# WeltXing/PyDyNet

Hardware: AMD Instinct MI355X
Metric: training-step samples/sec (6L Llama3, seq=256) (higher is better)
Workload: dtype f32

## Files before the change

### pydynet_amd/_lib.py

```python
from __future__ import annotations

import ctypes
import os
import re

_HERE = os.path.dirname(os.path.abspath(__file__))
LIB_PATH = os.environ.get("PDN_LIB") or os.path.join(_HERE, "libpdnhip.so")
HEADER_PATH = os.path.join(os.path.dirname(_HERE), "include", "pdn_hip.h")
EXT_HEADER_PATHS = (os.path.join(os.path.dirname(_HERE), "include", "pdn_optim.h"),)
LOSS_HEADER_PATHS = (os.path.join(os.path.dirname(_HERE), "include", "pdn_loss.h"),)
SEG_HEADER_PATHS = (os.path.join(os.path.dirname(_HERE), "include", "pdn_segattn.h"),)
ROWLOSS_HEADER_PATHS = (os.path.join(os.path.dirname(_HERE), "include", "pdn_rowloss.h"),)
SMOOTH_HEADER_PATHS = (os.path.join(os.path.dirname(_HERE), "include", "pdn_smoothloss.h"),)
EDIT_HEADER_PATHS = (os.path.join(os.path.dirname(_HERE), "include", "pdn_logitedit.h"),)
PERSAMPLE_HEADER_PATHS = (os.path.join(os.path.dirname(_HERE), "include", "pdn_persample.h"),)
FSM_HEADER_PATHS = (os.path.join(os.path.dirname(_HERE), "include", "pdn_fsm.h"),)
NORMGRAD_HEADER_PATHS = (os.path.join(os.path.dirname(_HERE), "include", "pdn_normgrad.h"),)

_CTYPE = {
    "int": ctypes.c_int,
    "int64_t": ctypes.c_int64,
    "float": ctypes.c_float,
    "double": ctypes.c_double,
}


def parse_header(path: str = HEADER_PATH):
    text = open(path).read()
    text = re.sub(r"/\*.*?\*/", "", text, flags=re.S)
    text = re.sub(r"//[^\n]*", "", text)
    protos = {}
    for m in re.finditer(r"(const\s+char\s*\*|int64_t|int)\s+(pdn[xlsrzeqfg]?_\w+)\s*\(([^)]*)\)\s*;", text, flags=re.S):
        ret, name, args = m.group(1), m.group(2), m.group(3)
        restype = ctypes.c_char_p if "char" in ret else _CTYPE[ret]
        argtypes = []
        args = args.strip()
        if args and args != "void":
            for a in args.split(","):
                a = a.strip()
                if "*" in a:
                    argtypes.append(ctypes.c_void_p)
                else:
                    base = a.replace("const", "").split()[0]
                    argtypes.append(_CTYPE[base])
        protos[name] = (restype, argtypes)
    return protos


class HipLibraryError(RuntimeError):

    def __init__(self, message, code=None):
        super().__init__(message)
        self.code = code


class _Lib:
    def __init__(self):
        if not os.path.exists(LIB_PATH):
            raise HipLibraryError(
                f"{LIB_PATH} not found: build it with `python -c 'import __graft_entry__ as g; g.build()'` "
                "(or `make -C pydynet_amd/csrc`). The HIP backend has no CPU fallback.")
        self.cdll = ctypes.CDLL(LIB_PATH, mode=ctypes.RTLD_GLOBAL)
        self.protos = parse_header()
        for path in (EXT_HEADER_PATHS + LOSS_HEADER_PATHS + SEG_HEADER_PATHS + ROWLOSS_HEADER_PATHS + SMOOTH_HEADER_PATHS
                     + EDIT_HEADER_PATHS + PERSAMPLE_HEADER_PATHS + FSM_HEADER_PATHS + NORMGRAD_HEADER_PATHS):
            self.protos.update(parse_header(path))
        self.fn = {}
        for name, (restype, argtypes) in self.protos.items():
            f = getattr(self.cdll, name)
            f.restype = restype
            f.argtypes = argtypes
            self.fn[name] = f
        self._last_error = self.fn["pdn_last_error"]
        self.free = self.fn["pdn_free"]

    def call(self, name, *args):
        rc = self.fn[name](*args)
        if rc != 0:
            msg = self._last_error()
            raise HipLibraryError(f"{name} failed (code {rc}): {msg.decode() if msg else ''}", rc)

    def query(self, name, *args):
        return self.fn[name](*args)


_LIB = None


def lib() -> _Lib:
    global _LIB
    if _LIB is None:
        _LIB = _Lib()
    return _LIB


def provides(name: str) -> bool:
    L = lib()
    fn = getattr(L, "fn", None)
    return name in fn if fn is not None else hasattr(L, name)


def is_built() -> bool:
    return os.path.exists(LIB_PATH)
```

### pydynet_amd/core/fused/_common.py

```python
from __future__ import annotations

import os

import numpy as np

from ...autograd import is_grad_enable
from ..tensor import Graph


def _hip():
    from ... import hipnp
    return hipnp


def _L():
    from ... import _lib
    return _lib.lib()


def _provides(name):
    from ... import _lib
    return _lib.provides(name)


# ... 37 lines not shown
def _is_leaf_f32(t):
    return (t.requires_grad and not t.last and t.grad is not None and t.grad.dtype == np.float32
            and (isinstance(t.grad, np.ndarray) or t.grad.is_contiguous()))


class _Deferred:

    _pending = None

    def _init_deferred(self, inputs, shape, dtype):
        self._pending, self._shape, self._dtype = tuple(inputs), tuple(int(v) for v in shape), np.dtype(dtype)
        self.__dict__["_data"] = None
        self.device = inputs[0].device
        self.copy = None
        self.grad = None
        self.requires_grad = bool(is_grad_enable() and any(t.requires_grad for t in inputs))
        self.last = list(inputs) if self.requires_grad else []
        if self.requires_grad:
            Graph._add_node(self)

    @property
    def data(self):
        d = self.__dict__.get("_data")
        if d is None and self._pending is not None:
            inputs, self._pending = self._pending, None
            with self.device:
                d = self.forward_(*inputs)
            self.__dict__["_data"] = d
        return d

    @data.setter
    def data(self, value):
        self.__dict__["_data"] = value
        self._pending = None

    @property
    def shape(self): return self._shape if self._pending is not None else self.data.shape
    @property
    def dtype(self): return self._dtype if self._pending is not None else self.data.dtype
    @property
    def ndim(self): return len(self.shape)
    @property
    def size(self): return int(np.prod(self.shape, dtype=np.int64))


def _pack_columns(hp, weights):
    fin = weights[0].shape[0]
    outs = [w.shape[1] for w in weights]
    cat = hp.empty((fin, int(np.sum(outs))), np.float32)
    pos = 0
    for w, n in zip(weights, outs):
        cat[:, pos:pos + n] = w
        pos += n
    return cat


def _weight_blocks(hp, L, dcat, weights, T, fin):
    ws = [_contig(w.data) for w in weights]
    stack = hp.stacked_view(ws)
    kb = ws[0].shape[1]
    if (fin == 288 and stack is not None and abs(stack._strides[0]) < (1 << 40) and dcat.is_contiguous()
            and os.environ.get("PDN_NO_DX_BLOCKS", "0") != "1"
            and L.query("pdn_gemm_outres_blocks_supported", T, kb, len(ws))):
        return ws, stack, kb
    return None


class DeferredInputGrad:

    def __init__(self, hp, dcat, ws, stack, kb, shape, T):
        self._hp, self.dcat, self.ws, self.stack, self.kb, self.T = hp, dcat, ws, stack, kb, T
        self.shape, self.dtype, self._array = tuple(shape), np.dtype(np.float32), None

    def materialise(self):
        if self._array is None:
            hp = self._hp
            dx = hp.empty(self.shape, np.float32)
            _L().call("pdn_gemm_outres_blocks_nt_f32", self.dcat._ptr, self.ws[0]._ptr, self.stack._strides[0], self.kb,
                      len(self.ws), dx._ptr, None, self.T, self.dcat.shape[1], 288, hp.stream())
            self._array, self.dcat, self.ws, self.stack = dx, None, None, None
        return self._array


def _materialised(g):
    return g.materialise() if isinstance(g, DeferredInputGrad) else g


def _dx_of_shared_input(hp, node, x, dcat, weights, T, fin, side=None):
    L = _L()
    blocks = _weight_blocks(hp, L, dcat, weights, T, fin)
    existing = getattr(node, "_existing", None)
    if (blocks is not None and side is None and not two_stream["enabled"] and type(x).__dict__.get("takes_deferred_grad", False)
            and type(x).fuse_bwd and T >= type(x).fuse_bwd_min_rows and x.device.is_hip and x.shape[-1] == 288
            and existing is not None and existing[0] is None and x.grad is None and x.last and x.requires_grad
            and hp.capturing() is None
            and _provides("pdng_outres_blocks_nt_rmsnorm_bwd_f32")):
        ws, stack, kb = blocks
        return DeferredInputGrad(hp, dcat, ws, stack, kb, x.shape, T)
    dx = hp.empty(x.shape, np.float32)
    ex = _foldable(node, 0, x)
    exr = ex.reshape(T, fin) if ex is not None else None
    if blocks is not None:
        ws, stack, kb = blocks
        L.call("pdn_gemm_outres_blocks_nt_f32", dcat._ptr, ws[0]._ptr, stack._strides[0], kb, len(ws),
               dx._ptr, exr._ptr if exr is not None else None, T, dcat.shape[1], fin, hp.stream())
    else:
        wcat = _pack_columns(hp, [w.data for w in weights])
        hp.gemm(dcat, wcat.T, dx.reshape(T, fin), residual=exr)
    return dx


def _gemm_raw(L, st, M, N, K, a_ptr, a_rs, a_cs, b, c_ptr, ldc, beta=0.0, residual_ptr=None, b_transposed=False):
    rs, cs = (b._strides[1], b._strides[0]) if b_transposed else (b._strides[0], b._strides[1])
    L.call("pdn_gemm_f32", M, N, K, 1.0, a_ptr, a_rs, a_cs, b._ptr, rs, cs, beta, c_ptr, ldc, None, 1, 1,
           0, 0, 0, 0, 0, 0, residual_ptr, None, 0, None, 0, st)
```

### pydynet_amd/core/fused/attn.py

```python
from __future__ import annotations

import contextlib
import math
import os

import numpy as np

from . import segments as _seg
from .norm import rms_norm
from ..tensor import Tensor, _Operator
from ._common import _hip, _L, _contig, _require_f32, _beside, _is_leaf_f32, _dx_of_shared_input


def _attn_layout(x):
    B, Lx, H, hd = x.shape
    st = x._strides
    if st[3] != 1 or (H > 1 and st[2] != hd) or st[1] % 4 or (B > 1 and st[0] % 4) or x._ptr % 16:
        return None
    return st[1], (st[0] if B > 1 else 0)


def _attn_mask_args(mask, B, H, Lq, Lk):
    if mask is None:
        return None, 0, 0, 0, 0, None
    m = mask
    if m.dtype != np.float32:
        m = m.astype(np.float32)
    shape = (1,) * (4 - m.ndim) + tuple(m.shape)
    if m.ndim > 4 or any(s not in (1, t) for s, t in zip(shape, (B, H, Lq, Lk))):
        raise ValueError(f"attention mask of shape {mask.shape} does not broadcast to {(B, H, Lq, Lk)}")
    m = _contig(m).reshape(shape)
    st = [0 if s == 1 else k for s, k in zip(shape, m._strides)]
    return m._ptr, st[0], st[1], st[2], st[3], m


def _key_bias_of(mask, B, H, Lq, Lk):
    shape = (1,) * (4 - mask.ndim) + tuple(mask.shape) if mask.ndim <= 4 else None
    if shape is None or shape[1] != 1 or shape[2] != 1 or shape[3] != Lk or shape[0] not in (1, B):
        return None
    m = mask if mask.dtype == np.float32 else mask.astype(np.float32)
    return _contig(m).reshape(shape[0], Lk)


_STREAM_MAX_BH = 65535


def _attn_kernel(B, H, hd, Lq, Lk, start_pos, mask, layouts):
    if not attention.use_flash or any(l is None for l in layouts):
        return None, None
    ql, kl, vl = layouts
    if Lq == Lk and start_pos == 0 and attention.use_resident and ql == kl == vl:
        kb = _key_bias_of(mask, B, H, Lq, Lk) if mask is not None else None
        if (mask is None or kb is not None) and _L().query("pdn_attention_supported", Lq, hd):
            return "resident", kb
    if _L().query("pdn_attention_stream_supported", hd) and kl == vl and B * H <= _STREAM_MAX_BH:
        return "stream", None
    return None, None


class SegmentBounds:
    __slots__ = ("start", "end", "shape", "on_hip")

    def __init__(self, start, end, shape, on_hip):
        self.start, self.end, self.shape, self.on_hip = start, end, tuple(shape), on_hip


def segment_bounds(segment_ids, on_hip):
    if isinstance(segment_ids, SegmentBounds):
        if segment_ids.on_hip != bool(on_hip):
            raise ValueError("segment bounds were made for another device")
        return segment_ids
    ids = segment_ids.data if isinstance(segment_ids, Tensor) else segment_ids
    if not on_hip:
        if not isinstance(ids, (np.ndarray, list, tuple)):
            ids = ids.get()
        ids = _seg.check(ids)
        start, end = _seg.bounds(ids)
        return SegmentBounds(start, end, ids.shape, False)
    hp, L = _hip(), _L()
    if isinstance(ids, (np.ndarray, list, tuple)):
        ids = hp.asarray(_seg.check(ids).astype(np.int32))
    elif ids.ndim != 2 or ids.dtype != np.int32:
        raise ValueError(f"segment_ids on the device must be a (B, L) int32 array, got shape {ids.shape} and dtype {ids.dtype}")
    ids = _contig(ids)
    B, Ls = ids.shape
    start, end = hp.empty((B, Ls), np.int32), hp.empty((B, Ls), np.int32)
    L.call("pdns_segment_bounds_i32", ids._ptr, B, Ls, start._ptr, end._ptr, hp.err_flag_ptr(), hp.stream())
    return SegmentBounds(start, end, (B, Ls), True)


def _segment_mask(seg, Lq):
    hp = _hip()
    keys = hp.asarray(np.arange(Lq, dtype=np.float32)).reshape(1, 1, 1, Lq)
    B = seg.shape[0]
# ... 109 lines not shown
    def backward_all(self, do):
        q, k, v = self.last
        B, Lq, H, hd = q.shape
        Lk = k.shape[1]
        causal = 1 if (self.causal and Lq > 1) else 0
        if self.xp is not np and self._kind == "segmented":
            hp, L = _hip(), _L()
            qd, kd, vd, seg, rs, bs = self._res
            self._res = None
            do = _contig(do)
            dq, dk, dv = (hp.empty((B, Lq, H, hd), np.float32) for _ in range(3))
            if rs != H * hd or (B > 1 and bs != Lq * H * hd):
                qd, kd, vd = qd.copy(), kd.copy(), vd.copy()
                rs, bs = H * hd, Lq * H * hd
            ws, wsb = hp.workspace(L.query("pdn_attention_bwd_workspace_bytes", B, H, Lq))
            L.call("pdns_attention_bwd_f32", qd._ptr, kd._ptr, vd._ptr, self.data._ptr, do._ptr, self._lse._ptr,
                   dq._ptr, dk._ptr, dv._ptr, B, H, Lq, hd, rs, bs, H * hd, Lq * H * hd, None, None, 0,
                   seg.start._ptr, seg.end._ptr, ws, wsb, hp.stream())
            return [dq, dk, dv]
        if self.xp is not np and self._kind == "resident":
            hp, L = _hip(), _L()
            qd, kd, vd, kb, rs, bs = self._res
            self._res = None
            do = _contig(do)
            dq, dk, dv = (hp.empty((B, Lq, H, hd), np.float32) for _ in range(3))
            if rs != H * hd or (B > 1 and bs != Lq * H * hd):
                qd, kd, vd = qd.copy(), kd.copy(), vd.copy()
                rs, bs = H * hd, Lq * H * hd
            ws, wsb = hp.workspace(L.query("pdn_attention_bwd_workspace_bytes", B, H, Lq))
            if kb is None:
                L.call("pdn_attention_bwd_f32", qd._ptr, kd._ptr, vd._ptr, self.data._ptr, do._ptr,
                       self._lse._ptr, dq._ptr, dk._ptr, dv._ptr, B, H, Lq, hd, rs, bs, H * hd, Lq * H * hd,
                       causal, None, None, ws, wsb, hp.stream())
            else:
                L.call("pdn_attention_bwd_bias_f32", qd._ptr, kd._ptr, vd._ptr, self.data._ptr, do._ptr,
                       self._lse._ptr, dq._ptr, dk._ptr, dv._ptr, B, H, Lq, hd, rs, bs, H * hd, Lq * H * hd,
                       causal, kb._ptr, Lq if kb.shape[0] > 1 else 0, ws, wsb, hp.stream())
            return [dq, dk, dv]
        if self.xp is not np and self._kind == "stream":
            hp, L = _hip(), _L()
            do = _contig(do)
            dq = hp.empty(q.shape, np.float32)
            ksrc, vsrc = _contig(k.data), _contig(v.data)
            dk, dv = hp.empty(k.shape, np.float32), hp.empty(v.shape, np.float32)
            klay = (H * hd, Lk * H * hd if B > 1 else 0)
            mp, sb, sh, sq, sk, keep = _attn_mask_args(self._mask_dev, B, H, Lq, Lk) \
                if self._mask_eff is not None else (None, 0, 0, 0, 0, None)
            ws, wsb = hp.workspace(L.query("pdn_attention_stream_bwd_workspace_bytes", B, H, Lq))
            qlay = (H * hd, Lq * H * hd if B > 1 else 0)
            qsrc = self._q_used
            L.call("pdn_attention_stream_bwd_f32", qsrc._ptr, ksrc._ptr, vsrc._ptr, self.data._ptr, do._ptr,
                   self._lse._ptr, dq._ptr, dk._ptr, dv._ptr, B, H, Lq, Lk, hd, qlay[0], qlay[1], klay[0], klay[1],
                   causal, self.start_pos, mp, sb, sh, sq, sk, None, None, ws, wsb, hp.stream())
            return [dq, dk, dv]
        p = self._p
        if self.xp is np:
            doT = do.transpose(0, 2, 1, 3)
            dv = np.matmul(p.swapaxes(-1, -2), doT).transpose(0, 2, 1, 3)
            dp = np.matmul(doT, v.data.transpose(0, 2, 3, 1))
            ds = (dp - (dp * p).sum(-1, keepdims=True)) * p / np.asarray(math.sqrt(hd), q.dtype)
            dq = np.matmul(ds, k.data.transpose(0, 2, 1, 3)).transpose(0, 2, 1, 3)
            dk = np.matmul(ds.swapaxes(-1, -2), q.data.transpose(0, 2, 1, 3)).transpose(0, 2, 1, 3)
            return [dq, dk, dv]
        hp, L = _hip(), _L()
        doT = do.transpose(0, 2, 1, 3)
        dv = hp.empty(v.shape, np.float32)
        hp.gemm(p.swapaxes(-1, -2), doT, dv.transpose(0, 2, 1, 3))
        dp = hp.empty(p.shape, np.float32)
        hp.gemm(doT, v.data.transpose(0, 2, 3, 1), dp)
        L.call("pdn_softmax_bwd_f32", p._ptr, dp._ptr, dp._ptr, B * H * Lq, Lk, math.sqrt(hd), hp.stream())
        dq, dk = hp.empty(q.shape, np.float32), hp.empty(k.shape, np.float32)
        hp.gemm(dp, k.data.transpose(0, 2, 1, 3), dq.transpose(0, 2, 1, 3))
        hp.gemm(dp.swapaxes(-1, -2), q.data.transpose(0, 2, 1, 3), dk.transpose(0, 2, 1, 3))
        return [dq, dk, dv]


class qkv_attention(_Operator):

    folds_existing = True
    enabled = True
    rope_epilogue = os.environ.get("PDN_NO_ROPE_EPILOGUE", "0") != "1"
    rope_min_rows = 4096
    prerotate = os.environ.get("PDN_NO_PREROTATE", "0") != "1"
    _rope_tables = {}

    @staticmethod
    def _rope_table(cos, sin, Lq, hd):
        hp, L = _hip(), _L()
        key = (cos._ptr, sin._ptr, Lq, hd)
        ent = qkv_attention._rope_tables.get(key)
        if ent is None:
            if len(qkv_attention._rope_tables) > 16:
                qkv_attention._rope_tables.clear()
            tab = hp.empty((Lq, hd, 2), np.float32)
            L.call("pdn_rope_table_f32", cos._ptr, sin._ptr, tab._ptr, Lq, hd, hp.stream())
            ent = qkv_attention._rope_tables[key] = (tab, cos, sin)
        return ent[0]

    def __init__(self, x, wq, wk, wv, cos, sin, n_heads, segment_ids=None):
        self._cos, self._sin, self.H = cos, sin, int(n_heads)
        self._segments = segment_ids
        super().__init__(x, wq, wk, wv)

    @staticmethod
    def _resident(L, hd):
        return bool(attention.use_resident and _L().query("pdn_attention_supported", L, hd))

    @staticmethod
    def applicable(x, L, hd, segment_ids=None):
        if not (qkv_attention.enabled and attention.use_flash and x.device.is_hip and x.dtype == np.float32
                and x.ndim == 3):
            return False
        if segment_ids is not None:
            return qkv_attention._resident(L, hd) and bool(_L().query("pdns_attention_supported", L, hd))
        return qkv_attention._resident(L, hd) or bool(_L().query("pdn_attention_stream_supported", hd))

    @staticmethod
    def _blocks(buf, T, D):
        hp = _hip()
        return hp.ndarray(buf._buf, buf._ptr, (3, T, D), (D, 3 * D, 1), buf.dtype)

    def forward_(self, x, wq, wk, wv):
        _require_f32(self, x, wq, wk, wv, self._cos, self._sin)
        hp, L = _hip(), _L()
        B, Lq, D = x.shape
        H, hd, T = self.H, D // self.H, B * Lq
        qkv = hp.empty((T, 3 * D), np.float32)
        blocks = self._blocks(qkv, T, D)
        ws = [_contig(w.data) for w in (wq, wk, wv)]
        stack = hp.stacked_view(ws)
        cos, sin = _contig(self._cos.data), _contig(self._sin.data)
        resident = qkv_attention._resident(Lq, hd)
        self.rotated = bool(qkv_attention.rope_epilogue and resident and stack is not None
                            and abs(stack._strides[0]) < (1 << 40)
                            and T >= qkv_attention.rope_min_rows
                            and L.query("pdn_qkv_rope_supported", T, D, D, Lq, hd))
        self.norm_folded = bool(self.rotated and isinstance(x, rms_norm) and x._pending is not None
                                and L.query("pdn_qkv_rope_norm_supported", T, D, D, Lq, hd))
        if self.norm_folded:
            raw_t, wn = x._pending
            raw = _contig(raw_t.data)
            xn, rms = hp.empty(x.shape, np.float32), hp.empty((T,), np.float32)
            tab = self._rope_table(cos, sin, Lq, hd)
            L.call("pdn_qkv_rope_norm_fwd_f32", raw._ptr, _contig(wn.data)._ptr, x.eps, xn._ptr, rms._ptr, ws[0]._ptr,
                   (ws[1]._ptr - ws[0]._ptr) // 4, qkv._ptr, tab._ptr, T, D, D, Lq, hd, D, hp.stream())
            x._adopt(raw, rms, xn)
        x2 = _contig(x.data).reshape(T, D)
        if self.norm_folded:
            pass
        elif self.rotated:
            tab = self._rope_table(cos, sin, Lq, hd)
            L.call("pdn_qkv_rope_fwd_f32", x2._ptr, ws[0]._ptr, (ws[1]._ptr - ws[0]._ptr) // 4, qkv._ptr, tab._ptr,
                   T, D, D, Lq, hd, D, hp.stream())
        elif stack is not None:
            hp.gemm(x2, stack, blocks)
        else:
            for i in range(3):
                hp.gemm(x2, ws[i], blocks[i])
        self.prerotated = bool(not self.rotated and resident and qkv_attention.rope_epilogue and qkv_attention.prerotate
                               and T >= qkv_attention.rope_min_rows
                               and L.query("pdn_attention_persistent_supported", Lq, hd))
        if self.prerotated:
            L.call("pdn_rope_rows_f32", qkv._ptr, cos._ptr, sin._ptr, qkv._ptr, T, Lq, 2 * H, hd, 3 * D, 3 * D, 0, hp.stream())
            self.rotated = True
        out = hp.empty((B, Lq, H, hd), np.float32)
        lse = hp.empty((B, H, Lq), np.float32)
        q, k, v = qkv._ptr, qkv._ptr + 4 * D, qkv._ptr + 8 * D
        self._seg = None
        if self._segments is not None:
            self._seg = seg = segment_bounds(self._segments, True)
            if seg.shape != (B, Lq) or not (resident and L.query("pdns_attention_supported", Lq, hd)):
                raise ValueError(f"qkv_attention: segment_ids of shape {seg.shape} for x of shape {tuple(x.shape)} "
                                 "(segments need a resident shape: see qkv_attention.applicable)")
            L.call("pdns_attention_fwd_f32", q, k, v, out._ptr, lse._ptr, B, H, Lq, hd, 3 * D, Lq * 3 * D, D, Lq * D,
                   None if self.rotated else cos._ptr, None if self.rotated else sin._ptr, seg.start._ptr, hp.stream())
        elif resident:
            L.call("pdn_attention_fwd_f32", q, k, v, out._ptr, lse._ptr, B, H, Lq, hd, 3 * D, Lq * 3 * D,
                   D, Lq * D, 1, None if self.rotated else cos._ptr, None if self.rotated else sin._ptr, hp.stream())
        else:
            if (3 * D) % 4 or D % 4:
                raise ValueError("qkv_attention: dim must be a multiple of 4")
            qd = blocks[0].copy()
            L.call("pdn_attention_stream_fwd_f32", qd._ptr, k, v, out._ptr, lse._ptr,
                   B, H, Lq, Lq, hd, D, Lq * D, 3 * D, Lq * 3 * D, 1 if Lq > 1 else 0, 0, None, 0, 0, 0, 0,
                   cos._ptr, sin._ptr, hp.stream())
        self._saved = (x2, qkv, lse, cos, sin)
        return out

    def backward_all(self, do):
        hp, L = _hip(), _L()
        x, wq, wk, wv = self.last
        B, Lq, D = x.shape
        H, hd, T = self.H, D // self.H, B * Lq
        x2, qkv, lse, cos, sin = self._saved
        do = _contig(do)
        dqkv = hp.empty((T, 3 * D), np.float32)
        dblocks = self._blocks(dqkv, T, D)
        q, k, v = qkv._ptr, qkv._ptr + 4 * D, qkv._ptr + 8 * D
        dq, dk, dv = dqkv._ptr, dqkv._ptr + 4 * D, dqkv._ptr + 8 * D
        if self._seg is not None:
            ws_, wsb = hp.workspace(L.query("pdn_attention_bwd_workspace_bytes", B, H, Lq))
            L.call("pdns_attention_bwd_f32", q, k, v, self.data._ptr, do._ptr, lse._ptr, dq, dk, dv, B, H, Lq, hd,
                   3 * D, Lq * 3 * D, D, Lq * D, cos._ptr, sin._ptr, 1 if self.rotated else 0,
                   self._seg.start._ptr, self._seg.end._ptr, ws_, wsb, hp.stream())
        elif qkv_attention._resident(Lq, hd):
            ws_, wsb = hp.workspace(L.query("pdn_attention_bwd_workspace_bytes", B, H, Lq))
            L.call("pdn_attention_bwd_rotated_f32" if self.rotated else "pdn_attention_bwd_f32", q, k, v, self.data._ptr,
                   do._ptr, lse._ptr, dq, dk, dv, B, H, Lq, hd,
                   3 * D, Lq * 3 * D, D, Lq * D, 1, cos._ptr, sin._ptr, ws_, wsb, hp.stream())
        else:
            ws_, wsb = hp.workspace(L.query("pdn_attention_stream_bwd_workspace_bytes", B, H, Lq))
            qd, dqd = self._blocks(qkv, T, D)[0].copy(), hp.empty((T, D), np.float32)
            L.call("pdn_attention_stream_bwd_f32", qd._ptr, k, v, self.data._ptr, do._ptr, lse._ptr, dqd._ptr, dk, dv,
                   B, H, Lq, Lq, hd, D, Lq * D, 3 * D, Lq * 3 * D, 1 if Lq > 1 else 0, 0, None, 0, 0, 0, 0,
                   cos._ptr, sin._ptr, ws_, wsb, hp.stream())
            dblocks[0] = dqd
        grads = [None] * 4
        weights = (wq, wk, wv)
        gstack = None
        if all(w.requires_grad and _is_leaf_f32(w) for w in weights):
            gstack = hp.stacked_view([w.grad for w in weights])
        side = _beside(hp, D, 3 * D, x.requires_grad and any(w.requires_grad for w in weights))
        dws = [hp.empty(w.shape, np.float32) if gstack is None and w.requires_grad and not _is_leaf_f32(w) else None
               for w in weights]
        with side or contextlib.nullcontext():
            if gstack is not None:
                hp.gemm(x2.T, dblocks, gstack, beta=1.0)
            else:
                for i, w in enumerate(weights):
                    if not w.requires_grad:
                        continue
                    if dws[i] is None:
                        hp.gemm(x2.T, dblocks[i], w.grad, beta=1.0)
                    else:
                        hp.gemm(x2.T, dblocks[i], dws[i])
                        grads[1 + i] = dws[i]
        if x.requires_grad:
            grads[0] = _dx_of_shared_input(hp, self, x, dqkv, (wq, wk, wv), T, D, side)
        if side is not None:
            side.join()
        return grads
```

### pydynet_amd/core/fused/ffn.py

```python
from __future__ import annotations

import contextlib
import os

import numpy as np

from .norm import rms_norm
from ..tensor import _Operator
from ._common import (_hip, _L, _contig, _require_f32, _foldable, _beside, _is_leaf_f32, _pack_columns, _dx_of_shared_input)


class gate_up_swiglu(_Operator):

    folds_existing = True
    enabled = True

    @staticmethod
    def applicable(x, wg, wu):
        return (gate_up_swiglu.enabled and x.device.is_hip and x.dtype == np.float32 and wg.dtype == np.float32
                and wu.dtype == np.float32 and wg.shape == wu.shape and wg.shape[1] % 4 == 0 and x.ndim >= 2)

    def __init__(self, x, w_gate, w_up):
        super().__init__(x, w_gate, w_up)

    @staticmethod
    def _halves(buf, T, F):
        hp = _hip()
        return hp.ndarray(buf._buf, buf._ptr, (2, T, F), (F, 2 * F, 1), buf.dtype)

    def forward_(self, x, wg, wu):
        _require_f32(self, x, wg, wu)
        hp, L = _hip(), _L()
        fin, F = wg.shape
        x2 = _contig(x.data).reshape(-1, fin)
        T = x2.shape[0]
        gu = hp.empty((T, 2 * F), np.float32)
        halves = self._halves(gu, T, F)
        ws = [_contig(wg.data), _contig(wu.data)]
        stack = hp.stacked_view(ws)
        if stack is not None:
            hp.gemm(x2, stack, halves)
        else:
            hp.gemm(x2, ws[0], halves[0])
            hp.gemm(x2, ws[1], halves[1])
        out = hp.empty(x.shape[:-1] + (F,), np.float32)
        L.call("pdn_swiglu_rows_fwd_f32", gu._ptr, out._ptr, T, F, hp.stream())
        self._saved = (x2, gu)
        return out

    def backward_all(self, dh):
        hp, L = _hip(), _L()
        x, wg, wu = self.last
        fin, F = wg.shape
        x2, gu = self._saved
        T = x2.shape[0]
        dh = _contig(dh)
        dgu = hp.empty((T, 2 * F), np.float32)
        L.call("pdn_swiglu_rows_bwd_f32", gu._ptr, dh._ptr, dgu._ptr, T, F, hp.stream())
        dhalves = self._halves(dgu, T, F)
        grads = [None] * 3
        weights = (wg, wu)
        gstack = None
        if all(w.requires_grad and _is_leaf_f32(w) for w in weights):
            gstack = hp.stacked_view([w.grad for w in weights])
        side = _beside(hp, fin, 2 * F, x.requires_grad and any(w.requires_grad for w in weights))
        dws = [hp.empty(w.shape, np.float32) if gstack is None and w.requires_grad and not _is_leaf_f32(w) else None
               for w in weights]
        with side or contextlib.nullcontext():
            if gstack is not None:
                hp.gemm(x2.T, dhalves, gstack, beta=1.0)
            else:
                for i, w in enumerate(weights):
                    if not w.requires_grad:
                        continue
                    if dws[i] is None:
                        hp.gemm(x2.T, dhalves[i], w.grad, beta=1.0)
                    else:
                        hp.gemm(x2.T, dhalves[i], dws[i])
                        grads[1 + i] = dws[i]
        if x.requires_grad:
            dx = hp.empty(x.shape, np.float32)
            ex = _foldable(self, 0, x)
            wcat = _pack_columns(hp, [wg.data, wu.data])
            hp.gemm(dgu, wcat.T, dx.reshape(T, fin), residual=ex.reshape(T, fin) if ex is not None else None)
            grads[0] = dx
        if side is not None:
            side.join()
        return grads


class ffn_swiglu(_Operator):

    folds_existing = True
    enabled = os.environ.get("PDN_NO_FFN_NODE", "0") != "1"
    epilogues = os.environ.get("PDN_NO_SWIGLU_EPILOGUE", "0") != "1"
    epilogue_min_rows = 4096

    @staticmethod
    def applicable(x, wg, wu, wd):
        return (ffn_swiglu.enabled and gate_up_swiglu.applicable(x, wg, wu) and wd.dtype == np.float32
                and wd.shape == (wg.shape[1], wg.shape[0]))

    def __init__(self, x, w_gate, w_up, w_down, residual=None):
        self.has_res = residual is not None
        super().__init__(*([x, w_gate, w_up, w_down] + ([residual] if self.has_res else [])))

    @staticmethod
    def _epilogue(T, F, fin, stack):
        return bool(ffn_swiglu.epilogues and stack is not None and T >= ffn_swiglu.epilogue_min_rows
                    and fin * F <= abs(stack._strides[0]) < (1 << 30) - fin * F
                    and _L().query("pdn_gateup_swiglu_supported", T, F, fin))

    def forward_(self, x, wg, wu, wd, r=None):
        _require_f32(self, x, wg, wu, wd, r)
        hp, L = _hip(), _L()
        fin, F = wg.shape
        T = x.size // fin
        gu = hp.empty((T, 2 * F), np.float32)
        h = hp.empty((T, F), np.float32)
        ws = [_contig(wg.data), _contig(wu.data)]
        stack = hp.stacked_view(ws)
        self.used_epilogue = self._epilogue(T, F, fin, stack)
        self.tiled_epilogue = bool(not self.used_epilogue and ffn_swiglu.epilogues and stack is not None
                                   and T >= ffn_swiglu.epilogue_min_rows and x.size == T * fin
                                   and L.query("pdn_gateup_swiglu_tiled_supported", T, F, fin))
        self.norm_folded = bool(self.used_epilogue and isinstance(x, rms_norm) and x._pending is not None
                                and L.query("pdn_gateup_swiglu_norm_supported", T, F, fin))
        if self.norm_folded:
            raw_t, wn = x._pending
            raw = _contig(raw_t.data)
            xn, rms = hp.empty(x.shape, np.float32), hp.empty((T,), np.float32)
            L.call("pdn_gateup_swiglu_norm_fwd_f32", raw._ptr, _contig(wn.data)._ptr, x.eps, xn._ptr, rms._ptr, ws[0]._ptr,
                   (ws[1]._ptr - ws[0]._ptr) // 4, gu._ptr, h._ptr, T, F, fin, fin, hp.stream())
            x._adopt(raw, rms, xn)
        x2 = _contig(x.data).reshape(-1, fin)
        if self.norm_folded:
            pass
        elif self.used_epilogue:
            L.call("pdn_gateup_swiglu_fwd_f32", x2._ptr, ws[0]._ptr, (ws[1]._ptr - ws[0]._ptr) // 4, gu._ptr, h._ptr,
                   T, F, fin, fin, hp.stream())
        elif self.tiled_epilogue:
            wsp, wsb = hp.workspace(L.query("pdn_gateup_swiglu_tiled_workspace_bytes", F, fin))
            L.call("pdn_gateup_swiglu_tiled_fwd_f32", x2._ptr, x2._strides[0], ws[0]._ptr, (ws[1]._ptr - ws[0]._ptr) // 4,
                   gu._ptr, h._ptr, T, F, fin, wsp, wsb, hp.stream())
        else:
            halves = gate_up_swiglu._halves(gu, T, F)
            if stack is not None:
                hp.gemm(x2, stack, halves)
            else:
                hp.gemm(x2, ws[0], halves[0])
                hp.gemm(x2, ws[1], halves[1])
            L.call("pdn_swiglu_rows_fwd_f32", gu._ptr, h._ptr, T, F, hp.stream())
        out = hp.empty(x.shape[:-1] + (fin,), np.float32)
        res = _contig(r.data).reshape(-1, fin) if r is not None else None
        hp.gemm(h, wd.data, out.reshape(-1, fin), residual=res)
        self._saved = (x2, gu, h)
        return out

    def backward_all(self, g):
        hp, L = _hip(), _L()
        x, wg, wu, wd = self.last[:4]
        fin, F = wg.shape
        x2, gu, h = self._saved
        T = x2.shape[0]
        grads = [None] * len(self.last)
        if self.has_res and self.last[4].requires_grad:
            grads[4] = g
        g2 = _contig(g).reshape(T, fin)
        if wd.requires_grad:
            if _is_leaf_f32(wd):
                hp.gemm(h.T, g2, wd.grad, beta=1.0)
            else:
                grads[3] = hp.empty((F, fin), np.float32)
                hp.gemm(h.T, g2, grads[3])
        if not (x.requires_grad or wg.requires_grad or wu.requires_grad):
            return grads
        dgu = hp.empty((T, 2 * F), np.float32)
        wdd = _contig(wd.data)
        if self.used_epilogue:
            L.call("pdn_swiglu_bwd_gemm_f32", g2._ptr, wdd._ptr, gu._ptr, dgu._ptr, T, F, fin, fin, hp.stream())
        elif self.tiled_epilogue and L.query("pdn_swiglu_bwd_tiled_supported", T, F, fin):
            L.call("pdn_swiglu_bwd_tiled_f32", g2._ptr, g2._strides[0], wdd._ptr, gu._ptr, dgu._ptr, T, F, fin, hp.stream())
        else:
            dh = hp.empty((T, F), np.float32)
            hp.gemm(g2, wdd.T, dh)
            L.call("pdn_swiglu_rows_bwd_f32", gu._ptr, dh._ptr, dgu._ptr, T, F, hp.stream())
        dhalves = gate_up_swiglu._halves(dgu, T, F)
        weights = (wg, wu)
        gstack = None
        if all(w.requires_grad and _is_leaf_f32(w) for w in weights):
            gstack = hp.stacked_view([w.grad for w in weights])
        if gstack is not None:
            hp.gemm(x2.T, dhalves, gstack, beta=1.0)
        else:
            for i, w in enumerate(weights):
                if not w.requires_grad:
                    continue
                if _is_leaf_f32(w):
                    hp.gemm(x2.T, dhalves[i], w.grad, beta=1.0)
                else:
                    grads[1 + i] = hp.empty(w.shape, np.float32)
                    hp.gemm(x2.T, dhalves[i], grads[1 + i])
        if x.requires_grad:
            grads[0] = _dx_of_shared_input(hp, self, x, dgu, (wg, wu), T, fin)
        return grads
```

### pydynet_amd/core/fused/norm.py

```python
from __future__ import annotations

import numpy as np

import os

from ...autograd import is_grad_enable
from ..tensor import _Operator
from ._common import (_hip, _L, _contig, _require_f32, _foldable, _is_leaf_f32, _Deferred, DeferredInputGrad, _materialised,
                      _provides)


class rms_norm(_Deferred, _Operator):

    folds_existing = True
    fold = os.environ.get("PDN_NO_NORM_FOLD", "0") != "1"
    fold_min_rows = 4096
    takes_deferred_grad = True
    fuse_bwd = os.environ.get("PDN_NO_NORM_BWD_FUSE", "0") != "1"
    fuse_bwd_min_rows = 65536

    def __init__(self, x, weight, eps=1e-6):
        self.eps = float(eps)
        if (rms_norm.fold and type(self) is rms_norm and x.device.is_hip and is_grad_enable()
                and x.dtype == np.float32 and weight.dtype == np.float32 and x.ndim >= 2 and x.shape[-1] == 288
                and weight.shape == (288,) and x.size // 288 >= rms_norm.fold_min_rows):
            self._init_deferred((x, weight), x.shape, np.float32)
        else:
            super().__init__(x, weight)

    def _adopt(self, raw, rms, out):
        self._x, self._rms = raw, rms
        self.data = out

    def forward_(self, x, w):
        if self.xp is np:
            self._rms = np.sqrt((x.data * x.data).mean(-1, keepdims=True) + np.asarray(self.eps, x.dtype))
            return x.data / self._rms * w.data
        _require_f32(self, x, w)
        hp, L = _hip(), _L()
        cols = x.shape[-1]
        self._x = _contig(x.data)
        rows = self._x.size // cols
        out = hp.empty(x.shape, np.float32)
        self._rms = hp.empty((rows,), np.float32)
        L.call("pdn_rmsnorm_fwd_f32", self._x._ptr, w.data._ptr, out._ptr, self._rms._ptr, rows, cols,
               self.eps, hp.stream())
        return out

    def backward_all(self, g):
        x, w = self.last
        if self.xp is np:
            z = x.data / self._rms
            dz = g * w.data
            dx = (dz - z * (z * dz).mean(-1, keepdims=True)) / self._rms
            return [dx if x.requires_grad else None,
                    (g * z).reshape(-1, w.shape[-1]).sum(0) if w.requires_grad else None]
        hp, L = _hip(), _L()
        cols = x.shape[-1]
        rows = self._x.size // cols
        fused = (isinstance(g, DeferredInputGrad) and x.requires_grad and cols == 288 and g.T == rows
                 and _provides("pdng_outres_blocks_nt_rmsnorm_bwd_f32"))
        g = g if fused else _contig(_materialised(g))
        dx = hp.empty(x.shape, np.float32)
        direct = w.requires_grad and _is_leaf_f32(w)
        dw = w.grad if direct else (hp.empty((cols,), np.float32) if w.requires_grad else None)
        ex = _foldable(self, 0, x) if x.requires_grad else None
        if fused:
            kb, nb = g.kb, len(g.ws)
            ws, wsb = hp.workspace(L.query("pdng_outres_blocks_nt_rmsnorm_bwd_workspace_bytes", rows, kb, nb))
            L.call("pdng_outres_blocks_nt_rmsnorm_bwd_f32", g.dcat._ptr, g.ws[0]._ptr, g.stack._strides[0], kb, nb,
                   self._x._ptr, w.data._ptr, self._rms._ptr, ex._ptr if ex is not None else None, dx._ptr,
                   dw._ptr if dw is not None else None, 1 if direct else 0, rows, g.dcat.shape[1], ws, wsb, hp.stream())
            return [dx, None if direct else dw]
        ws, wsb = hp.workspace(L.query("pdn_rmsnorm_bwd_workspace_bytes", rows, cols))
        L.call("pdn_rmsnorm_bwd_f32", self._x._ptr, w.data._ptr, self._rms._ptr, g._ptr,
               ex._ptr if ex is not None else None, dx._ptr,
               dw._ptr if dw is not None else None, 1 if direct else 0, rows, cols, ws, wsb, hp.stream())
        return [dx if x.requires_grad else None, None if direct else dw]


class layer_norm(_Operator):

    folds_existing = True

    def __init__(self, x, scale, shift, eps=1e-5):
        self.eps = float(eps)
        super().__init__(x, scale, shift)

    def forward_(self, x, w, b):
        if self.xp is np:
            mu = x.data.mean(-1, keepdims=True)
            self._c = x.data - mu
            self._sd = np.sqrt(np.square(self._c).mean(-1, keepdims=True) + np.asarray(self.eps, x.dtype))
            return self._c / self._sd * w.data + b.data
        _require_f32(self, x, w, b)
        hp, L = _hip(), _L()
        cols = x.shape[-1]
        self._x = _contig(x.data)
        rows = self._x.size // cols
        out = hp.empty(x.shape, np.float32)
        self._mean, self._rstd = hp.empty((rows,), np.float32), hp.empty((rows,), np.float32)
        L.call("pdn_layernorm_fwd_f32", self._x._ptr, _contig(w.data)._ptr, _contig(b.data)._ptr, out._ptr,
               self._mean._ptr, self._rstd._ptr, rows, cols, self.eps, hp.stream())
        return out

    def backward_all(self, g):
        x, w, b = self.last
        cols = x.shape[-1]
        if self.xp is np:
            xh = self._c / self._sd
            dz = g * w.data
            dx = (dz - dz.mean(-1, keepdims=True) - xh * (dz * xh).mean(-1, keepdims=True)) / self._sd
            return [dx if x.requires_grad else None,
                    (g * xh).reshape(-1, cols).sum(0).reshape(w.shape) if w.requires_grad else None,
                    g.reshape(-1, cols).sum(0).reshape(b.shape) if b.requires_grad else None]
        hp, L = _hip(), _L()
        rows = self._x.size // cols
        g = _contig(g)
        dx = hp.empty(x.shape, np.float32)
        dw_direct = w.requires_grad and _is_leaf_f32(w)
        db_direct = b.requires_grad and _is_leaf_f32(b)
        direct = dw_direct and db_direct
        dw = (w.grad if direct else hp.empty((cols,), np.float32)) if w.requires_grad else None
        db = (b.grad if direct else hp.empty((cols,), np.float32)) if b.requires_grad else None
        ws, wsb = hp.workspace(L.query("pdn_layernorm_bwd_workspace_bytes", rows, cols))
        ex = _foldable(self, 0, x) if x.requires_grad else None
        L.call("pdn_layernorm_bwd_f32", self._x._ptr, _contig(w.data)._ptr, self._mean._ptr, self._rstd._ptr, g._ptr,
               ex._ptr if ex is not None else None, dx._ptr, dw.reshape(-1)._ptr if dw is not None else None,
               db.reshape(-1)._ptr if db is not None else None, 1 if direct else 0, rows, cols, ws, wsb, hp.stream())
# ... 51 lines not shown
```

### pydynet_amd/csrc/gemm.hip

```cpp
#include "common.h"
#include <vector>
#include <mutex>
#include <stdlib.h>
#include <stdio.h>
#include <type_traits>

#include "gemm_tiled.h"
#include "gemm_stream.h"
#include "split_tn.h"

#include "gemm_select.h"
#include "gemm_prof.h"
#include "gemm_routes.h"


template <int WMV, int WNV, int WM, int WN, int BK, bool VEC, bool MASKS = false>
static void launch_layout(const GemmParams& p, bool a_kin, bool b_kin, dim3 grid, hipStream_t st) {
  constexpr int NT = WMV * WNV * 64;
  if (a_kin && b_kin)
    hipLaunchKernelGGL((gemm_f32_mfma_kernel<WMV, WNV, WM, WN, BK, true, true, VEC, false, MASKS>), grid, dim3(NT), 0, st, p);
  else if (a_kin && !b_kin)
    hipLaunchKernelGGL((gemm_f32_mfma_kernel<WMV, WNV, WM, WN, BK, true, false, VEC, false, MASKS>), grid, dim3(NT), 0, st, p);
  else if (!a_kin && b_kin)
    hipLaunchKernelGGL((gemm_f32_mfma_kernel<WMV, WNV, WM, WN, BK, false, true, VEC, false, MASKS>), grid, dim3(NT), 0, st, p);
// ... 27 lines not shown
extern "C" int pdn_gemm_prof_enable(int on) {
  std::lock_guard<std::mutex> lk(g_prof_mu);
  g_prof_on = on != 0;
  return PDN_OK;
}

extern "C" int pdn_gemm_prof_collect_fused(double* ms, double* flops, double* bytes, int64_t* launches) {
  std::lock_guard<std::mutex> lk(g_prof_mu);
  double tm = 0, tf = 0, tb = 0;
  int64_t n = 0;
  std::vector<ProfRec> keep;
  for (auto& r : g_prof) {
    if (r.family != 5) { keep.push_back(r); continue; }
    PDN_HIP(hipEventSynchronize(r.e1));
    float t = 0.f;
    PDN_HIP(hipEventElapsedTime(&t, r.e0, r.e1));
    tm += t; tf += r.flops; tb += r.bytes; n++;
    (void)hipEventDestroy(r.e0);
    (void)hipEventDestroy(r.e1);
  }
  g_prof.swap(keep);
  if (ms) *ms = tm;
  if (flops) *flops = tf;
  if (bytes) *bytes = tb;
  if (launches) *launches = n;
  return PDN_OK;
}

#define PDN_GEMM_FAMILIES 5
extern "C" int pdn_gemm_prof_collect_families(double* ms5, double* flops5, int64_t* launches5) {
  std::lock_guard<std::mutex> lk(g_prof_mu);
  double ms[PDN_GEMM_FAMILIES] = {0}, fl[PDN_GEMM_FAMILIES] = {0};
  int64_t n[PDN_GEMM_FAMILIES] = {0};
  for (auto& r : g_prof) {
    PDN_HIP(hipEventSynchronize(r.e1));
    float t = 0.f;
    PDN_HIP(hipEventElapsedTime(&t, r.e0, r.e1));
    const int f = r.family == 5 ? 2 : (r.family < 0 || r.family >= PDN_GEMM_FAMILIES ? 0 : r.family);
    ms[f] += t; fl[f] += r.flops; n[f]++;
    (void)hipEventDestroy(r.e0);
    (void)hipEventDestroy(r.e1);
  }
  for (int f = 0; f < PDN_GEMM_FAMILIES; ++f) {
    if (ms5) ms5[f] = ms[f];
    if (flops5) flops5[f] = fl[f];
    if (launches5) launches5[f] = n[f];
  }
  g_prof.clear();
  return PDN_OK;
}

extern "C" int pdn_gemm_prof_collect(double* total_ms, double* total_flops, int64_t* launches) {
  double ms[PDN_GEMM_FAMILIES], fl[PDN_GEMM_FAMILIES];
  int64_t n[PDN_GEMM_FAMILIES];
  int rc = pdn_gemm_prof_collect_families(ms, fl, n);
  if (rc) return rc;
  double tm = 0, tf = 0;
  int64_t tn = 0;
  for (int f = 0; f < PDN_GEMM_FAMILIES; ++f) { tm += ms[f]; tf += fl[f]; tn += n[f]; }
  if (total_ms) *total_ms = tm;
  if (total_flops) *total_flops = tf;
  if (launches) *launches = tn;
  return PDN_OK;
}

extern "C" int64_t pdn_gemm_f32_workspace_bytes(int M, int N, int K, int nbatch) {
  const int64_t base = (int64_t)64 * M * N * (int64_t)nbatch * 4;
  if (!pdn_outres_tn_split_supported(M, N, nbatch, K) && !(nbatch == 1 && pdn_down_dw_split_supported(M, N, K))) return base;
  return ((base + 255) & ~(int64_t)255) + pdn_outres_tn_split_extra_bytes(K);
}

struct GemmCall {
  GemmParams p;
  int nb1, nbatch;
  bool ext_on, mask_colsum;
  GemmLayout lay;
  int bt;
  int64_t ldb;
  void* workspace;
  int64_t workspace_bytes;
  int64_t ws_bytes, ws_floats;
  void* stream;
  hipStream_t st;
};
constexpr int kNotTaken = -0x7fffffff - 1;

static inline bool al16(const void* q) { return gemm_al16((uintptr_t)q); }

static int reduce_slabs(const GemmParams& p, int64_t total, int nbatch, int rvec, hipStream_t st) {
  const int blocks = (int)((total + 255) / 256 < 2048 ? (total + 255) / 256 : 2048);
  hipLaunchKernelGGL(gemm_splitk_reduce_kernel, dim3(blocks), dim3(256), 0, st, p, nbatch, rvec);
  PDN_LAUNCH_CHECK();
  return PDN_OK;
}

static int route_skinny(const GemmCall& c) {
  const GemmParams& p = c.p;
  if (!(p.M <= 4 && !c.ext_on && c.nbatch == 1 && !p.colsum && p.b_cs == 1 && p.a_cs == 1 && gemm_m4(p.N) && gemm_m4(p.b_rs) &&
        gemm_m4(p.ldc) && al16(p.B) && al16(p.C) && (!p.bias || al16(p.bias)) && (!p.residual || al16(p.residual)) && p.K > 0 &&
        (p.K <= 4096 || (int64_t)p.K <= 4ll * p.N)))
    return kNotTaken;
  const dim3 g((p.N + 127) / 128);
  switch (p.M) {
    case 1: hipLaunchKernelGGL((gemm_skinny_kernel<1>), g, dim3(256), 0, c.st, p); break;
    case 2: hipLaunchKernelGGL((gemm_skinny_kernel<2>), g, dim3(256), 0, c.st, p); break;
    case 3: hipLaunchKernelGGL((gemm_skinny_kernel<3>), g, dim3(256), 0, c.st, p); break;
    default: hipLaunchKernelGGL((gemm_skinny_kernel<4>), g, dim3(256), 0, c.st, p); break;
  }
  PDN_LAUNCH_CHECK();
  return PDN_OK;
}

static int route_narrow(GemmCall& c) {
  GemmParams& p = c.p;
  const int M = p.M, N = p.N, K = p.K;
  if (!(c.nbatch == 1 && !c.ext_on && N <= 16 && p.alpha == 1.f && !p.residual && !p.colsum && !getenv("PDN_GEMM_NO_NARROW")))
    return kNotTaken;
  if (p.beta == 0.f && pdn_gemm_narrow_nn_ok(M, N, K, p.a_rs, p.a_cs, p.A)) {
    if (getenv("PDN_GEMM_DEBUG")) fprintf(stderr, "pdn_gemm_f32 M=%d N=%d K=%d -> narrow NN\n", M, N, K);
    return pdn_gemm_narrow_nn_launch(p.A, p.a_rs, p.B, p.b_rs, p.b_cs, p.bias, p.C, p.ldc, M, N, K, c.stream);
  }
  int kps = 0;
  const int64_t cap = al16(c.workspace) ? c.ws_floats : 0;
  const int sp = !p.bias ? pdn_gemm_narrow_tn_plan(M, N, K, p.a_rs, p.a_cs, p.b_cs, p.A, cap, &kps) : 0;
  if (sp <= 0) return kNotTaken;
  if (getenv("PDN_GEMM_DEBUG")) fprintf(stderr, "pdn_gemm_f32 M=%d N=%d K=%d -> narrow TN (%d slabs)\n", M, N, K, sp);
  const int rc = pdn_gemm_narrow_tn_launch(p.A, p.a_cs, p.B, p.b_rs, (float*)c.workspace, M, N, K, kps, sp, c.stream);
  if (rc) return rc;
  p.splits = sp;
  return reduce_slabs(p, (int64_t)M * N, 1, (N % 4 == 0) && (p.ldc % 4 == 0) && al16(p.C), c.st);
}

static int route_outres(const GemmCall& c) {
  const GemmParams& p = c.p;
  const int M = p.M, N = p.N, K = p.K;
  if (!(c.nbatch == 1 && !c.ext_on && N == 288 && p.a_cs == 1 && p.alpha == 1.f && p.beta == 0.f && !p.colsum && K >= 768 &&
        al16(p.A) && al16(p.B) && !getenv("PDN_GEMM_NO_OUTRES")))
    return kNotTaken;
  const bool big = (M + 255) / 256 >= 224, mid = (M + 127) / 128 >= 224 && K >= 1536;
  int pl_nw, pl_kps;
  const bool cut = !big && M >= 8192 && K >= 1536 && pdn_gemm_outres_plan(M, K, &pl_nw, &pl_kps) > 1 &&
                   c.ws_bytes >= pdn_gemm_outres_workspace_bytes(M, K);
  if (!((big || mid || cut) && (c.bt || p.b_cs == 1) && pdn_gemm_outres_supported(M, N, K, p.a_rs, c.ldb, p.ldc, c.bt)))
    return kNotTaken;
  GemmProfScope prof(3, 2.0 * M * (double)N * (double)K, 0.0, c.stream);
  if (getenv("PDN_GEMM_DEBUG"))
    fprintf(stderr, "pdn_gemm_f32 M=%d N=%d K=%d -> output-resident (%s)\n", M, N, K, c.bt ? "NT" : "NN");
  return cut ? pdn_gemm_outres_ws_f32(p.A, p.B, p.C, p.bias, p.residual, M, N, K, p.a_rs, c.ldb, p.ldc, c.bt, c.workspace, c.ws_bytes,
                                      c.stream)
             : pdn_gemm_outres_f32(p.A, p.B, p.C, p.bias, p.residual, M, N, K, p.a_rs, c.ldb, p.ldc, c.bt, c.stream);
}

static int route_outres_split288(const GemmCall& c) {
  const GemmParams& p = c.p;
  const int M = p.M, N = p.N, K = p.K;
  if (!(c.nbatch == 1 && !c.ext_on && N == 288 && K == 288 && p.a_cs == 1 && p.alpha == 1.f && p.beta == 0.f && !p.colsum &&
        !getenv("PDN_GEMM_NO_OUTRES") && !getenv("PDN_GEMM_NO_ROWRES") && pdn_gemm_rowtile_mode(-1) != 3))
    return kNotTaken;
  auto overlaps_c = [&](const float* q, int64_t floats) {
    return q && q < (const float*)p.C + (int64_t)M * p.ldc && (const float*)p.C < q + floats;
  };
  if (!((c.bt || p.b_cs == 1) && pdn_rowtile_plain_ok(M, N, c.bt) && pdn_gemm_rowres_supported(M, N, K, p.a_rs, c.ldb, p.ldc, c.bt) &&
        !overlaps_c(p.A, (int64_t)M * p.a_rs) && !overlaps_c(p.B, (int64_t)288 * c.ldb) &&
        (p.residual == p.C || !overlaps_c(p.residual, (int64_t)M * p.ldc)) &&
        pdn_outres_split_takes(p.A, p.B, p.C, p.bias, p.residual, M, K, p.a_rs, c.ldb, p.ldc, c.bt, 0, 0, 1, c.stream)))
    return kNotTaken;
  if (getenv("PDN_GEMM_DEBUG"))
    fprintf(stderr, "pdn_gemm_f32 M=%d N=%d K=%d -> output-resident, split fp16 (%s)\n", M, N, K, c.bt ? "NT" : "NN");
  GemmProfScope prof(3, 2.0 * M * (double)N * (double)K, 0.0, c.stream);
  return pdn_outres_split_launch(p.A, p.B, p.C, p.bias, p.residual, M, K, p.a_rs, c.ldb, p.ldc, c.bt, 0, 0, c.stream, PDN_CNT_PROJ288_SPLIT);
}

static int route_rowres(const GemmCall& c) {
  const GemmParams& p = c.p;
  const int M = p.M, N = p.N, K = p.K, nbatch = c.nbatch;
  const bool one_dim = c.nb1 == 1 || p.nb2 == 1;
  const int64_t a_bs = c.nb1 == 1 ? p.a_bs2 : p.a_bs1, b_bs = c.nb1 == 1 ? p.b_bs2 : p.b_bs1, c_bs = c.nb1 == 1 ? p.c_bs2 : p.c_bs1;
  const bool blocks = nbatch > 1 && one_dim && a_bs == 0 && c_bs == N && p.ldc >= (int64_t)nbatch * N && !p.bias &&
                      N % 96 == 0 && (b_bs & 3) == 0;
  const int64_t n_all = (int64_t)N * (blocks ? nbatch : 1);
  const bool tilepiece = nbatch == 1 && K == 288 && n_all >= 96 && n_all % 32 == 0 && M >= 8192 &&
                         pdn_rowtile_plain_ok(M, (int)n_all, c.bt);
  if (!((nbatch == 1 || blocks) && !c.ext_on && K == 288 && p.a_cs == 1 && p.alpha == 1.f && p.beta == 0.f && !p.colsum &&
        (tilepiece || (!p.residual && n_all >= 768)) && n_all < (1 << 30) && M >= 8192 && al16(p.A) && al16(p.B) &&
        (!p.residual || al16(p.residual)) && !getenv("PDN_GEMM_NO_ROWRES")))
    return kNotTaken;
  if (!((c.bt || p.b_cs == 1) && pdn_gemm_rowres_supported(M, N, K, p.a_rs, c.ldb, p.ldc, c.bt))) return kNotTaken;
  GemmProfScope prof(2, 2.0 * M * (double)n_all * (double)K, 0.0, c.stream);
  if (getenv("PDN_GEMM_DEBUG"))
    fprintf(stderr, "pdn_gemm_f32 M=%d N=%lld K=%d -> row-resident (%s, %d block%s)\n", M, (long long)n_all, K,
            c.bt ? "NT" : "NN", blocks ? nbatch : 1, blocks ? "s" : "");
  return blocks ? pdn_gemm_rowres_blocks(p.A, p.B, p.C, M, (int)n_all, K, p.a_rs, c.ldb, p.ldc, c.bt, nbatch, b_bs, c.stream)
                : pdn_gemm_rowres_f32(p.A, p.B, p.C, p.bias, p.residual, M, N, K, p.a_rs, c.ldb, p.ldc, c.bt, c.stream);
}

static int route_outres_tn(GemmCall& c) {
  GemmParams& p = c.p;
  const int M = p.M, N = p.N, K = p.K;
  if (!(c.nbatch == 1 && !c.ext_on && M == 288 && p.a_rs == 1 && p.a_cs >= 288 && p.b_cs == 1 && p.alpha == 1.f && !p.colsum &&
        !p.bias && !p.residual && N >= 8192 && N % 32 == 0 && K % 32 == 0 && K >= 4096 && gemm_m4(p.a_cs) && gemm_m4(p.b_rs) &&
        al16(p.A) && al16(p.B) && (int64_t)288 * p.ldc < (1ll << 30) && (int64_t)32 * p.b_rs < (1ll << 30) &&
        !getenv("PDN_GEMM_NO_OUTRES")))
    return kNotTaken;
  int nw = 8, kps = K;
  const int splits = pdn_gemm_outres_tn_plan(N, K, &nw, &kps);
  const bool direct = splits == 1 && p.beta == 0.f;
  if (!(direct || (int64_t)splits * M * N <= c.ws_floats)) return kNotTaken;
  GemmProfScope prof(4, 2.0 * M * (double)N * (double)K, 0.0, c.stream);
  if (getenv("PDN_GEMM_DEBUG"))
    fprintf(stderr, "pdn_gemm_f32 M=%d N=%d K=%d -> output-resident TN (splits %d)\n", M, N, K, splits);
  const int rc = direct ? pdn_gemm_outres_tn_launch(p.A, p.B, p.C, N, K, p.a_cs, p.b_rs, p.ldc, 0, nw, kps, c.stream)
                        : pdn_gemm_outres_tn_launch(p.A, p.B, (float*)c.workspace, N, K, p.a_cs, p.b_rs, N, (int64_t)M * N, nw, kps,
                                                    c.stream);
  if (rc || direct) return rc;
  p.splits = splits;
  return reduce_slabs(p, (int64_t)M * N, 1, (p.ldc % 4 == 0) && al16(p.C) && al16(c.workspace), c.st);
}

static int route_outres_tn_blocks(GemmCall& c) {
  GemmParams& p = c.p;
  const int M = p.M, N = p.N, K = p.K, nbatch = c.nbatch;
  const bool one_dim = c.nb1 == 1 || p.nb2 == 1;
  const int64_t a_bs = c.nb1 == 1 ? p.a_bs2 : p.a_bs1, b_bs = c.nb1 == 1 ? p.b_bs2 : p.b_bs1;
  const int64_t n_all = (int64_t)N * nbatch;
  if (!(nbatch > 1 && one_dim && M == 288 && a_bs == 0 && b_bs == N && p.a_rs == 1 && p.a_cs >= 288 && p.b_cs == 1 &&
        p.b_rs >= n_all && p.alpha == 1.f && !p.colsum && !p.bias && !p.residual && N % 32 == 0 && n_all >= 768 && n_all <= 8192 &&
        K % 32 == 0 && K >= 16384 && gemm_m4(p.a_cs) && gemm_m4(p.b_rs) && al16(p.A) && al16(p.B) && !getenv("PDN_GEMM_NO_OUTRES")))
    return kNotTaken;
  int nw = 8, kps = K;
  int splits = pdn_gemm_outres_tn_plan((int)n_all, K, &nw, &kps);
  const int64_t xoff = (((int64_t)64 * M * n_all * 4 + 255) & ~(int64_t)255);
  const bool split16 = pdn_outres_tn_split_supported(M, N, nbatch, K) && pdn_outres_tn_split_enabled() && c.workspace &&
                       c.workspace_bytes >= xoff + pdn_outres_tn_split_extra_bytes(K) && al16(c.workspace);
  if (split16) {
    kps = ((K / 32 + pdn_outres_tn_split_ranges((int)n_all, K, splits) - 1) / pdn_outres_tn_split_ranges((int)n_all, K, splits)) * 32;
    splits = (K + kps - 1) / kps;
  }
  if (!(splits > 1 && (int64_t)splits * M * n_all <= c.ws_floats && nbatch * splits <= 65535)) return kNotTaken;
  GemmProfScope prof(4, 2.0 * M * (double)n_all * (double)K, 0.0, c.stream);
  if (getenv("PDN_GEMM_DEBUG"))
    fprintf(stderr, "pdn_gemm_f32 M=%d N=%lld K=%d -> output-resident TN%s (%d blocks, splits %d)\n", M,
            (long long)n_all, K, split16 ? ", split-fp16" : "", nbatch, splits);
  const int rc = split16 ? pdn_outres_tn_split_launch(p.A, p.B, (float*)c.workspace, (int)n_all, K, p.a_cs, p.b_rs, N, kps,
                                                      (char*)c.workspace + xoff, c.stream)
                         : pdn_gemm_outres_tn_blocks_launch(p.A, p.B, (float*)c.workspace, (int)n_all, K, p.a_cs, p.b_rs, N, nw, kps,
                                                            c.stream);
  if (rc) return rc;
  p.splits = splits;
  return reduce_slabs(p, (int64_t)M * n_all, nbatch,
                      (p.ldc % 4 == 0) && al16(p.C) && gemm_m4(p.c_bs1) && gemm_m4(p.c_bs2) && al16(c.workspace), c.st);
}

static int route_down_dw_split(GemmCall& c) {
  GemmParams& p = c.p;
  const int M = p.M, N = p.N, K = p.K;
  if (!(c.nbatch == 1 && !c.ext_on && p.a_rs == 1 && p.b_cs == 1 && p.alpha == 1.f && !p.colsum && !p.bias && !p.residual &&
        pdn_down_dw_split_supported(M, N, K) && p.a_cs >= M && p.b_rs >= N && gemm_m4(p.a_cs) && gemm_m4(p.b_rs) && al16(p.A) &&
        al16(p.B) && c.workspace && al16(c.workspace) && pdn_outres_tn_split_enabled() && !getenv("PDN_GEMM_NO_OUTRES")))
    return kNotTaken;
  const int64_t xoff = (((int64_t)64 * M * N * 4 + 255) & ~(int64_t)255);
  const int ranges = pdn_down_dw_split_ranges(M, K);
  const int kps = ((K / 32 + ranges - 1) / ranges) * 32;
  const int splits = (K + kps - 1) / kps;
  if (!(c.workspace_bytes >= xoff + pdn_outres_tn_split_extra_bytes(K) && splits > 1 && splits <= 64)) return kNotTaken;
  if (getenv("PDN_GEMM_DEBUG"))
    fprintf(stderr, "pdn_gemm_f32 M=%d N=%d K=%d -> output-resident TN, split-fp16, transposed (splits %d)\n", M, N, K, splits);
  GemmProfScope prof(4, 2.0 * M * (double)N * (double)K, 0.0, c.stream);
  const int rc = pdn_down_dw_split_launch(p.B, p.A, (float*)c.workspace, M, K, p.b_rs, p.a_cs, kps, (char*)c.workspace + xoff, c.stream);
  if (rc) return rc;
  p.splits = splits;
  return reduce_slabs(p, (int64_t)M * N, 1, (p.ldc % 4 == 0) && al16(p.C), c.st);
}

static int route_stream_or_tiled(GemmCall& c) {
  GemmParams& p = c.p;
  const int M = p.M, N = p.N, K = p.K, nbatch = c.nbatch;
  const bool a_kin = c.lay.a_kin, b_kin = c.lay.b_kin, vec = c.lay.vec;
  const GemmChoice ch = gemm_select(M, N, K, nbatch, p.a_rs, p.b_cs, c.lay, c.ext_on, p.colsum != nullptr, c.mask_colsum, c.ws_floats);
  PDN_CHECK_ARG(ch.cfg >= 0, "pdn_gemm_f32: no tile configuration");
  if (getenv("PDN_GEMM_DEBUG")) {
    char line[256];
    gemm_route_line(line, sizeof(line), M, N, K, nbatch, c.lay, ch);
    fputs(line, stderr);
  }
  p.tiles_m = ch.tiles_m; p.tiles_n = ch.tiles_n; p.k_per_split = ch.k_per_split; p.splits = ch.splits;
  PDN_CHECK_ARG((int64_t)nbatch * p.splits <= 65535, "pdn_gemm_f32: batch*splits too large (%d)",
                nbatch * p.splits);
  dim3 grid(p.tiles_m * p.tiles_n, nbatch * p.splits);
  hipStream_t st = c.st;

  GemmProfScope prof(ch.use_stream ? 1 : 0, 2.0 * M * N * (double)K * nbatch, 0.0, c.stream);
  if (ch.use_stream) {
    constexpr int SNW = kStreamWaves;
    const dim3 sgrid(p.tiles_m * p.tiles_n * p.splits, nbatch);
    switch (ch.kind) {
      case kStreamLdsEdge:
        switch (ch.sshape) {
          case 0: hipLaunchKernelGGL((gemm_tn_stream_lds_kernel<3, 3, SNW, true>), sgrid, dim3(SNW * 64), 0, st, p); break;
          case 1: hipLaunchKernelGGL((gemm_tn_stream_lds_kernel<5, 2, SNW, true>), sgrid, dim3(SNW * 64), 0, st, p); break;
          case 2: hipLaunchKernelGGL((gemm_tn_stream_lds_kernel<2, 5, SNW, true>), sgrid, dim3(SNW * 64), 0, st, p); break;
          case 3: hipLaunchKernelGGL((gemm_tn_stream_lds_kernel<4, 2, SNW, true>), sgrid, dim3(SNW * 64), 0, st, p); break;
          default: hipLaunchKernelGGL((gemm_tn_stream_lds_kernel<2, 4, SNW, true>), sgrid, dim3(SNW * 64), 0, st, p); break;
        }
        break;
      case kStreamDma: hipLaunchKernelGGL((gemm_tn_stream_dma_kernel<3, 3, SNW>), sgrid, dim3(SNW * 64), 0, st, p); break;
      case kStreamLds: hipLaunchKernelGGL((gemm_tn_stream_lds_kernel<3, 3, SNW, false>), sgrid, dim3(SNW * 64), 0, st, p); break;
      case kStreamDirect: hipLaunchKernelGGL((gemm_tn_stream_kernel<3, 3, SNW, false>), sgrid, dim3(SNW * 64), 0, st, p); break;
      case kStreamDirectEdge: hipLaunchKernelGGL((gemm_tn_stream_kernel<3, 3, SNW, true>), sgrid, dim3(SNW * 64), 0, st, p); break;
    }
  } else if (c.ext_on) {
    if (!vec) launch_layout<2, 2, 1, 1, 32, false, true>(p, a_kin, b_kin, grid, st);
    else switch (ch.cfg) {
      case 0: launch_layout<2, 2, 2, 2, 32, true, true>(p, a_kin, b_kin, grid, st); break;
      case 3: launch_layout<4, 1, 1, 2, 32, true, true>(p, a_kin, b_kin, grid, st); break;
      case 6: launch_layout<2, 2, 4, 2, 16, true, true>(p, a_kin, b_kin, grid, st); break;
      case 7: launch_layout<2, 2, 2, 4, 16, true, true>(p, a_kin, b_kin, grid, st); break;
      case 8: launch_layout<4, 1, 2, 3, 16, true, true>(p, a_kin, b_kin, grid, st); break;
      default: launch_layout<2, 2, 1, 1, 32, true, true>(p, a_kin, b_kin, grid, st); break;
    }
  } else if (vec) {
    switch (ch.cfg) {
      case 0: launch_layout<2, 2, 2, 2, 32, true>(p, a_kin, b_kin, grid, st); break;
      case 1: launch_layout<4, 1, 1, 3, 32, true>(p, a_kin, b_kin, grid, st); break;
      case 2: launch_layout<1, 4, 3, 1, 32, true>(p, a_kin, b_kin, grid, st); break;
      case 3: launch_layout<4, 1, 1, 2, 32, true>(p, a_kin, b_kin, grid, st); break;
      case 4: launch_layout<1, 4, 2, 1, 32, true>(p, a_kin, b_kin, grid, st); break;
      case 6: launch_layout<2, 2, 4, 2, 16, true>(p, a_kin, b_kin, grid, st); break;
      case 7: launch_layout<2, 2, 2, 4, 16, true>(p, a_kin, b_kin, grid, st); break;
      case 8: launch_layout<4, 1, 2, 3, 16, true>(p, a_kin, b_kin, grid, st); break;
      case 9: launch_layout<1, 4, 3, 2, 16, true>(p, a_kin, b_kin, grid, st); break;
      case 10: launch_layout<2, 1, 1, 3, 32, true>(p, a_kin, b_kin, grid, st); break;
      case 11: launch_layout<1, 2, 3, 1, 32, true>(p, a_kin, b_kin, grid, st); break;
      case 12: launch_layout<4, 1, 1, 3, 16, true>(p, a_kin, b_kin, grid, st); break;
      default: launch_layout<2, 2, 1, 1, 32, true>(p, a_kin, b_kin, grid, st); break;
    }
  } else {
    launch_layout<2, 2, 1, 1, 32, false>(p, a_kin, b_kin, grid, st);
  }
  PDN_LAUNCH_CHECK();
  if (p.splits <= 1) return PDN_OK;
  return reduce_slabs(p, (int64_t)M * N * nbatch, nbatch,
                      (N % 4 == 0) && (p.ldc % 4 == 0) && al16(p.C) && gemm_m4(p.c_bs1) && gemm_m4(p.c_bs2) &&
                          (!p.bias || al16(p.bias)) && (!p.residual || al16(p.residual)) && al16(c.workspace), st);
}

static int gemm_f32_impl(int M, int N, int K, float alpha, const float* A, int64_t a_rs,
                         int64_t a_cs, const float* B, int64_t b_rs, int64_t b_cs, float beta,
                         float* C, int64_t ldc, const float* bias, int nb1, int nb2,
                         int64_t a_bs1, int64_t a_bs2, int64_t b_bs1, int64_t b_bs2,
                         int64_t c_bs1, int64_t c_bs2, const float* residual,
                         float* b_colsum, int colsum_accumulate, void* workspace,
                         int64_t workspace_bytes, void* stream, uint32_t* relu_mask, const uint32_t* grad_mask,
                         float* mask_colsum = nullptr) {
  const bool ext_on = relu_mask || grad_mask;
  PDN_CHECK_ARG(!ext_on || (nb1 == 1 && nb2 == 1 && N % 32 == 0 && !b_colsum),
                "pdn_gemm_f32: the mask epilogues need one batch and N a multiple of 32 (N = %d)", N);
  PDN_CHECK_ARG(M >= 0 && N >= 0 && K >= 0 && nb1 >= 0 && nb2 >= 0, "pdn_gemm_f32: negative extent");
  if (M == 0 || N == 0 || nb1 == 0 || nb2 == 0) return PDN_OK;
  PDN_CHECK_ARG(A && B && C, "pdn_gemm_f32: null operand");
  PDN_CHECK_ARG(ldc >= N, "pdn_gemm_f32: ldc (%lld) < N (%d)", (long long)ldc, N);

  GemmCall c;
  GemmParams& p = c.p;
  p.A = A; p.B = B; p.C = C; p.bias = bias; p.ws = (float*)workspace;
  p.residual = residual; p.colsum = b_colsum; p.colsum_acc = colsum_accumulate;
  p.relu_mask = relu_mask; p.grad_mask = grad_mask; p.mask_colsum = grad_mask ? mask_colsum : nullptr;
  p.M = M; p.N = N; p.K = K;
  p.a_rs = a_rs; p.a_cs = a_cs; p.b_rs = b_rs; p.b_cs = b_cs; p.ldc = ldc;
  p.nb2 = nb2;
  p.a_bs1 = a_bs1; p.a_bs2 = a_bs2; p.b_bs1 = b_bs1; p.b_bs2 = b_bs2; p.c_bs1 = c_bs1; p.c_bs2 = c_bs2;
  p.alpha = alpha; p.beta = beta;
  c.nb1 = nb1; c.nbatch = nb1 * nb2;
  c.ext_on = ext_on; c.mask_colsum = mask_colsum != nullptr;
  c.lay = gemm_layout(M, N, K, a_rs, a_cs, b_rs, b_cs, a_bs1, a_bs2, b_bs1, b_bs2, (uintptr_t)A, (uintptr_t)B);
  c.bt = (b_rs == 1 && b_cs != 1) ? 1 : 0;
  c.ldb = c.bt ? b_cs : b_rs;
  c.workspace = workspace; c.workspace_bytes = workspace_bytes;
  c.ws_bytes = (workspace && workspace_bytes > 0) ? workspace_bytes : 0;
  c.ws_floats = c.ws_bytes / 4;
  c.stream = stream; c.st = (hipStream_t)stream;

  if (b_colsum) {
    if (c.lay.a_kin || c.lay.b_kin || !c.lay.vec || c.nbatch != 1) {
      pdn_set_error("pdn_gemm_f32: b_colsum needs the x^T @ g layout (A m-contiguous, B n-contiguous, aligned, unbatched)");
      return PDN_EUNSUPPORTED;
    }
  }
  int rc;
  if ((rc = route_skinny(c)) != kNotTaken) return rc;
  if ((rc = route_narrow(c)) != kNotTaken) return rc;
  if ((rc = route_outres(c)) != kNotTaken) return rc;
  if ((rc = route_outres_split288(c)) != kNotTaken) return rc;
  if ((rc = route_rowres(c)) != kNotTaken) return rc;
  if ((rc = route_outres_tn(c)) != kNotTaken) return rc;
  if ((rc = route_outres_tn_blocks(c)) != kNotTaken) return rc;
  if ((rc = route_down_dw_split(c)) != kNotTaken) return rc;
  return route_stream_or_tiled(c);
}

extern "C" int pdn_gemm_f32(int M, int N, int K, float alpha, const float* A, int64_t a_rs,
                            int64_t a_cs, const float* B, int64_t b_rs, int64_t b_cs, float beta,
                            float* C, int64_t ldc, const float* bias, int nb1, int nb2,
                            int64_t a_bs1, int64_t a_bs2, int64_t b_bs1, int64_t b_bs2,
                            int64_t c_bs1, int64_t c_bs2, const float* residual,
                            float* b_colsum, int colsum_accumulate, void* workspace,
                            int64_t workspace_bytes, void* stream) {
  return gemm_f32_impl(M, N, K, alpha, A, a_rs, a_cs, B, b_rs, b_cs, beta, C, ldc, bias, nb1, nb2, a_bs1, a_bs2, b_bs1, b_bs2,
                       c_bs1, c_bs2, residual, b_colsum, colsum_accumulate, workspace, workspace_bytes, stream, nullptr, nullptr);
}

extern "C" int pdn_relu_mask_supported(int64_t rows, int cols) { return rows > 0 && cols > 0 && cols % 32 == 0; }

extern "C" int pdn_linear_relu_fwd_f32(const float* x, int64_t x_rs, const float* W, int64_t w_rs, int64_t w_cs,
                                       const float* bias, float* h, int64_t ldh, uint32_t* mask, int M, int N, int K,
                                       void* stream) {
  PDN_CHECK_ARG(x && W && h && mask, "pdn_linear_relu_fwd_f32: null operand");
  PDN_CHECK_ARG(pdn_relu_mask_supported(M, N), "pdn_linear_relu_fwd_f32: out features must be a multiple of 32 (N = %d)", N);
  pdn_count(PDN_CNT_LINEAR_RELU_FWD);
  return gemm_f32_impl(M, N, K, 1.f, x, x_rs, 1, W, w_rs, w_cs, 0.f, h, ldh, bias, 1, 1, 0, 0, 0, 0, 0, 0, nullptr, nullptr, 0,
                       nullptr, 0, stream, mask, nullptr);
}

extern "C" int pdn_linear_dx_masked_f32(const float* g, int64_t g_rs, const float* W, int64_t w_rs, int64_t w_cs,
                                        float* dx, int64_t ld, const float* existing, const uint32_t* mask,
                                        float* colsum_partials, int M, int fin, int fout, void* stream) {
  PDN_CHECK_ARG(g && W && dx && mask, "pdn_linear_dx_masked_f32: null operand");
  PDN_CHECK_ARG(pdn_relu_mask_supported(M, fin), "pdn_linear_dx_masked_f32: in features must be a multiple of 32 (%d)", fin);
  PDN_CHECK_ARG(!colsum_partials || ((uintptr_t)colsum_partials & 15) == 0, "pdn_linear_dx_masked_f32: unaligned partials");
  pdn_count(PDN_CNT_LINEAR_DX_MASKED);
  return gemm_f32_impl(M, fin, fout, 1.f, g, g_rs, 1, W, w_cs, w_rs, 0.f, dx, ld, nullptr, 1, 1, 0, 0, 0, 0, 0, 0, existing,
                       nullptr, 0, nullptr, 0, stream, nullptr, mask, colsum_partials);
}

__global__ __launch_bounds__(256) void relu_mask_bwd_kernel(const float4* __restrict__ g, const uint32_t* __restrict__ mask,
                                                            float4* __restrict__ dz, int64_t n4) {
  for (int64_t i = (int64_t)blockIdx.x * 256 + threadIdx.x; i < n4; i += (int64_t)gridDim.x * 256) {
    const uint32_t w = mask[i >> 3] >> (4 * (i & 7));
    float4 v = g[i];
    v.x = (w & 1u) ? v.x : 0.f; v.y = (w & 2u) ? v.y : 0.f; v.z = (w & 4u) ? v.z : 0.f; v.w = (w & 8u) ? v.w : 0.f;
    dz[i] = v;
  }
}

extern "C" int pdn_relu_mask_bwd_f32(const float* g, const uint32_t* mask, float* dz, int64_t rows, int cols, void* stream) {
  PDN_CHECK_ARG(g && mask && dz, "pdn_relu_mask_bwd_f32: null operand");
  PDN_CHECK_ARG(pdn_relu_mask_supported(rows, cols) && (((uintptr_t)g | (uintptr_t)dz) & 15) == 0,
                "pdn_relu_mask_bwd_f32: cols must be a multiple of 32 and the arrays 16-byte aligned");
  const int64_t n4 = rows * cols / 4;
  const int blocks = (int)std::min<int64_t>((n4 + 255) / 256, 8192);
  hipLaunchKernelGGL(relu_mask_bwd_kernel, dim3(blocks), dim3(256), 0, (hipStream_t)stream, (const float4*)g, mask, (float4*)dz, n4);
  PDN_LAUNCH_CHECK();
  return PDN_OK;
}

__global__ __launch_bounds__(256) void swiglu_pack_weights_kernel(const float* __restrict__ wg, int64_t w_stride, float* __restrict__ out,
                                                                  int K, int F, int Np) {
  const int64_t total = (int64_t)K * (Np / 4);
  for (int64_t i = (int64_t)blockIdx.x * 256 + threadIdx.x; i < total; i += (int64_t)gridDim.x * 256) {
    const int k = (int)(i / (Np / 4)), c = (int)(i - (int64_t)k * (Np / 4)) * 4;
    const int grp = c >> 6, up = (c >> 5) & 1, col = 32 * grp + (c & 31);
    float4 v = make_float4(0.f, 0.f, 0.f, 0.f);
    if (col < F) v = *reinterpret_cast<const float4*>(wg + (up ? w_stride : 0) + (int64_t)k * F + col);
    *reinterpret_cast<float4*>(out + (int64_t)k * Np + c) = v;
  }
}

static int swiglu_packed_cols(int F) { return (2 * F + 255) / 256 * 256; }

extern "C" int pdn_gateup_swiglu_tiled_supported(int M, int F, int K) {
  return M >= 4096 && M % 128 == 0 && F >= 256 && F % 32 == 0 && K >= 64 && K % 4 == 0 && !getenv("PDN_NO_TILED_SWIGLU");
}
extern "C" int64_t pdn_gateup_swiglu_tiled_workspace_bytes(int F, int K) { return (int64_t)K * swiglu_packed_cols(F) * 4; }

static void swiglu_params(GemmParams& p, int M, int N, int K, int BM, int BN, int BK) {
  p.bias = nullptr; p.residual = nullptr; p.colsum = nullptr; p.colsum_acc = 0;
  p.relu_mask = nullptr; p.grad_mask = nullptr; p.mask_colsum = nullptr; p.ws = nullptr;
  p.M = M; p.N = N; p.K = K; p.nb2 = 1;
  p.a_bs1 = p.a_bs2 = p.b_bs1 = p.b_bs2 = p.c_bs1 = p.c_bs2 = 0;
  p.alpha = 1.f; p.beta = 0.f; p.splits = 1;
  p.k_per_split = (K + BK - 1) / BK * BK;
  p.tiles_m = (M + BM - 1) / BM; p.tiles_n = (N + BN - 1) / BN;
}

extern "C" int pdn_gateup_swiglu_tiled_fwd_f32(const float* x, int64_t ldx, const float* w_gate, int64_t w_stride, float* gu,
                                               float* h, int M, int F, int K, void* workspace, int64_t workspace_bytes,
                                               void* stream) {
  PDN_CHECK_ARG(x && w_gate && gu && h && workspace, "pdn_gateup_swiglu_tiled_fwd_f32: null operand");
  PDN_CHECK_ARG(pdn_gateup_swiglu_tiled_supported(M, F, K) && ldx % 4 == 0 && w_stride % 4 == 0 &&
                    ((((uintptr_t)x | (uintptr_t)w_gate | (uintptr_t)gu | (uintptr_t)h | (uintptr_t)workspace) & 15) == 0),
                "pdn_gateup_swiglu_tiled_fwd_f32: unsupported shape or alignment (M %d, F %d, K %d)", M, F, K);
  const int Np = swiglu_packed_cols(F);
// ... 132 lines not shown
```

### pydynet_amd/csrc/gemm_routes.h

```cpp
#pragma once
#include <stdint.h>

bool pdn_gemm_narrow_nn_ok(int M, int N, int K, int64_t a_rs, int64_t a_cs, const void* A);
int pdn_gemm_narrow_nn_launch(const float* A, int64_t lda, const float* B, int64_t b_rs, int64_t b_cs, const float* bias,
                              float* C, int64_t ldc, int M, int N, int K, void* stream);
int pdn_gemm_narrow_tn_plan(int Mc, int N, int K, int64_t a_rs, int64_t a_cs, int64_t b_cs, const void* A, int64_t ws_cap_floats,
                            int* kps);
int pdn_gemm_narrow_tn_launch(const float* A, int64_t a_cs, const float* B, int64_t b_rs, float* slabs, int Mc, int N, int K,
                              int kps, int splits, void* stream);

extern "C" int64_t pdn_gemm_outres_workspace_bytes(int M, int K);
extern "C" int pdn_gemm_outres_plan(int M, int K, int* nw, int* kps);
extern "C" int pdn_gemm_outres_supported(int M, int N, int K, int64_t lda, int64_t ldb, int64_t ldc, int b_trans);
extern "C" int pdn_gemm_outres_f32(const float* A, const float* B, float* C, const float* bias,
                                   const float* residual, int M, int N, int K, int64_t lda, int64_t ldb,
                                   int64_t ldc, int b_trans, void* stream);
extern "C" int pdn_gemm_outres_ws_f32(const float* A, const float* B, float* C, const float* bias, const float* residual,
                                      int M, int N, int K, int64_t lda, int64_t ldb, int64_t ldc, int b_trans,
                                      void* workspace, int64_t workspace_bytes, void* stream);
int pdn_outres_blocks_nt_launch(const float* A, const float* W, int64_t b_block_stride, int kb, int nb, float* C, int M,
                                int64_t lda, int64_t ldc, void* stream);
int pdn_gemm_outres_tn_plan(int N, int K, int* nw_out, int* k_per_split_out);
int pdn_gemm_outres_tn_launch(const float* X, const float* G, float* C, int N, int K, int64_t ldx, int64_t ldg,
                              int64_t ldc, int64_t slab, int nw, int k_per_split, void* stream);
int pdn_gemm_outres_tn_blocks_launch(const float* X, const float* G, float* C, int N, int K, int64_t ldx, int64_t ldg,
                                     int nb_cols, int nw, int k_per_split, void* stream);
int pdn_outres_ce_dx_launch(const float* logits, int64_t ldl, const float* lse, const int64_t* targets, float gscale,
                            const float* gdev, const float* W, int64_t ldw, float* dx, int64_t ldc,
                            const float* residual, int M, int V, void* workspace, int64_t workspace_bytes, void* stream);
int pdn_outres_ce_dw_launch(const float* X, const float* logits, float* C, int N, int K, int64_t ldx, int64_t ldg,
                            int64_t ldc, int64_t slab, int nw, int k_per_split, const float* lse,
                            const int64_t* targets, float gscale, const float* gdev, float* colsum, void* stream);
int pdn_outres_ce_dx_deferred_launch(const float* logits, int64_t ldl, const float* rowmax, int max_parts,
                                     const int64_t* targets, float gscale, const float* W, int64_t ldw, float* dx,
                                     int64_t ldc, float* lse_out, int M, int V, void* workspace, int64_t workspace_bytes,
                                     void* stream);
extern "C" int pdn_linear_ce_dx_deferred_supported(int64_t M, int V, int K);

int pdn_outres_split_takes(const float* A, const float* B, const float* C, const float* bias, const float* residual, int M,
                           int K, int64_t lda, int64_t ldb, int64_t ldc, int b_trans, int kb, int64_t b_bstride, int splits,
                           void* stream);
int pdn_outres_split_launch(const float* A, const float* B, float* C, const float* bias, const float* residual, int M, int K,
                            int64_t lda, int64_t ldb, int64_t ldc, int b_trans, int kb, int64_t b_bstride, void* stream,
                            int count_slot);
int pdn_outres_split_norm_bwd_partial_rows(int M);
int pdn_outres_split_norm_bwd_launch(const float* A, const float* W, int64_t b_bstride, int kb, int nb, const float* x,
                                     const float* w, const float* rms, const float* ex, float* dx, float* dwpart, int M,
                                     int64_t lda, void* stream);

int pdn_colsum_partials_launch(const float* part, int nb, int cols, float* out, int accumulate, void* stream);

extern "C" int pdn_gemm_rowres_supported(int M, int N, int K, int64_t lda, int64_t ldb, int64_t ldc, int b_trans);
int pdn_rowtile_plain_ok(int M, int N, int b_trans);
extern "C" int pdn_gemm_rowres_f32(const float* A, const float* B, float* C, const float* bias,
                                   const float* residual, int M, int N, int K, int64_t lda, int64_t ldb,
                                   int64_t ldc, int b_trans, void* stream);
int pdn_gemm_rowres_blocks(const float* A, const float* B, float* C, int M, int N, int K, int64_t lda, int64_t ldb,
                           int64_t ldc, int b_trans, int nblocks, int64_t b_block_stride, void* stream);
extern "C" int pdn_gemm_rowtile_mode(int mode);
```

### pydynet_amd/csrc/gemm_rowres.hip

```cpp
#include "common.h"
#include "gemm_rowtile.h"
#include "gemm_prof.h"
#include "gemm_routes.h"
#include <stdlib.h>

static int pdn_ablation_switch(const char* name) {
  const char* e = getenv(name);
  const int v = e ? atoi(e) : 0;
  if (v) fprintf(stderr, "[pdnhip] WARNING: %s=%d -- timing ablation active, results of the affected kernels are WRONG\n", name, v);
  return v;
}

typedef float f32x16 __attribute__((ext_vector_type(16)));

struct RowResParams {
  const float* A;
  const float* B;
  float* C;
  const float* bias;
  const float* residual;
  int M, N;
  int64_t lda, ldb, ldc;
  int chunks, chunks_per_wg;
  int cpb;
  int64_t b_bstride;
  float* H;
  const float* GU;
  const float2* rope;
  int64_t ldh;
  int F;
  int L, hd, rope_chunks;
  unsigned hd_magic;
  unsigned g_off, u_off;
  float* lse;
  int epi_ablate;
};

__device__ __forceinline__ void rr_glds16(const float* g, float* l) {
  __builtin_amdgcn_global_load_lds((const __attribute__((address_space(1))) void*)g,
                                   (__attribute__((address_space(3))) void*)l, 16, 0, 0);
}

#define RR_NC 96
#define RR_KP 96

__device__ __forceinline__ void rr_store(const RowResParams& p, f32x16 (&acc)[3], int m0, int c, int li, int lh,
                                         bool full, int nt) {
  float* __restrict__ Cw = p.C + (int64_t)m0 * p.ldc + c * RR_NC;
  const float* __restrict__ Rw = p.residual ? p.residual + (int64_t)m0 * p.ldc + c * RR_NC : nullptr;
  const unsigned ldc = (unsigned)p.ldc;
  unsigned o0 = (unsigned)(4 * lh) * ldc + li;
  asm volatile("" : "+v"(o0));
  float bv[3];
#pragma unroll
  for (int j = 0; j < 3; ++j) bv[j] = (p.bias && j < nt) ? p.bias[c * RR_NC + 32 * j + li] : 0.f;
  const int mrem = p.M - m0 - 4 * lh;
#define RR_ROWS(GUARD, RES)                                                      \
  {                                                                              \
    unsigned o = o0;                                                             \
    _Pragma("unroll") for (int q = 0; q < 4; ++q) {                              \
      _Pragma("unroll") for (int e = 0; e < 4; ++e) {                            \
        const int r = 4 * q + e;                                                 \
        if (!GUARD || 8 * q + e < mrem) {                                        \
          _Pragma("unroll") for (int j = 0; j < 3; ++j) {                        \
            if (!GUARD || j < nt) {                                              \
              float v = acc[j][r] + bv[j];                                       \
              if (RES) v += Rw[o + 32 * j];                                      \
              Cw[o + 32 * j] = v;                                                \
            }                                                                    \
          }                                                                      \
        }                                                                        \
        o += (e == 3) ? 5 * ldc : ldc;                                           \
      }                                                                          \
    }                                                                            \
  }
  if (p.epi_ablate & 4) {
  } else if (full && nt == 3) {
    if (Rw) RR_ROWS(false, true) else RR_ROWS(false, false)
  } else {
    if (Rw) RR_ROWS(true, true) else RR_ROWS(true, false)
  }
#undef RR_ROWS
#pragma unroll
  for (int j = 0; j < 3; ++j)
#pragma unroll
    for (int r = 0; r < 16; ++r) acc[j][r] = 0.f;
// ... 522 lines not shown
    p.rope = reinterpret_cast<const float2*>(epi->rope); p.L = epi->L; p.hd = epi->hd;
    p.rope_chunks = epi->rope_cols / RR_NC;
    p.hd_magic = (unsigned)(((1ull << 32) + (unsigned)epi->hd - 1) / (unsigned)epi->hd);
    p.g_off = epi->g_off; p.u_off = epi->u_off;
    p.lse = epi->lse;
  }
  static const int s_pdn_rowres_epi_ablate = pdn_ablation_switch("PDN_ROWRES_EPI_ABLATE");
  p.epi_ablate = s_pdn_rowres_epi_ablate;
  hipStream_t st = (hipStream_t)stream;
  static const int ablate = getenv("PDN_ROWRES_ABLATE") ? atoi(getenv("PDN_ROWRES_ABLATE")) : 0;
  static const int nw_env = getenv("PDN_ROWRES_NW") ? atoi(getenv("PDN_ROWRES_NW")) : 0;
  static const int stage_env = getenv("PDN_ROWRES_STAGE") ? atoi(getenv("PDN_ROWRES_STAGE")) : -1;
  const int rb8 = (M + 255) / 256;
  const int nw = kind ? 8 : nw_env ? nw_env : (rb8 >= 192 || (int64_t)rb8 * p.chunks >= 256) ? 8 : 4;
  const int stage = kind ? 1 : stage_env >= 0 ? stage_env : (nw == 8 ? 1 : 0);
  const int row_blocks = (M + 32 * nw - 1) / (32 * nw), target = nw == 4 ? 512 : 256;
  int nsplit = 1;
  while (row_blocks * nsplit < target && nsplit < p.chunks) ++nsplit;
  p.chunks_per_wg = (p.chunks + nsplit - 1) / nsplit;
  if (kind == 1) p.chunks_per_wg += p.chunks_per_wg & 1;
  if (kind == 4) p.chunks_per_wg = p.chunks;
  nsplit = (p.chunks + p.chunks_per_wg - 1) / p.chunks_per_wg;
  if (kind == 5 && !epi->lse) { const_cast<RowResEpi*>(epi)->parts = nsplit; return PDN_OK; }
  const dim3 grid(row_blocks, nsplit);
#define RR_LAUNCH(BT_, NW_, AB_) if (stage) hipLaunchKernelGGL((gemm_rowres_kernel<36, BT_, NW_, 1, 0>), grid, dim3(NW_ * 64), 0, st, p); else hipLaunchKernelGGL((gemm_rowres_kernel<36, BT_, NW_, 0, AB_>), grid, dim3(NW_ * 64), 0, st, p)
  if (kind == 1) {
    hipLaunchKernelGGL((gemm_rowres_kernel<36, false, 8, 1, 0, 1>), grid, dim3(512), 0, st, p);
  } else if (kind == 2) {
    hipLaunchKernelGGL((gemm_rowres_kernel<36, true, 8, 1, 0, 2>), grid, dim3(512), 0, st, p);
  } else if (kind == 3) {
    hipLaunchKernelGGL((gemm_rowres_kernel<36, false, 8, 1, 0, 3>), grid, dim3(512), 0, st, p);
  } else if (kind == 4) {
    hipLaunchKernelGGL((gemm_rowres_kernel<36, false, 8, 1, 0, 4>), grid, dim3(512), 0, st, p);
  } else if (kind == 5) {
    hipLaunchKernelGGL((gemm_rowres_kernel<36, false, 8, 1, 0, 5>), grid, dim3(512), 0, st, p);
  } else if (nw == 8) {
    if (b_trans) RR_LAUNCH(true, 8, 0); else RR_LAUNCH(false, 8, 0);
  } else if (b_trans) {
    RR_LAUNCH(true, 4, 0);
  } else if (ablate == 2) {
    RR_LAUNCH(false, 4, 2);
  } else if (ablate == 32) {
    RR_LAUNCH(false, 4, 32);
  } else {
    RR_LAUNCH(false, 4, 0);
  }
#undef RR_LAUNCH
  pdn_count(PDN_CNT_ROWRES_CHUNK);
  if (kind) pdn_count(PDN_CNT_ROWRES_CHUNK_EPI);
  PDN_LAUNCH_CHECK();
  return PDN_OK;
}

extern "C" int pdn_gateup_swiglu_supported(int M, int F, int K) {
  return (K == 288 && F % RR_NC == 0 && F >= RR_NC && M >= 1 && (int64_t)64 * F < (1ll << 29)) ? 1 : 0;
}
extern "C" int pdn_gateup_swiglu_fwd_f32(const float* x, const float* w_gate, int64_t w_stride, float* gu, float* h, int M,
                                         int F, int K, int64_t ldx, void* stream) {
  if (M == 0 || F == 0) return PDN_OK;
  PDN_CHECK_ARG(x && w_gate && gu && h, "pdn_gateup_swiglu_fwd_f32: null operand");
  const int64_t ws = w_stride < 0 ? -w_stride : w_stride;
  if (!pdn_gateup_swiglu_supported(M, F, K) || ws % 4 != 0 || ws < (int64_t)K * F || ws + (int64_t)K * F >= (1ll << 30)) {
    pdn_set_error("pdn_gateup_swiglu_fwd_f32: unsupported shape M=%d F=%d K=%d (K 288, F a multiple of 96)", M, F, K);
    return PDN_EUNSUPPORTED;
  }
  RowResEpi e{1, h, F, nullptr, F, nullptr, 1, 1, 0};
  e.g_off = w_stride < 0 ? (unsigned)ws : 0u;
  e.u_off = w_stride < 0 ? 0u : (unsigned)ws;
  const float* wbase = w_stride < 0 ? w_gate + w_stride : w_gate;
  const int tk = pdn_gemm_prof_begin(5, 2.0 * M * (2.0 * F) * K, 4.0 * ((double)M * K + 2.0 * K * F + 3.0 * M * F), stream);
  const int rc = rowres_launch(x, wbase, gu, nullptr, nullptr, M, 2 * F, K, ldx, F, 2 * F, 0, 2, ws, stream, &e);
  pdn_gemm_prof_end(tk, stream);
  return rc;
}
static int rowtile_would_take(int M, int N, int epi, int F) {
  RowTileArgs ta;
  memset(&ta, 0, sizeof(ta));
  ta.M = M; ta.N = N; ta.lda = 288; ta.ldb = N; ta.ldc = N; ta.nblocks = 1; ta.epi = epi; ta.F = F;
  return pdn_rowtile_takes(ta);
}
extern "C" int pdn_gateup_swiglu_norm_supported(int M, int F, int K) {
  return (pdn_gateup_swiglu_supported(M, F, K) && rowtile_would_take(M, 2 * F, 1, F)) ? 1 : 0;
}
extern "C" int pdn_gateup_swiglu_norm_fwd_f32(const float* x, const float* norm_w, float eps, float* xn, float* rms,
                                              const float* w_gate, int64_t w_stride, float* gu, float* h, int M, int F,
                                              int K, int64_t ldx, void* stream) {
  if (M == 0 || F == 0) return PDN_OK;
  PDN_CHECK_ARG(x && norm_w && xn && rms && w_gate && gu && h, "pdn_gateup_swiglu_norm_fwd_f32: null operand");
  const int64_t ws = w_stride < 0 ? -w_stride : w_stride;
  if (!pdn_gateup_swiglu_norm_supported(M, F, K) || ws % 4 != 0 || ws < (int64_t)K * F || ws + (int64_t)K * F >= (1ll << 30)) {
    pdn_set_error("pdn_gateup_swiglu_norm_fwd_f32: unsupported shape M=%d F=%d K=%d", M, F, K);
    return PDN_EUNSUPPORTED;
  }
  RowResEpi e{1, h, F, nullptr, F, nullptr, 1, 1, 0};
  e.g_off = w_stride < 0 ? (unsigned)ws : 0u;
  e.u_off = w_stride < 0 ? 0u : (unsigned)ws;
  e.norm_w = norm_w; e.xn = xn; e.rms = rms; e.ldxn = K; e.norm_eps = eps;
  const float* wbase = w_stride < 0 ? w_gate + w_stride : w_gate;
  const int tk = pdn_gemm_prof_begin(5, 2.0 * M * (2.0 * F) * K, 4.0 * (2.0 * M * K + 2.0 * K * F + 3.0 * M * F), stream);
  const int rc = rowres_launch(x, wbase, gu, nullptr, nullptr, M, 2 * F, K, ldx, F, 2 * F, 0, 2, ws, stream, &e);
  pdn_gemm_prof_end(tk, stream);
  return rc;
}
extern "C" int pdn_swiglu_bwd_gemm_f32(const float* dy, const float* w_down, const float* gu, float* dgu, int M, int F, int K,
                                       int64_t ldy, void* stream) {
  if (M == 0 || F == 0) return PDN_OK;
  PDN_CHECK_ARG(dy && w_down && gu && dgu, "pdn_swiglu_bwd_gemm_f32: null operand");
  if (!pdn_gateup_swiglu_supported(M, F, K)) {
    pdn_set_error("pdn_swiglu_bwd_gemm_f32: unsupported shape M=%d F=%d K=%d (K 288, F a multiple of 96)", M, F, K);
    return PDN_EUNSUPPORTED;
  }
  RowResEpi e{2, nullptr, 0, gu, F, nullptr, 1, 1, 0};
  const int tk = pdn_gemm_prof_begin(5, 2.0 * M * (double)F * K, 4.0 * ((double)M * K + (double)K * F + 4.0 * M * F), stream);
  const int rc = rowres_launch(dy, w_down, dgu, nullptr, nullptr, M, F, K, ldy, K, 2 * F, 1, 1, 0, stream, &e);
  pdn_gemm_prof_end(tk, stream);
  return rc;
}
extern "C" int pdn_qkv_rope_supported(int M, int D, int K, int L, int hd) {
  return (K == 288 && D % RR_NC == 0 && hd >= 32 && hd % 2 == 0 && D % hd == 0 && 3 * D < 65536 && L % 32 == 0 && L > 0 && M % L == 0) ? 1 : 0;
}
extern "C" int pdn_qkv_rope_fwd_f32(const float* x, const float* wq, int64_t w_stride, float* qkv, const float* rope, int M,
                                    int D, int K, int L, int hd, int64_t ldx, void* stream) {
  if (M == 0 || D == 0) return PDN_OK;
  PDN_CHECK_ARG(x && wq && qkv && rope && (((uintptr_t)rope & 7) == 0), "pdn_qkv_rope_fwd_f32: null / misaligned operand");
  if (!pdn_qkv_rope_supported(M, D, K, L, hd) || w_stride % 4 != 0) {
    pdn_set_error("pdn_qkv_rope_fwd_f32: unsupported shape M=%d D=%d K=%d L=%d hd=%d", M, D, K, L, hd);
    return PDN_EUNSUPPORTED;
  }
  RowResEpi e{3, nullptr, 0, nullptr, 0, rope, L, hd, 2 * D};
  const int tk = pdn_gemm_prof_begin(5, 2.0 * M * (3.0 * D) * K, 4.0 * ((double)M * K + 3.0 * K * D + 3.0 * M * D), stream);
  const int rc = rowres_launch(x, wq, qkv, nullptr, nullptr, M, 3 * D, K, ldx, D, 3 * D, 0, 3, w_stride, stream, &e);
  pdn_gemm_prof_end(tk, stream);
  return rc;
}

extern "C" int pdn_qkv_rope_norm_supported(int M, int D, int K, int L, int hd) {
  return (pdn_qkv_rope_supported(M, D, K, L, hd) && rowtile_would_take(M, 3 * D, 3, 0)) ? 1 : 0;
}
extern "C" int pdn_qkv_rope_norm_fwd_f32(const float* x, const float* norm_w, float eps, float* xn, float* rms, const float* wq,
                                         int64_t w_stride, float* qkv, const float* rope, int M, int D, int K, int L, int hd,
                                         int64_t ldx, void* stream) {
  if (M == 0 || D == 0) return PDN_OK;
  PDN_CHECK_ARG(x && norm_w && xn && rms && wq && qkv && rope && (((uintptr_t)rope & 7) == 0),
                "pdn_qkv_rope_norm_fwd_f32: null / misaligned operand");
  if (!pdn_qkv_rope_norm_supported(M, D, K, L, hd) || w_stride % 4 != 0) {
    pdn_set_error("pdn_qkv_rope_norm_fwd_f32: unsupported shape M=%d D=%d K=%d L=%d hd=%d", M, D, K, L, hd);
    return PDN_EUNSUPPORTED;
  }
  RowResEpi e{3, nullptr, 0, nullptr, 0, rope, L, hd, 2 * D};
  e.norm_w = norm_w; e.xn = xn; e.rms = rms; e.ldxn = K; e.norm_eps = eps;
  const int tk = pdn_gemm_prof_begin(5, 2.0 * M * (3.0 * D) * K, 4.0 * (2.0 * M * K + 3.0 * K * D + 3.0 * M * D), stream);
  const int rc = rowres_launch(x, wq, qkv, nullptr, nullptr, M, 3 * D, K, ldx, D, 3 * D, 0, 3, w_stride, stream, &e);
  pdn_gemm_prof_end(tk, stream);
  return rc;
}

extern "C" int pdn_linear_lse_supported(int64_t M, int V, int K) {
  return (K == 288 && V % 32 == 0 && V >= RR_NC && M >= 49152 && M < (1ll << 31)) ? 1 : 0;
}
extern "C" int pdn_linear_lse_fwd_f32(const float* x, const float* w, const float* bias, float* logits, float* lse, int M,
                                      int V, int K, int64_t ldx, int64_t ldw, int64_t ldl, void* stream) {
  if (M == 0 || V == 0) return PDN_OK;
  PDN_CHECK_ARG(x && w && logits && lse, "pdn_linear_lse_fwd_f32: null operand");
  if (!pdn_linear_lse_supported(M, V, K) || (ldl & 3) || ((uintptr_t)logits & 15) || ((uintptr_t)bias & 15)) {
    pdn_set_error("pdn_linear_lse_fwd_f32: unsupported shape M=%d V=%d K=%d", M, V, K);
    return PDN_EUNSUPPORTED;
  }
  RowResEpi e{4, nullptr, 0, nullptr, 0, nullptr, 1, 1, 0};
  e.lse = lse;
  const int tk = pdn_gemm_prof_begin(2, 2.0 * M * (double)V * K, 0.0, stream);
  const int rc = rowres_launch(x, w, logits, bias, nullptr, M, V, K, ldx, ldw, ldl, 0, 1, 0, stream, &e);
  pdn_gemm_prof_end(tk, stream);
  return rc;
}

extern "C" int pdn_linear_rowmax_supported(int64_t M, int V, int K) {
  return (K == 288 && V % 32 == 0 && V >= RR_NC && M >= 1 && M < (1ll << 31)) ? 1 : 0;
}
extern "C" int pdn_linear_rowmax_parts(int64_t M, int V, int K) {
  if (!pdn_linear_rowmax_supported(M, V, K)) return 0;
  RowResEpi e{5, nullptr, 0, nullptr, 0, nullptr, 1, 1, 0};
  alignas(16) static float dummy[4];
  if (rowres_launch(dummy, dummy, dummy, nullptr, nullptr, (int)M, V, K, K, V, V, 0, 1, 0, nullptr, &e) != PDN_OK) return 0;
  return e.parts;
}
extern "C" int pdn_linear_rowmax_fwd_f32(const float* x, const float* w, const float* bias, float* logits, float* rowmax,
                                         int M, int V, int K, int64_t ldx, int64_t ldw, int64_t ldl, void* stream) {
  if (M == 0 || V == 0) return PDN_OK;
  PDN_CHECK_ARG(x && w && logits && rowmax, "pdn_linear_rowmax_fwd_f32: null operand");
  if (!pdn_linear_rowmax_supported(M, V, K) || (ldl & 3) || ((uintptr_t)logits & 15) || ((uintptr_t)bias & 15)) {
    pdn_set_error("pdn_linear_rowmax_fwd_f32: unsupported shape M=%d V=%d K=%d", M, V, K);
    return PDN_EUNSUPPORTED;
  }
  RowResEpi e{5, nullptr, 0, nullptr, 0, nullptr, 1, 1, 0};
  e.lse = rowmax;
  const int tk = pdn_gemm_prof_begin(2, 2.0 * M * (double)V * K, 0.0, stream);
  const int rc = rowres_launch(x, w, logits, bias, nullptr, M, V, K, ldx, ldw, ldl, 0, 1, 0, stream, &e);
  pdn_gemm_prof_end(tk, stream);
  return rc;
}

__global__ void rr_rope_table_kernel(const float* __restrict__ cs, const float* __restrict__ sn, float2* __restrict__ out,
                                     int total, int hd) {
  const int i = blockIdx.x * blockDim.x + threadIdx.x;
  if (i >= total) return;
  const int pos = i / hd, col = i - pos * hd;
  const float c = cs[pos * (hd / 2) + (col >> 1)], s = sn[pos * (hd / 2) + (col >> 1)];
  out[i] = make_float2(c, (col & 1) ? s : -s);
}
extern "C" int pdn_rope_table_f32(const float* cos_t, const float* sin_t, float* out, int L, int hd, void* stream) {
  if (L == 0 || hd == 0) return PDN_OK;
  PDN_CHECK_ARG(cos_t && sin_t && out && hd % 2 == 0 && (((uintptr_t)out & 7) == 0), "pdn_rope_table_f32: bad arguments");
  hipLaunchKernelGGL(rr_rope_table_kernel, dim3((L * hd + 255) / 256), dim3(256), 0, (hipStream_t)stream, cos_t, sin_t,
                     reinterpret_cast<float2*>(out), L * hd, hd);
  PDN_LAUNCH_CHECK();
  return PDN_OK;
}

extern "C" int pdn_gemm_rowres_f32(const float* A, const float* B, float* C, const float* bias,
                                   const float* residual, int M, int N, int K, int64_t lda, int64_t ldb,
                                   int64_t ldc, int b_trans, void* stream) {
  return rowres_launch(A, B, C, bias, residual, M, N, K, lda, ldb, ldc, b_trans, 1, 0, stream);
}

int pdn_gemm_rowres_blocks(const float* A, const float* B, float* C, int M, int N, int K, int64_t lda, int64_t ldb,
                           int64_t ldc, int b_trans, int nblocks, int64_t b_block_stride, void* stream) {
  return rowres_launch(A, B, C, nullptr, nullptr, M, N, K, lda, ldb, ldc, b_trans, nblocks, b_block_stride, stream);
}
```

### pydynet_amd/csrc/gemm_rowtile.h

```cpp
#pragma once
#include <stdint.h>

struct RowTileArgs {
  const float* A;
  const float* B;
  float* C;
  const float* bias;
  const float* residual;
  int M, N;
  int64_t lda, ldb, ldc;
  int b_trans;
  int nblocks;
  int64_t b_block_stride;
  int epi;
  float* H; int64_t ldh;
  const float* GU;
  int F;
  const float* rope; int L, hd, rope_cols;
  unsigned g_off, u_off;
  float* lse;
  int* parts;
  const float* norm_w; float* xn; float* rms; int64_t ldxn; float norm_eps;
};

int pdn_rowtile_takes(const RowTileArgs& a);
int pdn_rowtile_launch(const RowTileArgs& a, void* stream);
int pdn_rowtile_split_takes(const RowTileArgs& a, void* stream);
int pdn_rowtile_split_launch(const RowTileArgs& a, void* stream);
```

### pydynet_amd/csrc/outres_tn_split.hip

```cpp
#include "split_tn.h"

struct OtsParams {
  const float* g;
  const char* ximg;
  const int* xsh;
  float* C;
  int n_all, nb_cols, K, k_per_split;
  int64_t ldg, slab, blk_stride;
};

__device__ __forceinline__ unsigned ots_finite_bits(float v) {
  const unsigned b = __float_as_uint(v) & 0x7fffffffu;
  return b < 0x7f800000u ? b : 0u;
}
__device__ __forceinline__ unsigned ots_wave_max_bits(const float (&v)[8]) {
  unsigned m = ots_finite_bits(v[0]);
#pragma unroll
  for (int k = 1; k < 8; ++k) m = max(m, ots_finite_bits(v[k]));
  m = max(m, (unsigned)__builtin_amdgcn_update_dpp(0, (int)m, 0xB1, 0xf, 0xf, false));
  m = max(m, (unsigned)__builtin_amdgcn_update_dpp(0, (int)m, 0x4E, 0xf, 0xf, false));
  m = max(m, (unsigned)__builtin_amdgcn_update_dpp(0, (int)m, 0x141, 0xf, 0xf, false));
  m = max(m, (unsigned)__builtin_amdgcn_update_dpp(0, (int)m, 0x140, 0xf, 0xf, false));
  const unsigned a = __builtin_amdgcn_readlane((int)m, 0), b = __builtin_amdgcn_readlane((int)m, 16);
  const unsigned c = __builtin_amdgcn_readlane((int)m, 32), d = __builtin_amdgcn_readlane((int)m, 48);
// ... 77 lines not shown
  int cur = 0;
  for (int s = 0; s < np; ++s) {
    asm volatile("s_waitcnt vmcnt(%0)" ::"n"(TOPWAIT) : "memory");
    __builtin_amdgcn_s_barrier();
    asm volatile("" ::: "memory");
    const char* fb = smem + cur + frag;
    const char* raw = smem + g_lane + ((s + 1) & (STN_RING - 1)) * STN_RAW;
    f16x8 xh[2], xl[2];
    u32x4 nh = __builtin_bit_cast(u32x4, bh), nl = __builtin_bit_cast(u32x4, bl);
    float rv[8] = {0.f, 0.f, 0.f, 0.f, 0.f, 0.f, 0.f, 0.f};
    int Sn = S;
    stn_load_frag(fb, 0, xh[0], xl[0]);
#pragma unroll
    for (int j = 0; j < STN_NT; ++j) {
      if (j + 1 < STN_NT) stn_load_frag(fb, j + 1, xh[(j + 1) & 1], xl[(j + 1) & 1]);
      if (j == 0) {
        dma_x(min(s + 1, np - 1), 1 - (cur != 0));
        if (ABLATE == 0) dma_g(s + 4, s & (STN_RING - 1));
        if (ABLATE != 1) {
#pragma unroll
          for (int k = 0; k < 8; ++k) rv[k] = *reinterpret_cast<const float*>(raw + k * 512);
        }
      }
      if (ABLATE != 1 && j == 2) Sn = ots_next_scale(ots_wave_max_bits(rv), S);
      __builtin_amdgcn_sched_barrier(0);
      stn_mfma3(xh[j & 1], xl[j & 1], bh, bl, acc0[j], acc1[j]);
      if (ABLATE != 1 && (j & 3) == 0 && j >= 4) {
        const int e = (j >> 2) - 1;
        unsigned hp, lp;
        ots_form2(rv[2 * e], rv[2 * e + 1], Sn, hp, lp);
        if (e == 0) { nh.x = hp; nl.x = lp; } else if (e == 1) { nh.y = hp; nl.y = lp; }
        else if (e == 2) { nh.z = hp; nl.z = lp; } else { nh.w = hp; nl.w = lp; }
        stn_sched_pair();
      }
      __builtin_amdgcn_sched_barrier(0);
    }
    bh = __builtin_bit_cast(f16x8, nh); bl = __builtin_bit_cast(f16x8, nl);
    if (Sn != S) {
      if (S != OTS_S_UNSET) {
        const int dS = Sn - S;
#pragma unroll
        for (int j = 0; j < STN_NT; ++j)
#pragma unroll
          for (int i = 0; i < 4; ++i) { acc0[j][i] = ldexpf(acc0[j][i], dS); acc1[j][i] = ldexpf(acc1[j][i], dS); }
      }
      S = Sn;
    }
    cur = cur ? 0 : stn_xpiece(OTS_XKIB);
  }
  asm volatile("s_waitcnt vmcnt(0)" ::: "memory");

  if (!active) return;
  const int Se = S == OTS_S_UNSET ? 0 : S;
  const int* __restrict__ shp = p.xsh + 4 * q;
#pragma unroll
  for (int j = 0; j < STN_NT; ++j) {
    const int4 sv = *reinterpret_cast<const int4*>(shp + 16 * j);
    const int sh[4] = {sv.x, sv.y, sv.z, sv.w};
    if (TSTORE) {
      float4 o;
      o.x = stn_unscale(acc1[j][0], acc0[j][0], Se + sh[0]); o.y = stn_unscale(acc1[j][1], acc0[j][1], Se + sh[1]);
      o.z = stn_unscale(acc1[j][2], acc0[j][2], Se + sh[2]); o.w = stn_unscale(acc1[j][3], acc0[j][3], Se + sh[3]);
      *reinterpret_cast<float4*>(p.C + ots_out_elem_t(by, p.slab, stn_out_row(j, q, 0), col)) = o;
    } else {
#pragma unroll
      for (int i = 0; i < 4; ++i)
        p.C[ots_out_elem(by, p.slab, p.blk_stride, p.nb_cols, stn_out_row(j, q, i), col)] =
            stn_unscale(acc1[j][i], acc0[j][i], Se + sh[i]);
    }
  }
}

int pdn_outres_tn_split_enabled() {
  static const int s_on = ls_env_switch("PDN_OUTRES_TN_SPLIT", 1, "the packed layer weight gradients stay on the fp32 MFMA kernel");
  return s_on;
}
int pdn_outres_tn_split_supported(int M, int nb_cols, int nbatch, int K) {
  const int64_t n_all = (int64_t)nb_cols * nbatch;
  return (M == STN_N && nbatch > 1 && nb_cols % 16 == 0 && n_all >= 768 && n_all <= 8192 && K >= OTS_MIN_K && K % STN_KP == 0) ? 1 : 0;
}
int64_t pdn_outres_tn_split_extra_bytes(int K) { return stn_extra_bytes(K, OTS_XKIB); }
int pdn_outres_tn_split_ranges(int n_all, int K, int plan) { return ots_ranges(n_all, plan, K / STN_KP); }

int pdn_outres_tn_split_launch(const float* X, const float* G, float* C, int n_all, int K, int64_t ldx, int64_t ldg,
                               int nb_cols, int k_per_split, void* extra, void* stream) {
  PDN_CHECK_ARG(n_all % nb_cols == 0 && pdn_outres_tn_split_supported(STN_N, nb_cols, n_all / nb_cols, K) && k_per_split > 0 &&
                    k_per_split % STN_KP == 0 && ((((uintptr_t)X | (uintptr_t)G | (uintptr_t)extra | (uintptr_t)C) & 15) == 0) &&
                    (ldx & 3) == 0 && (ldg & 3) == 0 && ldx >= STN_N && ldg >= n_all,
                "pdn_outres_tn_split_launch: unsupported shape or alignment (K %d, columns %d)", K, n_all);
  static const int s_ablate = ls_env_switch("PDN_OUTRES_TN_SPLIT_ABLATE", 0,
                                            "timing ablation active, the split packed layer weight gradients are WRONG");
  const int ranges = (K + k_per_split - 1) / k_per_split;
  PDN_CHECK_ARG(ranges <= 65535, "pdn_outres_tn_split_launch: %d K ranges", ranges);
  OtsParams p;
  memset(&p, 0, sizeof(p));
  p.g = G; p.ximg = static_cast<const char*>(extra); p.xsh = stn_x_planes_launch(X, ldx, K, extra, nullptr, nullptr, stream);
  p.C = C;
  p.n_all = n_all; p.nb_cols = nb_cols; p.K = K; p.k_per_split = k_per_split;
  p.ldg = ldg; p.slab = (int64_t)STN_N * nb_cols; p.blk_stride = (int64_t)ranges * STN_N * nb_cols;
  STN_LAUNCH_ABLATE(ots_main_kernel, s_ablate, dim3((unsigned)((n_all + STN_COLS - 1) / STN_COLS), (unsigned)ranges), stream, p);
  pdn_count(PDN_CNT_OUTRES_TN);
  pdn_count(PDN_CNT_OUTRES_TN_SPLIT);
  PDN_LAUNCH_CHECK();
  return PDN_OK;
}

int pdn_down_dw_split_supported(int M, int N, int K) {
  return (N == STN_N && M % 16 == 0 && M >= 512 && M <= 1024 && K >= OTS_MIN_K && K % STN_KP == 0) ? 1 : 0;
}
int pdn_down_dw_split_ranges(int M, int K) { return ots_t_ranges(M, K / STN_KP); }

int pdn_down_dw_split_launch(const float* G2, const float* H, float* C, int M, int K, int64_t ldx, int64_t ldg, int k_per_split,
                             void* extra, void* stream) {
  PDN_CHECK_ARG(pdn_down_dw_split_supported(M, STN_N, K) && k_per_split > 0 && k_per_split % STN_KP == 0 &&
                    ((((uintptr_t)G2 | (uintptr_t)H | (uintptr_t)extra | (uintptr_t)C) & 15) == 0) && (ldx & 3) == 0 &&
                    (ldg & 3) == 0 && ldx >= STN_N && ldg >= M,
                "pdn_down_dw_split_launch: unsupported shape or alignment (K %d, rows %d)", K, M);
  const int ranges = (K + k_per_split - 1) / k_per_split;
  PDN_CHECK_ARG(ranges <= OTS_MAX_RANGES, "pdn_down_dw_split_launch: %d K ranges", ranges);
  OtsParams p;
  memset(&p, 0, sizeof(p));
  p.g = H; p.ximg = static_cast<const char*>(extra); p.xsh = stn_x_planes_launch(G2, ldx, K, extra, nullptr, nullptr, stream);
  p.C = C;
  p.n_all = M; p.nb_cols = M; p.K = K; p.k_per_split = k_per_split;
  p.ldg = ldg; p.slab = (int64_t)STN_N * M; p.blk_stride = 0;
  hipLaunchKernelGGL((ots_main_kernel<0, true>), dim3((unsigned)((M + STN_COLS - 1) / STN_COLS), (unsigned)ranges), dim3(512), 0,
                     (hipStream_t)stream, p);
  pdn_count(PDN_CNT_DOWN_DW_SPLIT);
  PDN_LAUNCH_CHECK();
  return PDN_OK;
}
```

### pydynet_amd/csrc/rowtile_split.hip

```cpp
#include "common.h"
#include "lm_head_split.h"
#include "gemm_rowtile.h"
#include "rowtile_split_index.h"
#include <stdlib.h>
#include <type_traits>

typedef float f32x16 __attribute__((ext_vector_type(16)));
typedef _Float16 f16x8 __attribute__((ext_vector_type(8)));

extern "C" int pdn_malloc(void** ptr, int64_t bytes);
extern "C" int pdn_free(void* ptr);

struct RtsWParams {
  const float* B;
  char* wimg;
  int kind, nper;
  int64_t ldb, bstride;
  unsigned g_off, u_off;
};
__global__ __launch_bounds__(256) void rts_w_kernel(RtsWParams p) {
  __shared__ float sm[RTS_K * 33];
  __shared__ float smax[8 * 32];
  const int tid = threadIdx.x, c = tid & 31, kq = tid >> 5, tile = blockIdx.x;
  float amax = 0.f;
// ... 71 lines not shown
}

template <int EPI, bool GUARD, bool NORM>
__global__ __launch_bounds__(512, 1) void rts_main_kernel(RtsParams p) {
  static_assert(EPI == 1 || EPI == 2 || EPI == 3, "SwiGLU, SwiGLU backward or RoPE");
  static_assert(EPI != 2 || !NORM, "SwiGLU backward: no RMSNorm in front");
  __shared__ __attribute__((aligned(16))) char smem[RTS_LDS];
  const int tid = threadIdx.x, lane = tid & 63;
  const int wave = __builtin_amdgcn_readfirstlane(tid >> 6);
  const int li = lane & 31, lh = lane >> 5;
  const int m0 = (blockIdx.x * 8 + wave) * 32;
  const int T0 = blockIdx.y * p.tpw;
  const int T1 = min(p.ntiles, T0 + p.tpw);
  if (T0 >= T1) return;

  const bool q4_on = rts_stage_on(4, tid);
  auto stage_ld = [&](const char* base, int q, uint4& r) __attribute__((always_inline)) {
    if (q < 4 || q4_on) r = *reinterpret_cast<const uint4*>(base + (unsigned)rts_stage_unit(q, tid) * 16u);
  };
  auto stage_park = [&](int slot, int q, const uint4& r) __attribute__((always_inline)) {
    if (q < 4 || q4_on) *reinterpret_cast<uint4*>(smem + slot + rts_stage_unit(q, tid) * 16) = r;
  };

  {
    const char* b0 = p.wimg + (int64_t)T0 * RTS_TILE;
    uint4 t0 = make_uint4(0, 0, 0, 0), t1 = t0, t2 = t0, t3 = t0, t4 = t0;
    stage_ld(b0, 0, t0); stage_ld(b0, 1, t1); stage_ld(b0, 2, t2); stage_ld(b0, 3, t3); stage_ld(b0, 4, t4);
    stage_park(0, 0, t0); stage_park(0, 1, t1); stage_park(0, 2, t2); stage_park(0, 3, t3); stage_park(0, 4, t4);
  }
  char* stg0 = smem + 3 * RTS_TILE + wave * RTS_STG;
  f16x8 xh[RTS_KS], xl[RTS_KS];
  int nexv = 0;
  if (p.ablate & 2) {
#pragma unroll
    for (int s = 0; s < RTS_KS; ++s)
#pragma unroll
      for (int j = 0; j < 8; ++j) { xh[s][j] = (_Float16)1.f; xl[s][j] = (_Float16)0.5f; }
  } else {
    const char* arow[4];
#pragma unroll
    for (int i = 0; i < 4; ++i)
      arow[i] = reinterpret_cast<const char*>(p.A + rts_a_row(m0, rts_pl_row(lane, i), p.M) * p.lda + rts_pl_col(lane, 0));
    const char* wp = reinterpret_cast<const char*>(p.norm_w + rts_pl_col(lane, 0));
    float4 xa[RTS_CHUNKS][4];
#pragma unroll
    for (int c = 0; c < RTS_CHUNKS; ++c)
#pragma unroll
      for (int i = 0; i < 4; ++i) xa[c][i] = *reinterpret_cast<const float4*>(arow[i] + 128 * c);
    float ss[4] = {0.f, 0.f, 0.f, 0.f}, am[4] = {0.f, 0.f, 0.f, 0.f};
#pragma unroll
    for (int c = 0; c < RTS_CHUNKS; ++c) {
      float4 w = make_float4(1.f, 1.f, 1.f, 1.f);
      if (NORM) w = *reinterpret_cast<const float4*>(wp + 128 * c);
#pragma unroll
      for (int i = 0; i < 4; ++i) {
        const float4 a = xa[c][i];
        ss[i] += (a.x * a.x + a.y * a.y) + (a.z * a.z + a.w * a.w);
        const float f0 = fabsf(a.x * w.x), f1 = fabsf(a.y * w.y), f2 = fabsf(a.z * w.z), f3 = fabsf(a.w * w.w);
        am[i] = fmaxf(am[i], fmaxf(fmaxf(f0, f1), fmaxf(f2, f3)));
        if (!((f0 + f1) + (f2 + f3) < INFINITY)) am[i] = INFINITY;
      }
    }
    float inv[4];
#pragma unroll
    for (int i = 0; i < 4; ++i) {
#pragma unroll
      for (int d = 1; d < 8; d <<= 1) {
        ss[i] += __shfl_xor(ss[i], d, 64);
        am[i] = fmaxf(am[i], __shfl_xor(am[i], d, 64));
      }
      float r = 1.f;
      inv[i] = 1.f;
      if (NORM) { r = sqrtf(ss[i] / 288.f + p.norm_eps); inv[i] = 1.f / r; }
      const float amax = NORM ? am[i] * inv[i] : am[i];
      const int sh_i = ls_shift(!(amax < INFINITY) ? INFINITY : amax);
      if ((lane & 7) == 0)
        *reinterpret_cast<float2*>(__builtin_assume_aligned(stg0 + rts_pl_stat(rts_pl_row(lane, i)), 8)) = make_float2(r, __int_as_float(sh_i));
    }
    const float2 st = *reinterpret_cast<const float2*>(__builtin_assume_aligned(stg0 + rts_pl_stat(li), 8));
    const int sh = __float_as_int(st.y);
    nexv = -sh;
    const bool wr_on = blockIdx.y == 0 && !(p.ablate & 1);
    if (NORM && lh == 0 && wr_on && (!GUARD || m0 + li < p.M)) p.rms[m0 + li] = st.x;
    char* xrow[4];
#pragma unroll
    for (int i = 0; i < 4; ++i)
      xrow[i] = reinterpret_cast<char*>(p.xn + rts_a_row(m0, rts_pl_row(lane, i), p.M) * p.ldxn + rts_pl_col(lane, 0));
    char* pw = stg0 + rts_pl_stg_w(lane, 0);
    const char* pf = stg0 + rts_pl_stg_r(li, lh, 0, 0);
#pragma unroll
    for (int c = 0; c < RTS_CHUNKS; ++c) {
      float4 w = make_float4(1.f, 1.f, 1.f, 1.f);
      if (NORM) w = *reinterpret_cast<const float4*>(wp + 128 * c);
#pragma unroll
      for (int i = 0; i < 4; ++i) {
        float4 v = xa[c][i];
        if (NORM) {
          v.x = v.x * inv[i] * w.x; v.y = v.y * inv[i] * w.y; v.z = v.z * inv[i] * w.z; v.w = v.w * inv[i] * w.w;
          if (wr_on && (!GUARD || m0 + rts_pl_row(lane, i) < p.M)) *reinterpret_cast<float4*>(xrow[i] + 128 * c) = v;
        }
        *reinterpret_cast<float4*>(__builtin_assume_aligned(pw + i * (8 * 144), 16)) = v;
      }
#pragma unroll
      for (int e = 0; e < 2; ++e) {
        const int s = 2 * c + e;
        const float4 va = *reinterpret_cast<const float4*>(__builtin_assume_aligned(pf + 64 * e, 16));
        const float4 vb = *reinterpret_cast<const float4*>(__builtin_assume_aligned(pf + 64 * e + 16, 16));
        const float v[8] = {va.x, va.y, va.z, va.w, vb.x, vb.y, vb.z, vb.w};
#pragma unroll
        for (int j = 0; j < 8; ++j) {
          _Float16 h, l;
          ls_split(v[j], sh, h, l);
          xh[s][j] = h; xl[s][j] = l;
        }
      }
    }
  }

  f32x16 acc0, acc1;
  float out[16];
#pragma unroll
  for (int r = 0; r < 16; ++r) { acc0[r] = 0.f; acc1[r] = 0.f; out[r] = 0.f; }
  const f32x16 zero16 = {0.f, 0.f, 0.f, 0.f, 0.f, 0.f, 0.f, 0.f, 0.f, 0.f, 0.f, 0.f, 0.f, 0.f, 0.f, 0.f};

  const int fr_even = rts_frag_base(li, lh, 0), fr_odd = rts_frag_base(li, lh, 1);
  const int tail_lane = RTS_TAIL + 4 * rts_reg_col(0, lh);
  char* stg = stg0;
  char* stg_w = stg + rts_stg_w(li, lh, 0);
  const char* stg_r = stg + rts_stg_r(lane, 0);
  const char* stgh_r = stg + rts_h_r(lane, 0);
  const bool st_all = !(p.ablate & 1);
  const int srow = m0 + rts_st_row(lane, 0), hrow = m0 + rts_h_row(lane, 0);
  const unsigned ob = 4u * (unsigned)rts_st_row(lane, 0) * p.ldc +
                      (EPI == 1 ? ((lane & 4) ? 4u * (unsigned)p.F + 16u * (unsigned)(lane & 3) : 16u * (unsigned)(lane & 3))
                                : 4u * (unsigned)rts_st_col(lane));
  const unsigned obh = 4u * (unsigned)rts_h_row(lane, 0) * p.ldh + 16u * (unsigned)(lane & 3);
  const unsigned ldc32 = 32u * p.ldc, ldh64 = 64u * p.ldh;
  const unsigned Fb = 4u * (unsigned)p.F;
  const bool gu_on = !(p.ablate & 4);
  float4 pg[2], pu[2];
  pg[0] = pg[1] = pu[0] = pu[1] = make_float4(1.f, 1.f, 1.f, 1.f);
  const unsigned tab_lane = 8u * (unsigned)rts_rope_pos(m0, li, p.L) * (unsigned)p.hd;

  auto rope_ld = [&](int t, int g, float4& r) __attribute__((always_inline)) {
    const unsigned x = 32u * (unsigned)t + 8u * (unsigned)g + 4u * (unsigned)lh;
    const unsigned colh = rts_rope_colh_magic(x, (unsigned)p.hd, p.hd_magic);
    const char* src = reinterpret_cast<const char*>(p.rope) + (tab_lane + 8u * colh);
    const float2 a = *reinterpret_cast<const float2*>(src), b = *reinterpret_cast<const float2*>(src + 16);
    r.x = a.x; r.y = a.y; r.z = b.x; r.w = b.y;
  };
  auto drain_group = [&](int g, const int4& ne, const float4& tb, bool rot) __attribute__((always_inline)) {
    float4 o;
    o.x = ldexpf(out[4 * g + 0], nexv + ne.x);
    o.y = ldexpf(out[4 * g + 1], nexv + ne.y);
    o.z = ldexpf(out[4 * g + 2], nexv + ne.z);
    o.w = ldexpf(out[4 * g + 3], nexv + ne.w);
    if (EPI == 3) {
      const float ex = fmaf(o.x, tb.x, o.y * tb.y), oy = fmaf(o.y, tb.x, -(o.x * tb.y));
      const float ez = fmaf(o.z, tb.z, o.w * tb.w), ow = fmaf(o.w, tb.z, -(o.z * tb.w));
      if (rot) { o.x = ex; o.y = oy; o.z = ez; o.w = ow; }
    }
    *reinterpret_cast<float4*>(__builtin_assume_aligned(stg_w + 32 * g, 16)) = o;
  };
  auto h_group = [&](int g, const int4& ng, const int4& nu) __attribute__((always_inline)) {
    const float g0 = ldexpf(out[4 * g + 0], nexv + ng.x), u0 = ldexpf(out[4 * g + 8], nexv + nu.x);
    const float g1 = ldexpf(out[4 * g + 1], nexv + ng.y), u1 = ldexpf(out[4 * g + 9], nexv + nu.y);
    const float g2 = ldexpf(out[4 * g + 2], nexv + ng.z), u2 = ldexpf(out[4 * g + 10], nexv + nu.z);
    const float g3 = ldexpf(out[4 * g + 3], nexv + ng.w), u3 = ldexpf(out[4 * g + 11], nexv + nu.w);
    float4 o;
    o.x = g0 * rts_sigmoid(g0) * u0; o.y = g1 * rts_sigmoid(g1) * u1;
    o.z = g2 * rts_sigmoid(g2) * u2; o.w = g3 * rts_sigmoid(g3) * u3;
    *reinterpret_cast<float4*>(__builtin_assume_aligned(stg + rts_h_w(li, lh, 0) + 32 * g, 16)) = o;
  };
  auto store_rows = [&](int j, float* Cd) __attribute__((always_inline)) {
    const float4 v = *reinterpret_cast<const float4*>(__builtin_assume_aligned(stg_r + j * (8 * 144), 16));
    if (st_all && (!GUARD || srow + 8 * j < p.M))
      *reinterpret_cast<float4*>(reinterpret_cast<char*>(Cd) + ob + (unsigned)j * ldc32) = v;
  };
  auto store_h = [&](int j, float* Hd) __attribute__((always_inline)) {
    const float4 v = *reinterpret_cast<const float4*>(__builtin_assume_aligned(stgh_r + j * (16 * 144), 16));
    if (st_all && (!GUARD || hrow + 16 * j < p.M))
      *reinterpret_cast<float4*>(reinterpret_cast<char*>(Hd) + obh + (unsigned)j * ldh64) = v;
// ... 68 lines not shown
      if (!FIRST && dg >= 0) drain_group(dg, ne, tb, rot);
      if (EPI == 3 && !FIRST && (s == 0 || s == 4 || s == 8 || s == 12)) rope_ld(t - 1, s >> 2, tb);
      if (EPI == 2 && !FIRST && (s == 4 || s == 5)) store_bwd(s - 4, Cd, pg[s - 4], pu[s - 4]);
      if (EPI == 2 && !FIRST && s == 6) { gu_ld(2, g_of(t - 1), pg[0], pu[0]); gu_ld(3, g_of(t - 1), pg[1], pu[1]); }
      if (EPI == 2 && !FIRST && (s == 11 || s == 12)) store_bwd(s - 9, Cd, pg[s - 11], pu[s - 11]);
      if (s == 0) { stage_ld(nb, 0, r0); stage_ld(nb, 1, r1); }
      if (s == 6) { stage_ld(nb, 2, r0); stage_ld(nb, 3, r1); }
      if (s == 12) stage_ld(nb, 4, r0);
      if (EPI == 2 && s == 13) { gu_ld(0, g_of(t), pg[0], pu[0]); gu_ld(1, g_of(t), pg[1], pu[1]); }
      if (EPI == 3 && !FIRST && s >= 16) { store_rows(2 * (s - 16), Cd); store_rows(2 * (s - 16) + 1, Cd); }
      if (EPI == 1 && !FIRST && s >= 8 && s < 12) store_rows(s - 8, Cd);
      if (!FIRST && hg >= 0) h_group(hg, ne, nu);
      if (EPI == 1 && !FIRST && (s == 14 || s == 15)) store_h(s - 14, Hd);
      __builtin_amdgcn_sched_barrier(0);
    }
#undef RTS_LOADH
#undef RTS_LOADL
#pragma unroll
    for (int r = 0; r < 16; ++r) out[r] = fmaf(acc1[r], 1.f / 2048.f, acc0[r]);
  };

  int cur = 0, prv = 2 * RTS_TILE, nxt = RTS_TILE;
  run_tile(rts_ic<1>{}, T0, cur, prv, nxt);
  for (int t = T0 + 1; t < T1; ++t) {
    prv = cur; cur = nxt; nxt = nxt == 2 * RTS_TILE ? 0 : nxt + RTS_TILE;
    run_tile(rts_ic<0>{}, t, cur, prv, nxt);
  }
  {
    float* Cd = c_of(T1 - 1);
    const bool rot = EPI == 3 && T1 - 1 < p.rope_tiles;
    const char* tl = smem + cur + tail_lane;
    float4 tb[4];
#pragma unroll
    for (int g = 0; g < 4; ++g) {
      tb[g] = make_float4(0.f, 0.f, 0.f, 0.f);
      if (EPI == 3) rope_ld(T1 - 1, g, tb[g]);
    }
    float4 lg[2], lu[2];
    lg[0] = lg[1] = lu[0] = lu[1] = make_float4(1.f, 1.f, 1.f, 1.f);
    if (EPI == 2) { gu_ld(2, g_of(T1 - 1), lg[0], lu[0]); gu_ld(3, g_of(T1 - 1), lg[1], lu[1]); }
#pragma unroll
    for (int g = 0; g < 4; ++g) {
      const int4 ne = *reinterpret_cast<const int4*>(__builtin_assume_aligned(tl + 32 * g, 16));
      drain_group(g, ne, tb[g], rot);
    }
    __builtin_amdgcn_sched_barrier(0);
    if (EPI == 2) {
      store_bwd(0, Cd, pg[0], pu[0]); store_bwd(1, Cd, pg[1], pu[1]);
      store_bwd(2, Cd, lg[0], lu[0]); store_bwd(3, Cd, lg[1], lu[1]);
    } else {
#pragma unroll
      for (int j = 0; j < 4; ++j) store_rows(j, Cd);
    }
    if (EPI == 1) {
      __builtin_amdgcn_sched_barrier(0);
#pragma unroll
      for (int g = 0; g < 2; ++g) {
        const int4 ng = *reinterpret_cast<const int4*>(__builtin_assume_aligned(tl + 32 * g, 16));
        const int4 nu = *reinterpret_cast<const int4*>(__builtin_assume_aligned(tl + 32 * g + 64, 16));
        h_group(g, ng, nu);
      }
      __builtin_amdgcn_sched_barrier(0);
      float* Hd = h_of(T1 - 1);
      store_h(0, Hd); store_h(1, Hd);
    }
  }
}

namespace {
struct RtsTemp {
  void* p = nullptr;
  hipStream_t st = nullptr;
  int get(int64_t bytes, void* stream) { st = (hipStream_t)stream; return pdn_malloc(&p, bytes); }
  ~RtsTemp() {
    static const bool two_stream = getenv("PDN_TWO_STREAM") && atoi(getenv("PDN_TWO_STREAM")) != 0;
    if (p && two_stream) (void)hipStreamSynchronize(st);
    if (p) pdn_free(p);
  }
};
}

static int rts_tiles(const RowTileArgs& a) { return a.epi == 1 ? a.F / 16 : a.N / 32; }

int pdn_rowtile_split_takes(const RowTileArgs& a, void* stream) {
  static const int s_on = ls_env_switch("PDN_ROWTILE_SPLIT", 1, "the q | k | v and gate | up projections and dh + SwiGLU backward stay on the fp32 MFMA kernel");
  if (!s_on || (a.epi != 1 && a.epi != 2 && a.epi != 3) || a.M < RTS_MIN_ROWS || a.bias || a.residual) return 0;
  if ((a.epi == 2) != (a.b_trans != 0)) return 0;
  if (a.N < 32 || a.N % 32 != 0 || a.nblocks < 1 || (a.N / a.nblocks) * a.nblocks != a.N || (a.N / a.nblocks) % 32 != 0) return 0;
  if ((a.lda & 3) || (a.ldc & 3) || a.lda < RTS_K || a.ldc < a.N || a.ldc >= (1 << 24) || a.ldb < (a.b_trans ? RTS_K : a.N / a.nblocks)) return 0;
  if (((uintptr_t)a.A | (uintptr_t)a.C) & 15) return 0;
  if (a.epi == 1 && (a.F < 16 || a.F % 16 != 0 || a.N != 2 * a.F || a.nblocks != 2 || !a.H || (a.ldh & 3) || a.ldh < a.F ||
                     a.ldh >= (1 << 24) || ((uintptr_t)a.H & 15)))
    return 0;
  if (a.epi == 2) {
    if (a.F < 32 || a.F % 32 != 0 || a.N != a.F || a.nblocks != 1 || a.ldc < 2 * (int64_t)a.F || !a.GU || ((uintptr_t)a.GU & 15)) return 0;
    const float* ce = a.C + (int64_t)a.M * a.ldc;
    if ((const float*)a.C < a.GU + (int64_t)a.M * a.ldc && a.GU < ce) return 0;
    if ((const float*)a.C < a.A + (int64_t)a.M * a.lda && a.A < ce) return 0;
  }
  if (a.epi == 3 && (!a.rope || a.hd < 4 || a.hd % 4 != 0 || a.L < 1 || a.rope_cols % 32 != 0 || a.rope_cols > a.N ||
                     (int64_t)a.L * a.hd >= (1 << 27) || ((uintptr_t)a.rope & 7)))
    return 0;
  if (a.norm_w && !(a.xn && a.rms && (a.ldxn & 3) == 0 && a.ldxn >= RTS_K && (((uintptr_t)a.xn | (uintptr_t)a.norm_w) & 15) == 0)) return 0;
  hipStreamCaptureStatus cs = hipStreamCaptureStatusNone;
  if (hipStreamIsCapturing((hipStream_t)stream, &cs) != hipSuccess) { (void)hipGetLastError(); return 0; }
  return cs == hipStreamCaptureStatusNone ? 1 : 0;
}

int pdn_rowtile_split_launch(const RowTileArgs& a, void* stream) {
  static const int s_ablate = ls_env_switch("PDN_ROWTILE_SPLIT_ABLATE", 0, "timing ablation active, the results of the split q | k | v, gate | up and dh + SwiGLU backward kernels are WRONG");
  const int nt = rts_tiles(a);
  RtsTemp img;
  const int rc = img.get((int64_t)nt * RTS_TILE, stream);
  if (rc) return rc;
  hipStream_t st = (hipStream_t)stream;
  RtsWParams w;
  memset(&w, 0, sizeof(w));
  w.B = a.B; w.wimg = static_cast<char*>(img.p); w.kind = a.epi; w.nper = a.N / a.nblocks; w.ldb = a.ldb;
  w.bstride = a.nblocks > 1 ? a.b_block_stride : 0; w.g_off = a.g_off; w.u_off = a.u_off;
  hipLaunchKernelGGL(rts_w_kernel, dim3(nt), dim3(256), 0, st, w);
  RtsParams p;
  memset(&p, 0, sizeof(p));
  p.A = a.A; p.lda = a.lda; p.wimg = w.wimg; p.C = a.C; p.H = a.H; p.GU = a.GU ? a.GU : a.A; p.ldc = (unsigned)a.ldc; p.ldh = (unsigned)a.ldh;
  p.rope = a.rope ? a.rope : a.A; p.L = a.L > 0 ? a.L : 1; p.hd = a.hd > 0 ? a.hd : 32; p.rope_tiles = a.rope_cols / 32;
  p.hd_magic = rts_rope_magic(p.hd);
  p.F = a.F; p.norm_w = a.norm_w ? a.norm_w : a.A; p.xn = a.xn ? a.xn : a.C; p.rms = a.rms; p.ldxn = a.ldxn; p.norm_eps = a.norm_eps;
  p.M = a.M; p.ntiles = nt; p.ablate = s_ablate;
  int parts;
  rts_plan(a.M, nt, &p.tpw, &parts);
  const dim3 grid((a.M + 255) / 256, parts), block(512);
  const bool guard = a.M % 256 != 0, norm = a.norm_w != nullptr;
#define RTS_LAUNCH(EPI_)                                                                                      \
  if (guard) { if (norm) hipLaunchKernelGGL((rts_main_kernel<EPI_, true, true>), grid, block, 0, st, p);      \
               else hipLaunchKernelGGL((rts_main_kernel<EPI_, true, false>), grid, block, 0, st, p); }        \
  else { if (norm) hipLaunchKernelGGL((rts_main_kernel<EPI_, false, true>), grid, block, 0, st, p);           \
         else hipLaunchKernelGGL((rts_main_kernel<EPI_, false, false>), grid, block, 0, st, p); }
  if (a.epi == 1) { RTS_LAUNCH(1) }
  else if (a.epi == 3) { RTS_LAUNCH(3) }
  else if (guard) hipLaunchKernelGGL((rts_main_kernel<2, true, false>), grid, block, 0, st, p);
  else hipLaunchKernelGGL((rts_main_kernel<2, false, false>), grid, block, 0, st, p);
#undef RTS_LAUNCH
  pdn_count(PDN_CNT_ROWTILE_PLAIN + a.epi);
  pdn_count(a.epi == 2 ? PDN_CNT_ROWTILE_BWD_SPLIT : PDN_CNT_ROWTILE_SPLIT);
  PDN_LAUNCH_CHECK();
  return PDN_OK;
}
```

### pydynet_amd/csrc/split_tn.h

```cpp
#pragma once
#include "common.h"
#include "lm_head_split.h"
#include "split_tn_index.h"

int* stn_x_planes_launch(const float* x, int64_t ldx, int rows, void* extra, const float* lse, const int64_t* targets, void* stream);
int pdn_outres_tn_split_enabled();
int pdn_outres_tn_split_supported(int M, int nb_cols, int nbatch, int K);
int64_t pdn_outres_tn_split_extra_bytes(int K);
int pdn_outres_tn_split_ranges(int n_all, int K, int plan);
int pdn_outres_tn_split_launch(const float* X, const float* G, float* C, int n_all, int K, int64_t ldx, int64_t ldg,
                               int nb_cols, int k_per_split, void* extra, void* stream);
int pdn_down_dw_split_supported(int M, int N, int K);
int pdn_down_dw_split_ranges(int M, int K);
int pdn_down_dw_split_launch(const float* G2, const float* H, float* C, int M, int K, int64_t ldx, int64_t ldg, int k_per_split,
                             void* extra, void* stream);
int pdn_outres_ce_dw_split_enabled();
int pdn_outres_ce_dw_split_supported(int64_t rows, int V, int in_features);
int64_t pdn_outres_ce_dw_split_extra_bytes(int64_t rows);
int pdn_outres_ce_dw_split_launch(const float* x, int64_t ldx, const float* logits, float* C, int V, int64_t rows,
                                  int64_t slab, int k_per_split, const float* lse, const int64_t* targets, float gscale,
                                  const float* gdev, float* colsum, void* extra, void* stream);

typedef float f32x4 __attribute__((ext_vector_type(4)));
typedef _Float16 f16x8 __attribute__((ext_vector_type(8)));
typedef _Float16 f16x2 __attribute__((ext_vector_type(2)));
typedef unsigned u32x4 __attribute__((ext_vector_type(4)));

__device__ __forceinline__ void split_dma16(const void* g, unsigned lds) {
  asm volatile("s_mov_b32 m0, %1\n\ts_nop 0\n\tglobal_load_lds_dwordx4 %0, off" ::"v"(g), "s"(lds) : "memory");
}

__device__ __forceinline__ void stn_load_frag(const char* fb, int J, f16x8& h, f16x8& l) {
  h = *reinterpret_cast<const f16x8*>(__builtin_assume_aligned(fb + J * 1024, 16));
  l = *reinterpret_cast<const f16x8*>(__builtin_assume_aligned(fb + J * 1024 + STN_PLANE, 16));
}
__device__ __forceinline__ void stn_mfma3(f16x8 xh, f16x8 xl, f16x8 bh, f16x8 bl, f32x4& acc0, f32x4& acc1) {
  acc0 = __builtin_amdgcn_mfma_f32_16x16x32_f16(xh, bh, acc0, 0, 0, 0);
  acc1 = __builtin_amdgcn_mfma_f32_16x16x32_f16(xl, bh, acc1, 0, 0, 0);
  acc1 = __builtin_amdgcn_mfma_f32_16x16x32_f16(xh, bl, acc1, 0, 0, 0);
}
__device__ __forceinline__ void stn_sched_pair() {
  __builtin_amdgcn_sched_group_barrier(0x008, 1, 0);
  __builtin_amdgcn_sched_group_barrier(0x002, 8, 0);
  __builtin_amdgcn_sched_group_barrier(0x008, 1, 0);
  __builtin_amdgcn_sched_group_barrier(0x002, 8, 0);
  __builtin_amdgcn_sched_group_barrier(0x008, 1, 0);
}
__device__ __forceinline__ f16x8 stn_pack4(unsigned w0, unsigned w1, unsigned w2, unsigned w3) {
  const u32x4 v = {w0, w1, w2, w3};
  return __builtin_bit_cast(f16x8, v);
}
#define STN_CLEAR(acc0, acc1)                                                \
  _Pragma("unroll") for (int j_ = 0; j_ < STN_NT; ++j_)                      \
    _Pragma("unroll") for (int i_ = 0; i_ < 4; ++i_) { acc0[j_][i_] = 0.f; acc1[j_][i_] = 0.f; }
__device__ __forceinline__ float stn_unscale(float a1, float a0, int e) { return ldexpf(fmaf(a1, 1.f / 2048.f, a0), -e); }

#define STN_LAUNCH_ABLATE(K, ablate, grid, stream, p)                                              \
  do {                                                                                             \
    if ((ablate) == 1) hipLaunchKernelGGL(K<1>, grid, dim3(512), 0, (hipStream_t)(stream), p);     \
    else if ((ablate) == 2) hipLaunchKernelGGL(K<2>, grid, dim3(512), 0, (hipStream_t)(stream), p); \
    else hipLaunchKernelGGL(K<0>, grid, dim3(512), 0, (hipStream_t)(stream), p);                   \
  } while (0)
```

### pydynet_amd/csrc/split_tn_planes.hip

```cpp
#include "split_tn.h"

#define STN_L2E 1.4426950408889634f

__global__ __launch_bounds__(288) void stn_x_colmax_kernel(const float* __restrict__ x, int64_t ldx, int rows, int rows_per_block,
                                                            float* __restrict__ partial) {
  __shared__ float sm[4][STN_N];
  const int c4 = threadIdx.x % 72, g = threadIdx.x / 72;
  const int r0 = blockIdx.x * rows_per_block, r1 = min(rows, r0 + rows_per_block);
  float4 m = make_float4(0.f, 0.f, 0.f, 0.f);
  float4 z = m;
#pragma unroll 4
  for (int r = r0 + g; r < r1; r += 4) {
    const float4 v = *reinterpret_cast<const float4*>(x + (int64_t)r * ldx + 4 * c4);
    m.x = fmaxf(m.x, fabsf(v.x)); m.y = fmaxf(m.y, fabsf(v.y)); m.z = fmaxf(m.z, fabsf(v.z)); m.w = fmaxf(m.w, fabsf(v.w));
    z.x = fmaf(v.x, 0.f, z.x); z.y = fmaf(v.y, 0.f, z.y); z.z = fmaf(v.z, 0.f, z.z); z.w = fmaf(v.w, 0.f, z.w);
  }
  if (z.x != z.x) m.x = INFINITY;
  if (z.y != z.y) m.y = INFINITY;
  if (z.z != z.z) m.z = INFINITY;
  if (z.w != z.w) m.w = INFINITY;
  sm[g][4 * c4 + 0] = m.x; sm[g][4 * c4 + 1] = m.y; sm[g][4 * c4 + 2] = m.z; sm[g][4 * c4 + 3] = m.w;
  __syncthreads();
  const int d = threadIdx.x;
  partial[(int64_t)blockIdx.x * STN_N + d] = fmaxf(fmaxf(sm[0][d], sm[1][d]), fmaxf(sm[2][d], sm[3][d]));
}

__global__ __launch_bounds__(256) void stn_x_shift_kernel(const float* __restrict__ partial, int nparts, int* __restrict__ xsh) {
  __shared__ float sm[4];
  const int d = blockIdx.x;
  float m = 0.f;
  for (int b = threadIdx.x; b < nparts; b += 256) m = fmaxf(m, partial[(int64_t)b * STN_N + d]);
  m = wave_max(m);
  if ((threadIdx.x & 63) == 0) sm[threadIdx.x >> 6] = m;
  __syncthreads();
  if (threadIdx.x == 0) xsh[d] = ls_shift(fmaxf(fmaxf(sm[0], sm[1]), fmaxf(sm[2], sm[3])));
}

template <int XKIB, bool TAIL>
__device__ __forceinline__ void stn_split_x(const float* __restrict__ x, int64_t ldx, const int* __restrict__ xsh,
                                            const float* __restrict__ lse, const int64_t* __restrict__ targets, int rows,
                                            char* __restrict__ ximg) {
  __shared__ __attribute__((aligned(16))) float raw[STN_KP * STN_N];
  char* img = ximg + (int64_t)blockIdx.x * stn_xpiece(XKIB);
  const float* xp = x + (int64_t)blockIdx.x * STN_KP * ldx;
  float4 v[STN_PASS_LOADS];
#pragma unroll
  for (int e = 0; e < STN_PASS_LOADS; ++e) {
    const int i = threadIdx.x + STN_PASS_THREADS * e;
    v[e] = *reinterpret_cast<const float4*>(xp + (int64_t)stn_pass_row(i) * ldx + 4 * stn_pass_chunk(i));
  }
#pragma unroll
  for (int e = 0; e < STN_PASS_LOADS; ++e) {
    const int i = threadIdx.x + STN_PASS_THREADS * e;
    *reinterpret_cast<float4*>(raw + stn_pass_lds(stn_pass_row(i), 4 * stn_pass_chunk(i))) = v[e];
  }
  __syncthreads();
#pragma unroll
  for (int e = 0; e < (STN_N * 4 + STN_PASS_THREADS - 1) / STN_PASS_THREADS; ++e) {
    const int u = threadIdx.x + STN_PASS_THREADS * e;
    if (u < STN_N * 4) {
      const int d = stn_pass_unit_d(u), q = stn_pass_unit_q(u);
      const int sh = xsh[d];
      f16x8 hv, lv;
#pragma unroll
      for (int k = 0; k < 8; ++k) {
        _Float16 h, l;
        ls_split(raw[stn_pass_lds(8 * q + k, d)], sh, h, l);
        hv[k] = h; lv[k] = l;
      }
      *reinterpret_cast<f16x8*>(img + 16 * u) = hv;
      *reinterpret_cast<f16x8*>(img + STN_PLANE + 16 * u) = lv;
    }
  }
  if (TAIL) {
    const int i = threadIdx.x;
    const int64_t t = ((int64_t)blockIdx.x + 1) * STN_KP + (i & 31);
    unsigned v = 0u;
    if (i < 64 && t < rows) v = i < 32 ? __float_as_uint(-STN_L2E * lse[t]) : (unsigned)(int)targets[t];
    reinterpret_cast<unsigned*>(img + LDW_TAIL)[i] = v;
  }
}
__global__ __launch_bounds__(256) void stn_split_x_kernel(const float* __restrict__ x, int64_t ldx, const int* __restrict__ xsh,
                                                           char* __restrict__ ximg) {
  stn_split_x<OTS_XKIB, false>(x, ldx, xsh, nullptr, nullptr, 0, ximg);
}
__global__ __launch_bounds__(256) void stn_split_x_tail_kernel(const float* __restrict__ x, int64_t ldx, const int* __restrict__ xsh,
                                                                const float* __restrict__ lse, const int64_t* __restrict__ targets,
                                                                int rows, char* __restrict__ ximg) {
  stn_split_x<LDW_XKIB, true>(x, ldx, xsh, lse, targets, rows, ximg);
}

int* stn_x_planes_launch(const float* x, int64_t ldx, int rows, void* extra, const float* lse, const int64_t* targets, void* stream) {
  hipStream_t st = (hipStream_t)stream;
  const bool tail = lse != nullptr;
  const int npieces = rows / STN_KP;
  char* ximg = static_cast<char*>(extra);
  int* xsh = reinterpret_cast<int*>(ximg + (int64_t)npieces * stn_xpiece(tail ? LDW_XKIB : OTS_XKIB));
  float* partial = reinterpret_cast<float*>(ximg);
  const int nparts = stn_partials(rows);
  const int rpb = (rows + nparts - 1) / nparts;
  const int nblk = (rows + rpb - 1) / rpb;
  hipLaunchKernelGGL(stn_x_colmax_kernel, dim3(nblk), dim3(288), 0, st, x, ldx, rows, rpb, partial);
  hipLaunchKernelGGL(stn_x_shift_kernel, dim3(STN_N), dim3(256), 0, st, partial, nblk, xsh);
  if (tail) hipLaunchKernelGGL(stn_split_x_tail_kernel, dim3(npieces), dim3(256), 0, st, x, ldx, xsh, lse, targets, rows, ximg);
  else hipLaunchKernelGGL(stn_split_x_kernel, dim3(npieces), dim3(256), 0, st, x, ldx, xsh, ximg);
  return xsh;
}
```

Before: 9388.

## Fold RMSNorm into QKV and gate/up weight-gradient planes instead of storing xn

For large row counts, the fused norm+QKV/rope and norm+gate/up forward kernels no longer write the normalized activation xn; they keep only the raw input and the per-row rms. In backward, the stacked weight-gradient GEMM rebuilds the normalized input on the fly inside a new plane-split kernel. That kernel scales raw x by 1/rms and the norm weight while producing the fp16 hi/lo planes. It derives the per-column shift from the norm weights, which skips the column-max and shift passes. This removes an activation-sized write and read per layer, at the cost of recomputing the normalization and relying on a weight-based scaling bound for the split precision.

```diff
diff --git a/include/pdn_normplanes.h b/include/pdn_normplanes.h
--- /dev/null
+++ b/include/pdn_normplanes.h
@@ -0,0 +1,25 @@
+#ifndef PDN_NORMPLANES_H
+#define PDN_NORMPLANES_H
+#include <stdint.h>
+#ifdef __cplusplus
+extern "C" {
+#endif
+
+int pdnp_gateup_swiglu_norm_supported(int M, int F, int K);
+int pdnp_gateup_swiglu_norm_fwd_f32(const float* x, const float* norm_w, float eps, float* rms, const float* w_gate,
+                                    int64_t w_stride, float* gu, float* h, int M, int F, int K, int64_t ldx, void* stream);
+int pdnp_qkv_rope_norm_supported(int M, int D, int K, int L, int hd);
+int pdnp_qkv_rope_norm_fwd_f32(const float* x, const float* norm_w, float eps, float* rms, const float* wq, int64_t w_stride,
+                               float* qkv, const float* rope, int M, int D, int K, int L, int hd, int64_t ldx, void* stream);
+
+int pdnp_norm_dw_blocks_f32(const float* x, const float* norm_w, const float* rms, const float* G, int64_t ldg, float* dW,
+                            int64_t dw_block_stride, float beta, int K, int nb_cols, int nb, void* workspace,
+                            int64_t workspace_bytes, void* stream);
+int64_t pdnp_norm_dw_blocks_workspace_bytes(int K, int nb_cols, int nb);
+int pdnp_norm_dw_blocks_supported(int K, int nb_cols, int nb);
+int64_t pdnp_norm_dw_blocks_plane_launches(int reset);
+
+#ifdef __cplusplus
+}
+#endif
+#endif
diff --git a/pydynet_amd/_lib.py b/pydynet_amd/_lib.py
--- a/pydynet_amd/_lib.py
+++ b/pydynet_amd/_lib.py
@@ -16,6 +16,7 @@
 PERSAMPLE_HEADER_PATHS = (os.path.join(os.path.dirname(_HERE), "include", "pdn_persample.h"),)
 FSM_HEADER_PATHS = (os.path.join(os.path.dirname(_HERE), "include", "pdn_fsm.h"),)
 NORMGRAD_HEADER_PATHS = (os.path.join(os.path.dirname(_HERE), "include", "pdn_normgrad.h"),)
+NORMPLANES_HEADER_PATHS = (os.path.join(os.path.dirname(_HERE), "include", "pdn_normplanes.h"),)
 
 _CTYPE = {
     "int": ctypes.c_int,
@@ -30,7 +31,7 @@
     text = re.sub(r"/\*.*?\*/", "", text, flags=re.S)
     text = re.sub(r"//[^\n]*", "", text)
     protos = {}
-    for m in re.finditer(r"(const\s+char\s*\*|int64_t|int)\s+(pdn[xlsrzeqfg]?_\w+)\s*\(([^)]*)\)\s*;", text, flags=re.S):
+    for m in re.finditer(r"(const\s+char\s*\*|int64_t|int)\s+(pdn[xlsrzeqfgp]?_\w+)\s*\(([^)]*)\)\s*;", text, flags=re.S):
         ret, name, args = m.group(1), m.group(2), m.group(3)
         restype = ctypes.c_char_p if "char" in ret else _CTYPE[ret]
         argtypes = []
@@ -63,7 +64,8 @@
         self.cdll = ctypes.CDLL(LIB_PATH, mode=ctypes.RTLD_GLOBAL)
         self.protos = parse_header()
         for path in (EXT_HEADER_PATHS + LOSS_HEADER_PATHS + SEG_HEADER_PATHS + ROWLOSS_HEADER_PATHS + SMOOTH_HEADER_PATHS
-                     + EDIT_HEADER_PATHS + PERSAMPLE_HEADER_PATHS + FSM_HEADER_PATHS + NORMGRAD_HEADER_PATHS):
+                     + EDIT_HEADER_PATHS + PERSAMPLE_HEADER_PATHS + FSM_HEADER_PATHS + NORMGRAD_HEADER_PATHS
+                     + NORMPLANES_HEADER_PATHS):
             self.protos.update(parse_header(path))
         self.fn = {}
         for name, (restype, argtypes) in self.protos.items():
diff --git a/pydynet_amd/core/fused/_common.py b/pydynet_amd/core/fused/_common.py
--- a/pydynet_amd/core/fused/_common.py
+++ b/pydynet_amd/core/fused/_common.py
@@ -143,6 +143,20 @@
         return self._array
 
 
+def _norm_dw_blocks(hp, L, norm, dcat, gstack, T, nb_cols, nb):
+    raw, rms, wn, eps = norm
+    ws, wsb = hp.workspace(L.query("pdnp_norm_dw_blocks_workspace_bytes", T, nb_cols, nb))
+    L.call("pdnp_norm_dw_blocks_f32", raw._ptr, wn._ptr, rms._ptr, dcat._ptr, dcat._strides[0], gstack._ptr, gstack._strides[0],
+           1.0, T, nb_cols, nb, ws, wsb, hp.stream())
+
+
+def _xn_of(hp, L, norm, T, cols):
+    raw, rms, wn, eps = norm
+    xn = hp.empty((T, cols), np.float32)
+    L.call("pdn_rmsnorm_fwd_f32", raw._ptr, wn._ptr, xn._ptr, None, T, cols, eps, hp.stream())
+    return xn
+
+
 def _materialised(g):
     return g.materialise() if isinstance(g, DeferredInputGrad) else g
 
diff --git a/pydynet_amd/core/fused/attn.py b/pydynet_amd/core/fused/attn.py
--- a/pydynet_amd/core/fused/attn.py
+++ b/pydynet_amd/core/fused/attn.py
@@ -9,7 +9,8 @@
 from . import segments as _seg
 from .norm import rms_norm
 from ..tensor import Tensor, _Operator
-from ._common import _hip, _L, _contig, _require_f32, _beside, _is_leaf_f32, _dx_of_shared_input
+from ._common import (_hip, _L, _contig, _require_f32, _beside, _is_leaf_f32, _dx_of_shared_input, _provides, _norm_dw_blocks,
+                      _xn_of)
 
 
 def _attn_layout(x):
@@ -285,6 +286,8 @@
     rope_epilogue = os.environ.get("PDN_NO_ROPE_EPILOGUE", "0") != "1"
     rope_min_rows = 4096
     prerotate = os.environ.get("PDN_NO_PREROTATE", "0") != "1"
+    norm_planes = os.environ.get("PDN_NO_NORM_PLANES", "0") != "1"
+    norm_planes_min_rows = 65536
     _rope_tables = {}
 
     @staticmethod
@@ -340,15 +343,25 @@
                             and L.query("pdn_qkv_rope_supported", T, D, D, Lq, hd))
         self.norm_folded = bool(self.rotated and isinstance(x, rms_norm) and x._pending is not None
                                 and L.query("pdn_qkv_rope_norm_supported", T, D, D, Lq, hd))
+        self._norm = None
         if self.norm_folded:
             raw_t, wn = x._pending
             raw = _contig(raw_t.data)
-            xn, rms = hp.empty(x.shape, np.float32), hp.empty((T,), np.float32)
+            rms = hp.empty((T,), np.float32)
             tab = self._rope_table(cos, sin, Lq, hd)
-            L.call("pdn_qkv_rope_norm_fwd_f32", raw._ptr, _contig(wn.data)._ptr, x.eps, xn._ptr, rms._ptr, ws[0]._ptr,
-                   (ws[1]._ptr - ws[0]._ptr) // 4, qkv._ptr, tab._ptr, T, D, D, Lq, hd, D, hp.stream())
-            x._adopt(raw, rms, xn)
-        x2 = _contig(x.data).reshape(T, D)
+            if (qkv_attention.norm_planes and T >= qkv_attention.norm_planes_min_rows and _provides("pdnp_norm_dw_blocks_f32") and hp.capturing() is None
+                    and L.query("pdnp_qkv_rope_norm_supported", T, D, D, Lq, hd)):
+                wnd = _contig(wn.data)
+                L.call("pdnp_qkv_rope_norm_fwd_f32", raw._ptr, wnd._ptr, x.eps, rms._ptr, ws[0]._ptr,
+                       (ws[1]._ptr - ws[0]._ptr) // 4, qkv._ptr, tab._ptr, T, D, D, Lq, hd, D, hp.stream())
+                x._adopt_stats(raw, rms)
+                self._norm = (raw, rms, wnd, x.eps)
+            else:
+                xn = hp.empty(x.shape, np.float32)
+                L.call("pdn_qkv_rope_norm_fwd_f32", raw._ptr, _contig(wn.data)._ptr, x.eps, xn._ptr, rms._ptr, ws[0]._ptr,
+                       (ws[1]._ptr - ws[0]._ptr) // 4, qkv._ptr, tab._ptr, T, D, D, Lq, hd, D, hp.stream())
+                x._adopt(raw, rms, xn)
+        x2 = _contig(x.data).reshape(T, D) if self._norm is None else None
         if self.norm_folded:
             pass
         elif self.rotated:
@@ -427,9 +440,13 @@
         dws = [hp.empty(w.shape, np.float32) if gstack is None and w.requires_grad and not _is_leaf_f32(w) else None
                for w in weights]
         with side or contextlib.nullcontext():
-            if gstack is not None:
+            if gstack is not None and self._norm is not None:
+                _norm_dw_blocks(hp, L, self._norm, dqkv, gstack, T, D, 3)
+            elif gstack is not None:
                 hp.gemm(x2.T, dblocks, gstack, beta=1.0)
             else:
+                if x2 is None:
+                    x2 = _xn_of(hp, L, self._norm, T, D)
                 for i, w in enumerate(weights):
                     if not w.requires_grad:
                         continue
diff --git a/pydynet_amd/core/fused/ffn.py b/pydynet_amd/core/fused/ffn.py
--- a/pydynet_amd/core/fused/ffn.py
+++ b/pydynet_amd/core/fused/ffn.py
@@ -7,7 +7,8 @@
 
 from .norm import rms_norm
 from ..tensor import _Operator
-from ._common import (_hip, _L, _contig, _require_f32, _foldable, _beside, _is_leaf_f32, _pack_columns, _dx_of_shared_input)
+from ._common import (_hip, _L, _contig, _require_f32, _foldable, _beside, _is_leaf_f32, _pack_columns, _dx_of_shared_input,
+                      _provides, _norm_dw_blocks, _xn_of)
 
 
 class gate_up_swiglu(_Operator):
@@ -95,6 +96,8 @@
     enabled = os.environ.get("PDN_NO_FFN_NODE", "0") != "1"
     epilogues = os.environ.get("PDN_NO_SWIGLU_EPILOGUE", "0") != "1"
     epilogue_min_rows = 4096
+    norm_planes = os.environ.get("PDN_NO_NORM_PLANES", "0") != "1"
+    norm_planes_min_rows = 65536
 
     @staticmethod
     def applicable(x, wg, wu, wd):
@@ -126,14 +129,24 @@
                                    and L.query("pdn_gateup_swiglu_tiled_supported", T, F, fin))
         self.norm_folded = bool(self.used_epilogue and isinstance(x, rms_norm) and x._pending is not None
                                 and L.query("pdn_gateup_swiglu_norm_supported", T, F, fin))
+        self._norm = None
         if self.norm_folded:
             raw_t, wn = x._pending
             raw = _contig(raw_t.data)
-            xn, rms = hp.empty(x.shape, np.float32), hp.empty((T,), np.float32)
-            L.call("pdn_gateup_swiglu_norm_fwd_f32", raw._ptr, _contig(wn.data)._ptr, x.eps, xn._ptr, rms._ptr, ws[0]._ptr,
-                   (ws[1]._ptr - ws[0]._ptr) // 4, gu._ptr, h._ptr, T, F, fin, fin, hp.stream())
-            x._adopt(raw, rms, xn)
-        x2 = _contig(x.data).reshape(-1, fin)
+            rms = hp.empty((T,), np.float32)
+            if (ffn_swiglu.norm_planes and T >= ffn_swiglu.norm_planes_min_rows and _provides("pdnp_norm_dw_blocks_f32") and hp.capturing() is None
+                    and L.query("pdnp_gateup_swiglu_norm_supported", T, F, fin)):
+                wnd = _contig(wn.data)
+                L.call("pdnp_gateup_swiglu_norm_fwd_f32", raw._ptr, wnd._ptr, x.eps, rms._ptr, ws[0]._ptr,
+                       (ws[1]._ptr - ws[0]._ptr) // 4, gu._ptr, h._ptr, T, F, fin, fin, hp.stream())
+                x._adopt_stats(raw, rms)
+                self._norm = (raw, rms, wnd, x.eps)
+            else:
+                xn = hp.empty(x.shape, np.float32)
+                L.call("pdn_gateup_swiglu_norm_fwd_f32", raw._ptr, _contig(wn.data)._ptr, x.eps, xn._ptr, rms._ptr, ws[0]._ptr,
+                       (ws[1]._ptr - ws[0]._ptr) // 4, gu._ptr, h._ptr, T, F, fin, fin, hp.stream())
+                x._adopt(raw, rms, xn)
+        x2 = _contig(x.data).reshape(-1, fin) if self._norm is None else None
         if self.norm_folded:
             pass
         elif self.used_epilogue:
@@ -162,7 +175,7 @@
         x, wg, wu, wd = self.last[:4]
         fin, F = wg.shape
         x2, gu, h = self._saved
-        T = x2.shape[0]
+        T = h.shape[0]
         grads = [None] * len(self.last)
         if self.has_res and self.last[4].requires_grad:
             grads[4] = g
@@ -190,9 +203,13 @@
         gstack = None
         if all(w.requires_grad and _is_leaf_f32(w) for w in weights):
             gstack = hp.stacked_view([w.grad for w in weights])
-        if gstack is not None:
+        if gstack is not None and self._norm is not None:
+            _norm_dw_blocks(hp, L, self._norm, dgu, gstack, T, F, 2)
+        elif gstack is not None:
             hp.gemm(x2.T, dhalves, gstack, beta=1.0)
         else:
+            if x2 is None:
+                x2 = _xn_of(hp, L, self._norm, T, fin)
             for i, w in enumerate(weights):
                 if not w.requires_grad:
                     continue
diff --git a/pydynet_amd/core/fused/norm.py b/pydynet_amd/core/fused/norm.py
--- a/pydynet_amd/core/fused/norm.py
+++ b/pydynet_amd/core/fused/norm.py
@@ -32,6 +32,12 @@
         self._x, self._rms = raw, rms
         self.data = out
 
+    def _adopt_stats(self, raw, rms):
+        self._x, self._rms = raw, rms
+        self._stats_adopted = True
+
+    _stats_adopted = False
+
     def forward_(self, x, w):
         if self.xp is np:
             self._rms = np.sqrt((x.data * x.data).mean(-1, keepdims=True) + np.asarray(self.eps, x.dtype))
@@ -39,12 +45,13 @@
         _require_f32(self, x, w)
         hp, L = _hip(), _L()
         cols = x.shape[-1]
-        self._x = _contig(x.data)
-        rows = self._x.size // cols
+        xc = _contig(x.data)
+        rows = xc.size // cols
         out = hp.empty(x.shape, np.float32)
-        self._rms = hp.empty((rows,), np.float32)
-        L.call("pdn_rmsnorm_fwd_f32", self._x._ptr, w.data._ptr, out._ptr, self._rms._ptr, rows, cols,
-               self.eps, hp.stream())
+        rms = hp.empty((rows,), np.float32)
+        L.call("pdn_rmsnorm_fwd_f32", xc._ptr, w.data._ptr, out._ptr, rms._ptr, rows, cols, self.eps, hp.stream())
+        if not self._stats_adopted:
+            self._x, self._rms = xc, rms
         return out
 
     def backward_all(self, g):
diff --git a/pydynet_amd/csrc/gemm.hip b/pydynet_amd/csrc/gemm.hip
--- a/pydynet_amd/csrc/gemm.hip
+++ b/pydynet_amd/csrc/gemm.hip
@@ -133,6 +133,8 @@
   int64_t ws_bytes, ws_floats;
   void* stream;
   hipStream_t st;
+  const float* norm_w = nullptr;
+  const float* norm_rms = nullptr;
 };
 constexpr int kNotTaken = -0x7fffffff - 1;
 
@@ -283,6 +285,7 @@
   const int64_t xoff = (((int64_t)64 * M * n_all * 4 + 255) & ~(int64_t)255);
   const bool split16 = pdn_outres_tn_split_supported(M, N, nbatch, K) && pdn_outres_tn_split_enabled() && c.workspace &&
                        c.workspace_bytes >= xoff + pdn_outres_tn_split_extra_bytes(K) && al16(c.workspace);
+  if (c.norm_w && !split16) return kNotTaken;
   if (split16) {
     kps = ((K / 32 + pdn_outres_tn_split_ranges((int)n_all, K, splits) - 1) / pdn_outres_tn_split_ranges((int)n_all, K, splits)) * 32;
     splits = (K + kps - 1) / kps;
@@ -292,7 +295,9 @@
   if (getenv("PDN_GEMM_DEBUG"))
     fprintf(stderr, "pdn_gemm_f32 M=%d N=%lld K=%d -> output-resident TN%s (%d blocks, splits %d)\n", M,
             (long long)n_all, K, split16 ? ", split-fp16" : "", nbatch, splits);
-  const int rc = split16 ? pdn_outres_tn_split_launch(p.A, p.B, (float*)c.workspace, (int)n_all, K, p.a_cs, p.b_rs, N, kps,
+  const int rc = c.norm_w ? pdn_outres_tn_split_norm_launch(p.A, c.norm_w, c.norm_rms, p.B, (float*)c.workspace, (int)n_all, K,
+                                                            p.a_cs, p.b_rs, N, kps, (char*)c.workspace + xoff, c.stream)
+                 : split16 ? pdn_outres_tn_split_launch(p.A, p.B, (float*)c.workspace, (int)n_all, K, p.a_cs, p.b_rs, N, kps,
                                                       (char*)c.workspace + xoff, c.stream)
                          : pdn_gemm_outres_tn_blocks_launch(p.A, p.B, (float*)c.workspace, (int)n_all, K, p.a_cs, p.b_rs, N, nw, kps,
                                                             c.stream);
@@ -402,7 +407,7 @@
                          int64_t c_bs1, int64_t c_bs2, const float* residual,
                          float* b_colsum, int colsum_accumulate, void* workspace,
                          int64_t workspace_bytes, void* stream, uint32_t* relu_mask, const uint32_t* grad_mask,
-                         float* mask_colsum = nullptr) {
+                         float* mask_colsum = nullptr, const float* norm_w = nullptr, const float* norm_rms = nullptr) {
   const bool ext_on = relu_mask || grad_mask;
   PDN_CHECK_ARG(!ext_on || (nb1 == 1 && nb2 == 1 && N % 32 == 0 && !b_colsum),
                 "pdn_gemm_f32: the mask epilogues need one batch and N a multiple of 32 (N = %d)", N);
@@ -412,6 +417,7 @@
   PDN_CHECK_ARG(ldc >= N, "pdn_gemm_f32: ldc (%lld) < N (%d)", (long long)ldc, N);
 
   GemmCall c;
+  c.norm_w = norm_w; c.norm_rms = norm_rms;
   GemmParams& p = c.p;
   p.A = A; p.B = B; p.C = C; p.bias = bias; p.ws = (float*)workspace;
   p.residual = residual; p.colsum = b_colsum; p.colsum_acc = colsum_accumulate;
@@ -438,6 +444,7 @@
     }
   }
   int rc;
+  if (c.norm_w) return route_outres_tn_blocks(c);
   if ((rc = route_skinny(c)) != kNotTaken) return rc;
   if ((rc = route_narrow(c)) != kNotTaken) return rc;
   if ((rc = route_outres(c)) != kNotTaken) return rc;
@@ -458,6 +465,14 @@
                             int64_t workspace_bytes, void* stream) {
   return gemm_f32_impl(M, N, K, alpha, A, a_rs, a_cs, B, b_rs, b_cs, beta, C, ldc, bias, nb1, nb2, a_bs1, a_bs2, b_bs1, b_bs2,
                        c_bs1, c_bs2, residual, b_colsum, colsum_accumulate, workspace, workspace_bytes, stream, nullptr, nullptr);
+}
+
+int pdn_gemm_outres_tn_blocks_norm(const float* x, const float* norm_w, const float* rms, const float* G, int64_t ldg, float* dW,
+                                   int64_t ldc, int64_t c_bs, float beta, int K, int nb_cols, int nb, void* workspace,
+                                   int64_t workspace_bytes, void* stream) {
+  const int rc = gemm_f32_impl(288, nb_cols, K, 1.f, x, 1, 288, G, ldg, 1, beta, dW, ldc, nullptr, 1, nb, 0, 0, 0, nb_cols, 0, c_bs,
+                               nullptr, nullptr, 0, workspace, workspace_bytes, stream, nullptr, nullptr, nullptr, norm_w, rms);
+  return rc == kNotTaken ? PDN_NORMPLANES_NOT_TAKEN : rc;
 }
 
 extern "C" int pdn_relu_mask_supported(int64_t rows, int cols) { return rows > 0 && cols > 0 && cols % 32 == 0; }
diff --git a/pydynet_amd/csrc/gemm_routes.h b/pydynet_amd/csrc/gemm_routes.h
--- a/pydynet_amd/csrc/gemm_routes.h
+++ b/pydynet_amd/csrc/gemm_routes.h
@@ -58,3 +58,8 @@
 int pdn_gemm_rowres_blocks(const float* A, const float* B, float* C, int M, int N, int K, int64_t lda, int64_t ldb,
                            int64_t ldc, int b_trans, int nblocks, int64_t b_block_stride, void* stream);
 extern "C" int pdn_gemm_rowtile_mode(int mode);
+
+#define PDN_NORMPLANES_NOT_TAKEN (-0x7fffffff)
+int pdn_gemm_outres_tn_blocks_norm(const float* x, const float* norm_w, const float* rms, const float* G, int64_t ldg, float* dW,
+                                   int64_t ldc, int64_t c_bs, float beta, int K, int nb_cols, int nb, void* workspace,
+                                   int64_t workspace_bytes, void* stream);
diff --git a/pydynet_amd/csrc/gemm_rowres.hip b/pydynet_amd/csrc/gemm_rowres.hip
--- a/pydynet_amd/csrc/gemm_rowres.hip
+++ b/pydynet_amd/csrc/gemm_rowres.hip
@@ -2,6 +2,7 @@
 #include "gemm_rowtile.h"
 #include "gemm_prof.h"
 #include "gemm_routes.h"
+#include "rowtile_split_index.h"
 #include <stdlib.h>
 
 static int pdn_ablation_switch(const char* name) {
@@ -690,14 +691,12 @@
 extern "C" int pdn_gateup_swiglu_norm_supported(int M, int F, int K) {
   return (pdn_gateup_swiglu_supported(M, F, K) && rowtile_would_take(M, 2 * F, 1, F)) ? 1 : 0;
 }
-extern "C" int pdn_gateup_swiglu_norm_fwd_f32(const float* x, const float* norm_w, float eps, float* xn, float* rms,
-                                              const float* w_gate, int64_t w_stride, float* gu, float* h, int M, int F,
-                                              int K, int64_t ldx, void* stream) {
-  if (M == 0 || F == 0) return PDN_OK;
-  PDN_CHECK_ARG(x && norm_w && xn && rms && w_gate && gu && h, "pdn_gateup_swiglu_norm_fwd_f32: null operand");
+static int gateup_norm_fwd(const char* name, const float* x, const float* norm_w, float eps, float* xn, float* rms,
+                           const float* w_gate, int64_t w_stride, float* gu, float* h, int M, int F, int K, int64_t ldx,
+                           void* stream) {
   const int64_t ws = w_stride < 0 ? -w_stride : w_stride;
   if (!pdn_gateup_swiglu_norm_supported(M, F, K) || ws % 4 != 0 || ws < (int64_t)K * F || ws + (int64_t)K * F >= (1ll << 30)) {
-    pdn_set_error("pdn_gateup_swiglu_norm_fwd_f32: unsupported shape M=%d F=%d K=%d", M, F, K);
+    pdn_set_error("%s: unsupported shape M=%d F=%d K=%d", name, M, F, K);
     return PDN_EUNSUPPORTED;
   }
   RowResEpi e{1, h, F, nullptr, F, nullptr, 1, 1, 0};
@@ -710,6 +709,28 @@
   pdn_gemm_prof_end(tk, stream);
   return rc;
 }
+extern "C" int pdn_gateup_swiglu_norm_fwd_f32(const float* x, const float* norm_w, float eps, float* xn, float* rms,
+                                              const float* w_gate, int64_t w_stride, float* gu, float* h, int M, int F,
+                                              int K, int64_t ldx, void* stream) {
+  if (M == 0 || F == 0) return PDN_OK;
+  PDN_CHECK_ARG(x && norm_w && xn && rms && w_gate && gu && h, "pdn_gateup_swiglu_norm_fwd_f32: null operand");
+  return gateup_norm_fwd("pdn_gateup_swiglu_norm_fwd_f32", x, norm_w, eps, xn, rms, w_gate, w_stride, gu, h, M, F, K, ldx, stream);
+}
+static bool rowtile_split_open() { return pdn_rowtile_split_enabled() && pdn_gemm_rowtile_mode(-1) != 3; }
+extern "C" int pdnp_gateup_swiglu_norm_supported(int M, int F, int K) {
+  return (pdn_gateup_swiglu_norm_supported(M, F, K) && M >= RTS_MIN_ROWS && 2 * (int64_t)F < (1 << 24) && rowtile_split_open()) ? 1 : 0;
+}
+extern "C" int pdnp_gateup_swiglu_norm_fwd_f32(const float* x, const float* norm_w, float eps, float* rms, const float* w_gate,
+                                               int64_t w_stride, float* gu, float* h, int M, int F, int K, int64_t ldx,
+                                               void* stream) {
+  if (M == 0 || F == 0) return PDN_OK;
+  PDN_CHECK_ARG(x && norm_w && rms && w_gate && gu && h, "pdnp_gateup_swiglu_norm_fwd_f32: null operand");
+  if (!pdnp_gateup_swiglu_norm_supported(M, F, K)) {
+    pdn_set_error("pdnp_gateup_swiglu_norm_fwd_f32: unsupported shape M=%d F=%d K=%d, or the split-fp16 kernel is switched off", M, F, K);
+    return PDN_EUNSUPPORTED;
+  }
+  return gateup_norm_fwd("pdnp_gateup_swiglu_norm_fwd_f32", x, norm_w, eps, nullptr, rms, w_gate, w_stride, gu, h, M, F, K, ldx, stream);
+}
 extern "C" int pdn_swiglu_bwd_gemm_f32(const float* dy, const float* w_down, const float* gu, float* dgu, int M, int F, int K,
                                        int64_t ldy, void* stream) {
   if (M == 0 || F == 0) return PDN_OK;
@@ -745,22 +766,43 @@
 extern "C" int pdn_qkv_rope_norm_supported(int M, int D, int K, int L, int hd) {
   return (pdn_qkv_rope_supported(M, D, K, L, hd) && rowtile_would_take(M, 3 * D, 3, 0)) ? 1 : 0;
 }
+static int qkv_norm_fwd(const char* name, const float* x, const float* norm_w, float eps, float* xn, float* rms, const float* wq,
+                        int64_t w_stride, float* qkv, const float* rope, int M, int D, int K, int L, int hd, int64_t ldx,
+                        void* stream) {
+  if (!pdn_qkv_rope_norm_supported(M, D, K, L, hd) || w_stride % 4 != 0) {
+    pdn_set_error("%s: unsupported shape M=%d D=%d K=%d L=%d hd=%d", name, M, D, K, L, hd);
+    return PDN_EUNSUPPORTED;
+  }
+  RowResEpi e{3, nullptr, 0, nullptr, 0, rope, L, hd, 2 * D};
+  e.norm_w = norm_w; e.xn = xn; e.rms = rms; e.ldxn = K; e.norm_eps = eps;
+  const int tk = pdn_gemm_prof_begin(5, 2.0 * M * (3.0 * D) * K, 4.0 * (2.0 * M * K + 3.0 * K * D + 3.0 * M * D), stream);
+  const int rc = rowres_launch(x, wq, qkv, nullptr, nullptr, M, 3 * D, K, ldx, D, 3 * D, 0, 3, w_stride, stream, &e);
+  pdn_gemm_prof_end(tk, stream);
+  return rc;
+}
 extern "C" int pdn_qkv_rope_norm_fwd_f32(const float* x, const float* norm_w, float eps, float* xn, float* rms, const float* wq,
                                          int64_t w_stride, float* qkv, const float* rope, int M, int D, int K, int L, int hd,
                                          int64_t ldx, void* stream) {
   if (M == 0 || D == 0) return PDN_OK;
   PDN_CHECK_ARG(x && norm_w && xn && rms && wq && qkv && rope && (((uintptr_t)rope & 7) == 0),
                 "pdn_qkv_rope_norm_fwd_f32: null / misaligned operand");
-  if (!pdn_qkv_rope_norm_supported(M, D, K, L, hd) || w_stride % 4 != 0) {
-    pdn_set_error("pdn_qkv_rope_norm_fwd_f32: unsupported shape M=%d D=%d K=%d L=%d hd=%d", M, D, K, L, hd);
-    return PDN_EUNSUPPORTED;
-  }
-  RowResEpi e{3, nullptr, 0, nullptr, 0, rope, L, hd, 2 * D};
-  e.norm_w = norm_w; e.xn = xn; e.rms = rms; e.ldxn = K; e.norm_eps = eps;
-  const int tk = pdn_gemm_prof_begin(5, 2.0 * M * (3.0 * D) * K, 4.0 * (2.0 * M * K + 3.0 * K * D + 3.0 * M * D), stream);
-  const int rc = rowres_launch(x, wq, qkv, nullptr, nullptr, M, 3 * D, K, ldx, D, 3 * D, 0, 3, w_stride, stream, &e);
-  pdn_gemm_prof_end(tk, stream);
-  return rc;
+  return qkv_norm_fwd("pdn_qkv_rope_norm_fwd_f32", x, norm_w, eps, xn, rms, wq, w_stride, qkv, rope, M, D, K, L, hd, ldx, stream);
+}
+extern "C" int pdnp_qkv_rope_norm_supported(int M, int D, int K, int L, int hd) {
+  return (pdn_qkv_rope_norm_supported(M, D, K, L, hd) && M >= RTS_MIN_ROWS && hd % 4 == 0 && (int64_t)L * hd < (1 << 27) &&
+          3 * (int64_t)D < (1 << 24) && rowtile_split_open()) ? 1 : 0;
+}
+extern "C" int pdnp_qkv_rope_norm_fwd_f32(const float* x, const float* norm_w, float eps, float* rms, const float* wq,
+                                          int64_t w_stride, float* qkv, const float* rope, int M, int D, int K, int L, int hd,
+                                          int64_t ldx, void* stream) {
+  if (M == 0 || D == 0) return PDN_OK;
+  PDN_CHECK_ARG(x && norm_w && rms && wq && qkv && rope && (((uintptr_t)rope & 7) == 0),
+                "pdnp_qkv_rope_norm_fwd_f32: null / misaligned operand");
+  if (!pdnp_qkv_rope_norm_supported(M, D, K, L, hd)) {
+    pdn_set_error("pdnp_qkv_rope_norm_fwd_f32: unsupported shape M=%d D=%d K=%d L=%d hd=%d, or the split-fp16 kernel is switched off", M, D, K, L, hd);
+    return PDN_EUNSUPPORTED;
+  }
+  return qkv_norm_fwd("pdnp_qkv_rope_norm_fwd_f32", x, norm_w, eps, nullptr, rms, wq, w_stride, qkv, rope, M, D, K, L, hd, ldx, stream);
 }
 
 extern "C" int pdn_linear_lse_supported(int64_t M, int V, int K) {
diff --git a/pydynet_amd/csrc/gemm_rowtile.h b/pydynet_amd/csrc/gemm_rowtile.h
--- a/pydynet_amd/csrc/gemm_rowtile.h
+++ b/pydynet_amd/csrc/gemm_rowtile.h
@@ -25,5 +25,6 @@
 
 int pdn_rowtile_takes(const RowTileArgs& a);
 int pdn_rowtile_launch(const RowTileArgs& a, void* stream);
+int pdn_rowtile_split_enabled();
 int pdn_rowtile_split_takes(const RowTileArgs& a, void* stream);
 int pdn_rowtile_split_launch(const RowTileArgs& a, void* stream);
diff --git a/pydynet_amd/csrc/normplanes.hip b/pydynet_amd/csrc/normplanes.hip
--- /dev/null
+++ b/pydynet_amd/csrc/normplanes.hip
@@ -0,0 +1,122 @@
+#include "common.h"
+#include "gemm_routes.h"
+#include "split_tn.h"
+#include <atomic>
+
+extern "C" int pdn_gemm_f32(int M, int N, int K, float alpha, const float* A, int64_t a_rs, int64_t a_cs, const float* B,
+                            int64_t b_rs, int64_t b_cs, float beta, float* C, int64_t ldc, const float* bias, int nb1, int nb2,
+                            int64_t a_bs1, int64_t a_bs2, int64_t b_bs1, int64_t b_bs2, int64_t c_bs1, int64_t c_bs2,
+                            const float* residual, float* b_colsum, int colsum_accumulate, void* workspace,
+                            int64_t workspace_bytes, void* stream);
+extern "C" int64_t pdn_gemm_f32_workspace_bytes(int M, int N, int K, int nbatch);
+extern "C" int pdn_malloc(void** ptr, int64_t bytes);
+extern "C" int pdn_free(void* ptr);
+
+static std::atomic<int64_t> s_plane_launches{0};
+
+static inline int64_t pnp_round256(int64_t b) { return (b + 255) & ~(int64_t)255; }
+static inline int64_t pnp_xn_bytes(int K) { return pnp_round256((int64_t)K * STN_N * 4); }
+static inline int64_t pnp_gemm_bytes(int K, int nb_cols, int nb) {
+  const int64_t b = pdn_gemm_f32_workspace_bytes(STN_N, nb_cols, K, nb);
+  return pnp_round256(b < (1ll << 28) ? b : (1ll << 28));
+}
+
+static bool pnp_env_off(const char* name) {
+  const char* e = getenv(name);
+  return e && atoi(e) == 0;
+}
+static bool pnp_enabled() {
+  if (pnp_env_off("PDN_NORM_PLANES")) {
+    static bool s_told = false;
+    if (!s_told) {
+      s_told = true;
+      fprintf(stderr, "[pdnhip] WARNING: PDN_NORM_PLANES=0 -- the weight gradients behind an RMSNorm write its output and run the product on it\n");
+    }
+    return false;
+  }
+  return true;
+}
+static bool pnp_planes_expected(int K, int nb_cols, int nb) {
+  return pdn_outres_tn_split_supported(STN_N, nb_cols, nb, K) && nb_cols % 32 == 0 && pdn_outres_tn_split_enabled() &&
+         !pnp_env_off("PDN_NORM_PLANES") && !getenv("PDN_GEMM_NO_OUTRES");
+}
+
+extern "C" int pdnp_norm_dw_blocks_supported(int K, int nb_cols, int nb) {
+  return (K >= 1 && nb >= 1 && nb_cols >= 4 && nb_cols % 4 == 0 && (int64_t)nb_cols * nb < (1 << 24)) ? 1 : 0;
+}
+extern "C" int64_t pdnp_norm_dw_blocks_workspace_bytes(int K, int nb_cols, int nb) {
+  if (!pdnp_norm_dw_blocks_supported(K, nb_cols, nb)) return 0;
+  return pnp_gemm_bytes(K, nb_cols, nb) + (pnp_planes_expected(K, nb_cols, nb) ? 0 : pnp_xn_bytes(K));
+}
+extern "C" int64_t pdnp_norm_dw_blocks_plane_launches(int reset) {
+  return reset ? s_plane_launches.exchange(0) : s_plane_launches.load();
+}
+
+__global__ __launch_bounds__(256) void pnp_xn_kernel(const float* __restrict__ x, const float* __restrict__ w,
+                                                      const float* __restrict__ rms, float* __restrict__ xn, int64_t n4) {
+  for (int64_t i = (int64_t)blockIdx.x * 256 + threadIdx.x; i < n4; i += (int64_t)gridDim.x * 256) {
+    const int64_t row = i / (STN_N / 4);
+    const int c4 = (int)(i - row * (STN_N / 4));
+    const float inv = 1.f / rms[row];
+    const float4 wv = *reinterpret_cast<const float4*>(w + 4 * c4);
+    float4 v = *reinterpret_cast<const float4*>(x + 4 * i);
+    v.x = v.x * inv * wv.x; v.y = v.y * inv * wv.y; v.z = v.z * inv * wv.z; v.w = v.w * inv * wv.w;
+    *reinterpret_cast<float4*>(xn + 4 * i) = v;
+  }
+}
+
+namespace {
+struct PnpTemp {
+  void* p = nullptr;
+  hipStream_t st = nullptr;
+  ~PnpTemp() {
+    static const bool two_stream = getenv("PDN_TWO_STREAM") && atoi(getenv("PDN_TWO_STREAM")) != 0;
+    if (p && two_stream) (void)hipStreamSynchronize(st);
+    if (p) pdn_free(p);
+  }
+};
+}
+
+extern "C" int pdnp_norm_dw_blocks_f32(const float* x, const float* w, const float* rms, const float* G, int64_t ldg, float* dW,
+                                       int64_t dw_block_stride, float beta, int K, int nb_cols, int nb, void* workspace,
+                                       int64_t workspace_bytes, void* stream) {
+  PDN_CHECK_ARG(x && w && rms && G && dW, "pdnp_norm_dw_blocks_f32: null operand");
+  if (!pdnp_norm_dw_blocks_supported(K, nb_cols, nb) || ldg < (int64_t)nb_cols * nb) {
+    pdn_set_error("pdnp_norm_dw_blocks_f32: unsupported shape K=%d nb_cols=%d nb=%d", K, nb_cols, nb);
+    return PDN_EUNSUPPORTED;
+  }
+  PDN_CHECK_ARG((((uintptr_t)x | (uintptr_t)w | (uintptr_t)workspace) & 15) == 0 && ((uintptr_t)rms & 3) == 0,
+                "pdnp_norm_dw_blocks_f32: 16B alignment");
+  const int64_t gbytes = pnp_gemm_bytes(K, nb_cols, nb);
+  if (!workspace || workspace_bytes < gbytes) {
+    pdn_set_error("pdnp_norm_dw_blocks_f32: workspace too small");
+    return PDN_EWORKSPACE;
+  }
+  if (pnp_enabled()) {
+    const int rc = pdn_gemm_outres_tn_blocks_norm(x, w, rms, G, ldg, dW, nb_cols, dw_block_stride, beta, K, nb_cols, nb, workspace,
+                                                  gbytes, stream);
+    if (rc == PDN_OK) s_plane_launches.fetch_add(1);
+    if (rc != PDN_NORMPLANES_NOT_TAKEN) return rc;
+  }
+  PnpTemp tmp;
+  float* xn = reinterpret_cast<float*>(static_cast<char*>(workspace) + gbytes);
+  if (workspace_bytes < gbytes + pnp_xn_bytes(K)) {
+    hipStreamCaptureStatus cs = hipStreamCaptureStatusNone;
+    if (hipStreamIsCapturing((hipStream_t)stream, &cs) != hipSuccess || cs != hipStreamCaptureStatusNone) {
+      (void)hipGetLastError();
+      pdn_set_error("pdnp_norm_dw_blocks_f32: the product on a written xn in a captured stream needs %lld bytes of workspace",
+                    (long long)(gbytes + pnp_xn_bytes(K)));
+      return PDN_EWORKSPACE;
+    }
+    const int rm = pdn_malloc(&tmp.p, pnp_xn_bytes(K));
+    if (rm) return rm;
+    tmp.st = (hipStream_t)stream;
+    xn = static_cast<float*>(tmp.p);
+  }
+  const int64_t n4 = (int64_t)K * (STN_N / 4);
+  const int blocks = (int)((n4 + 255) / 256 < 8192 ? (n4 + 255) / 256 : 8192);
+  hipLaunchKernelGGL(pnp_xn_kernel, dim3(blocks), dim3(256), 0, (hipStream_t)stream, x, w, rms, xn, n4);
+  PDN_LAUNCH_CHECK();
+  return pdn_gemm_f32(STN_N, nb_cols, K, 1.f, xn, 1, STN_N, G, ldg, 1, beta, dW, nb_cols, nullptr, 1, nb, 0, 0, 0, nb_cols, 0,
+                      dw_block_stride, nullptr, nullptr, 0, workspace, gbytes, stream);
+}
diff --git a/pydynet_amd/csrc/outres_tn_split.hip b/pydynet_amd/csrc/outres_tn_split.hip
--- a/pydynet_amd/csrc/outres_tn_split.hip
+++ b/pydynet_amd/csrc/outres_tn_split.hip
@@ -183,8 +183,8 @@
 int64_t pdn_outres_tn_split_extra_bytes(int K) { return stn_extra_bytes(K, OTS_XKIB); }
 int pdn_outres_tn_split_ranges(int n_all, int K, int plan) { return ots_ranges(n_all, plan, K / STN_KP); }
 
-int pdn_outres_tn_split_launch(const float* X, const float* G, float* C, int n_all, int K, int64_t ldx, int64_t ldg,
-                               int nb_cols, int k_per_split, void* extra, void* stream) {
+static int ots_launch(const float* X, const float* norm_w, const float* rms, const float* G, float* C, int n_all, int K,
+                      int64_t ldx, int64_t ldg, int nb_cols, int k_per_split, void* extra, void* stream) {
   PDN_CHECK_ARG(n_all % nb_cols == 0 && pdn_outres_tn_split_supported(STN_N, nb_cols, n_all / nb_cols, K) && k_per_split > 0 &&
                     k_per_split % STN_KP == 0 && ((((uintptr_t)X | (uintptr_t)G | (uintptr_t)extra | (uintptr_t)C) & 15) == 0) &&
                     (ldx & 3) == 0 && (ldg & 3) == 0 && ldx >= STN_N && ldg >= n_all,
@@ -195,7 +195,8 @@
   PDN_CHECK_ARG(ranges <= 65535, "pdn_outres_tn_split_launch: %d K ranges", ranges);
   OtsParams p;
   memset(&p, 0, sizeof(p));
-  p.g = G; p.ximg = static_cast<const char*>(extra); p.xsh = stn_x_planes_launch(X, ldx, K, extra, nullptr, nullptr, stream);
+  p.g = G; p.ximg = static_cast<const char*>(extra);
+  p.xsh = norm_w ? stn_xn_planes_launch(X, ldx, norm_w, rms, K, extra, stream) : stn_x_planes_launch(X, ldx, K, extra, nullptr, nullptr, stream);
   p.C = C;
   p.n_all = n_all; p.nb_cols = nb_cols; p.K = K; p.k_per_split = k_per_split;
   p.ldg = ldg; p.slab = (int64_t)STN_N * nb_cols; p.blk_stride = (int64_t)ranges * STN_N * nb_cols;
@@ -204,6 +205,15 @@
   pdn_count(PDN_CNT_OUTRES_TN_SPLIT);
   PDN_LAUNCH_CHECK();
   return PDN_OK;
+}
+int pdn_outres_tn_split_launch(const float* X, const float* G, float* C, int n_all, int K, int64_t ldx, int64_t ldg,
+                               int nb_cols, int k_per_split, void* extra, void* stream) {
+  return ots_launch(X, nullptr, nullptr, G, C, n_all, K, ldx, ldg, nb_cols, k_per_split, extra, stream);
+}
+int pdn_outres_tn_split_norm_launch(const float* x, const float* norm_w, const float* rms, const float* G, float* C, int n_all,
+                                    int K, int64_t ldx, int64_t ldg, int nb_cols, int k_per_split, void* extra, void* stream) {
+  PDN_CHECK_ARG(norm_w && rms && (((uintptr_t)norm_w | (uintptr_t)rms) & 3) == 0, "pdn_outres_tn_split_norm_launch: norm operands");
+  return ots_launch(x, norm_w, rms, G, C, n_all, K, ldx, ldg, nb_cols, k_per_split, extra, stream);
 }
 
 int pdn_down_dw_split_supported(int M, int N, int K) {
diff --git a/pydynet_amd/csrc/rowtile_split.hip b/pydynet_amd/csrc/rowtile_split.hip
--- a/pydynet_amd/csrc/rowtile_split.hip
+++ b/pydynet_amd/csrc/rowtile_split.hip
@@ -177,6 +177,7 @@
     nexv = -sh;
     const bool wr_on = blockIdx.y == 0 && !(p.ablate & 1);
     if (NORM && lh == 0 && wr_on && (!GUARD || m0 + li < p.M)) p.rms[m0 + li] = st.x;
+    const bool xn_on = wr_on && p.xn != nullptr;
     char* xrow[4];
 #pragma unroll
     for (int i = 0; i < 4; ++i)
@@ -192,7 +193,7 @@
         float4 v = xa[c][i];
         if (NORM) {
           v.x = v.x * inv[i] * w.x; v.y = v.y * inv[i] * w.y; v.z = v.z * inv[i] * w.z; v.w = v.w * inv[i] * w.w;
-          if (wr_on && (!GUARD || m0 + rts_pl_row(lane, i) < p.M)) *reinterpret_cast<float4*>(xrow[i] + 128 * c) = v;
+          if (xn_on && (!GUARD || m0 + rts_pl_row(lane, i) < p.M)) *reinterpret_cast<float4*>(xrow[i] + 128 * c) = v;
         }
         *reinterpret_cast<float4*>(__builtin_assume_aligned(pw + i * (8 * 144), 16)) = v;
       }
@@ -427,9 +428,12 @@
 
 static int rts_tiles(const RowTileArgs& a) { return a.epi == 1 ? a.F / 16 : a.N / 32; }
 
+int pdn_rowtile_split_enabled() {
+  static const int s_on = ls_env_switch("PDN_ROWTILE_SPLIT", 1, "the q | k | v and gate | up projections and dh + SwiGLU backward stay on the fp32 MFMA kernel");
+  return s_on;
+}
 int pdn_rowtile_split_takes(const RowTileArgs& a, void* stream) {
-  static const int s_on = ls_env_switch("PDN_ROWTILE_SPLIT", 1, "the q | k | v and gate | up projections and dh + SwiGLU backward stay on the fp32 MFMA kernel");
-  if (!s_on || (a.epi != 1 && a.epi != 2 && a.epi != 3) || a.M < RTS_MIN_ROWS || a.bias || a.residual) return 0;
+  if (!pdn_rowtile_split_enabled() ||(a.epi != 1 && a.epi != 2 && a.epi != 3) || a.M < RTS_MIN_ROWS || a.bias || a.residual) return 0;
   if ((a.epi == 2) != (a.b_trans != 0)) return 0;
   if (a.N < 32 || a.N % 32 != 0 || a.nblocks < 1 || (a.N / a.nblocks) * a.nblocks != a.N || (a.N / a.nblocks) % 32 != 0) return 0;
   if ((a.lda & 3) || (a.ldc & 3) || a.lda < RTS_K || a.ldc < a.N || a.ldc >= (1 << 24) || a.ldb < (a.b_trans ? RTS_K : a.N / a.nblocks)) return 0;
@@ -446,7 +450,7 @@
   if (a.epi == 3 && (!a.rope || a.hd < 4 || a.hd % 4 != 0 || a.L < 1 || a.rope_cols % 32 != 0 || a.rope_cols > a.N ||
                      (int64_t)a.L * a.hd >= (1 << 27) || ((uintptr_t)a.rope & 7)))
     return 0;
-  if (a.norm_w && !(a.xn && a.rms && (a.ldxn & 3) == 0 && a.ldxn >= RTS_K && (((uintptr_t)a.xn | (uintptr_t)a.norm_w) & 15) == 0)) return 0;
+  if (a.norm_w && !(a.rms && (!a.xn || ((a.ldxn & 3) == 0 && a.ldxn >= RTS_K)) && (((uintptr_t)a.xn | (uintptr_t)a.norm_w) & 15) == 0)) return 0;
   hipStreamCaptureStatus cs = hipStreamCaptureStatusNone;
   if (hipStreamIsCapturing((hipStream_t)stream, &cs) != hipSuccess) { (void)hipGetLastError(); return 0; }
   return cs == hipStreamCaptureStatusNone ? 1 : 0;
@@ -469,7 +473,7 @@
   p.A = a.A; p.lda = a.lda; p.wimg = w.wimg; p.C = a.C; p.H = a.H; p.GU = a.GU ? a.GU : a.A; p.ldc = (unsigned)a.ldc; p.ldh = (unsigned)a.ldh;
   p.rope = a.rope ? a.rope : a.A; p.L = a.L > 0 ? a.L : 1; p.hd = a.hd > 0 ? a.hd : 32; p.rope_tiles = a.rope_cols / 32;
   p.hd_magic = rts_rope_magic(p.hd);
-  p.F = a.F; p.norm_w = a.norm_w ? a.norm_w : a.A; p.xn = a.xn ? a.xn : a.C; p.rms = a.rms; p.ldxn = a.ldxn; p.norm_eps = a.norm_eps;
+  p.F = a.F; p.norm_w = a.norm_w ? a.norm_w : a.A; p.xn = a.norm_w ? a.xn : a.C; p.rms = a.rms; p.ldxn = a.ldxn; p.norm_eps = a.norm_eps;
   p.M = a.M; p.ntiles = nt; p.ablate = s_ablate;
   int parts;
   rts_plan(a.M, nt, &p.tpw, &parts);
diff --git a/pydynet_amd/csrc/split_tn.h b/pydynet_amd/csrc/split_tn.h
--- a/pydynet_amd/csrc/split_tn.h
+++ b/pydynet_amd/csrc/split_tn.h
@@ -4,12 +4,15 @@
 #include "split_tn_index.h"
 
 int* stn_x_planes_launch(const float* x, int64_t ldx, int rows, void* extra, const float* lse, const int64_t* targets, void* stream);
+int* stn_xn_planes_launch(const float* x, int64_t ldx, const float* w, const float* rms, int rows, void* extra, void* stream);
 int pdn_outres_tn_split_enabled();
 int pdn_outres_tn_split_supported(int M, int nb_cols, int nbatch, int K);
 int64_t pdn_outres_tn_split_extra_bytes(int K);
 int pdn_outres_tn_split_ranges(int n_all, int K, int plan);
 int pdn_outres_tn_split_launch(const float* X, const float* G, float* C, int n_all, int K, int64_t ldx, int64_t ldg,
                                int nb_cols, int k_per_split, void* extra, void* stream);
+int pdn_outres_tn_split_norm_launch(const float* x, const float* norm_w, const float* rms, const float* G, float* C, int n_all,
+                                    int K, int64_t ldx, int64_t ldg, int nb_cols, int k_per_split, void* extra, void* stream);
 int pdn_down_dw_split_supported(int M, int N, int K);
 int pdn_down_dw_split_ranges(int M, int K);
 int pdn_down_dw_split_launch(const float* G2, const float* H, float* C, int M, int K, int64_t ldx, int64_t ldg, int k_per_split,
diff --git a/pydynet_amd/csrc/split_tn_planes.hip b/pydynet_amd/csrc/split_tn_planes.hip
--- a/pydynet_amd/csrc/split_tn_planes.hip
+++ b/pydynet_amd/csrc/split_tn_planes.hip
@@ -90,6 +90,56 @@
   stn_split_x<LDW_XKIB, true>(x, ldx, xsh, lse, targets, rows, ximg);
 }
 
+__global__ __launch_bounds__(256) void stn_split_xn_kernel(const float* __restrict__ x, int64_t ldx, const float* __restrict__ w,
+                                                            const float* __restrict__ rms, int* __restrict__ xsh,
+                                                            char* __restrict__ ximg) {
+  __shared__ __attribute__((aligned(16))) float raw[STN_KP * STN_N];
+  __shared__ float inv[STN_KP];
+  char* img = ximg + (int64_t)blockIdx.x * stn_xpiece(OTS_XKIB);
+  const float* xp = x + (int64_t)blockIdx.x * STN_KP * ldx;
+  float4 v[STN_PASS_LOADS];
+#pragma unroll
+  for (int e = 0; e < STN_PASS_LOADS; ++e) {
+    const int i = threadIdx.x + STN_PASS_THREADS * e;
+    v[e] = *reinterpret_cast<const float4*>(xp + (int64_t)stn_pass_row(i) * ldx + 4 * stn_pass_chunk(i));
+  }
+  if (threadIdx.x < STN_KP) inv[threadIdx.x] = 1.f / rms[(int64_t)blockIdx.x * STN_KP + threadIdx.x];
+  if (blockIdx.x == 0)
+    for (int d = threadIdx.x; d < STN_N; d += STN_PASS_THREADS) xsh[d] = ls_shift(17.f * fabsf(w[d]));
+#pragma unroll
+  for (int e = 0; e < STN_PASS_LOADS; ++e) {
+    const int i = threadIdx.x + STN_PASS_THREADS * e;
+    *reinterpret_cast<float4*>(raw + stn_pass_lds(stn_pass_row(i), 4 * stn_pass_chunk(i))) = v[e];
+  }
+  __syncthreads();
+#pragma unroll
+  for (int e = 0; e < (STN_N * 4 + STN_PASS_THREADS - 1) / STN_PASS_THREADS; ++e) {
+    const int u = threadIdx.x + STN_PASS_THREADS * e;
+    if (u < STN_N * 4) {
+      const int d = stn_pass_unit_d(u), q = stn_pass_unit_q(u);
+      const float wd = w[d];
+      const int sh = ls_shift(17.f * fabsf(wd));
+      f16x8 hv, lv;
+#pragma unroll
+      for (int k = 0; k < 8; ++k) {
+        _Float16 h, l;
+        ls_split(raw[stn_pass_lds(8 * q + k, d)] * inv[8 * q + k] * wd, sh, h, l);
+        hv[k] = h; lv[k] = l;
+      }
+      *reinterpret_cast<f16x8*>(img + 16 * u) = hv;
+      *reinterpret_cast<f16x8*>(img + STN_PLANE + 16 * u) = lv;
+    }
+  }
+}
+
+int* stn_xn_planes_launch(const float* x, int64_t ldx, const float* w, const float* rms, int rows, void* extra, void* stream) {
+  const int npieces = rows / STN_KP;
+  char* ximg = static_cast<char*>(extra);
+  int* xsh = reinterpret_cast<int*>(ximg + (int64_t)npieces * stn_xpiece(OTS_XKIB));
+  hipLaunchKernelGGL(stn_split_xn_kernel, dim3(npieces), dim3(256), 0, (hipStream_t)stream, x, ldx, w, rms, xsh, ximg);
+  return xsh;
+}
+
 int* stn_x_planes_launch(const float* x, int64_t ldx, int rows, void* extra, const float* lse, const int64_t* targets, void* stream) {
   hipStream_t st = (hipStream_t)stream;
   const bool tail = lse != nullptr;
```

After: 9510 (median of 6 runs). 1.01x the previous value.
